# real-stanford/semantic-abstraction

Hardware: AMD Instinct MI355X
Metric: scenes/sec (relevancy+3D-UNet infer), 480x480x16-label x128^3 (higher is better)
Workload: dtype f16 (MFMA operands, fp32 accumulate; UNet hi/lo-split = fp32-equivalent); 1 GPU; end-to-end relevancy->fusion->OVSSC per scene: 480x480 RGB-D, 16 labels, ViT-B/16, 'ours' saliency config (2448 tile forwards), 128^3 voxels, 80000 input points; scene-sharded; arch=ViT-B/16, unet_precision=exact, tile_chunk_streams=1, scenes_per_gpu=26, parallelism=scene-shard x1, mode=throughput

## Files before the change

### include/semabs.h

```cpp
#ifndef SEMABS_H
#define SEMABS_H
#include <stdint.h>
#ifdef __cplusplus
extern "C" {
#endif

#define SEMABS_OK 0
#define SEMABS_EINVAL (-1)
#define SEMABS_EHIP (-2)

const char* semabs_last_error(void);
int semabs_abi_version(void);
int semabs_stream_create_cumask(const unsigned int* mask, int n_words, void** stream);
int semabs_stream_destroy(void* stream);
int semabs_stream_cu_count(void* stream, int* cus);

int semabs_fill_u32(void* p, long long nbytes, unsigned int value, void* stream);
int semabs_replicate(const void* src, void* dst, long long nbytes, int reps, void* stream);
int semabs_copy2d(const void* src, long long src_pitch_bytes, void* dst, long long dst_pitch_bytes, long long width_bytes, long long rows, void* stream);
int semabs_poison_empty(const long long* n_in, float* logits, long long n_logits, int* labels, long long n_labels, void* stream);
int semabs_device_info(char* name , int name_len, int* cu_count , long long* hbm_bytes );


int semabs_pointcloud(const float* depth, int H, int W, const double* params, int has_pose, float* xyz,
                      unsigned char* mask, void* stream);
int semabs_pointcloud_f64(const float* depth, int H, int W, const double* params_dev, int has_pose, double* xyz64, void* stream);

int semabs_voxel_index(const float* pts, long N, const float* off3, const float* scale3, const int* shape3,
                       long long* flat, int* idx3, void* stream);

int semabs_tsdf_integrate(const unsigned char* color, const float* depth, int H, int W, const double* params,
                          const float* origin3, const float* intr4, const int* dims3, float* tsdf, float* weight,
                          float* colvol, long long* pix_out, void* stream);

int semabs_frustum_mask(const double* pts, long M, const double* params, int H, int W, unsigned char* mask, void* stream);

int semabs_compact_subsample(const unsigned char* mask, long n, unsigned long long seed, long num, long long* pix, long long* n_in,
                             long long* sel, void* stream);

int semabs_gather_point_features(const float* rel, const long long* sel, const float* xyz, int L, long HW, long n,
                                 float mult, int subtract_mean, float* feat, float* xyz_out, void* stream);

int semabs_ovssc_labels(const float* logits, const unsigned char* in_frustum, const float* tsdf, int L, long M,
                        float cutoff, int* label, void* stream);


int semabs_resize_coeffs(int in_size, int out_size, int* xmin, int* kk, int kmax, int* ksize);

int semabs_tile_patches(const unsigned char* images, int n_img, int H, int W, const int* tiles, int n_tiles,
                        const int* coef_xmin, const int* coef_kk, const int* coef_ksize, const void* lut, void* patches,
                        int patch, int flip, int max_ksize, void* stream);

int semabs_patchify(const float* x, void* patches, int n, int patch, int flip, void* stream);

int semabs_aggregate(const float* rel, const float* rel_flip, int L, int N, int g, int H, int W, const int* scales,
                     int n_scales, int n_img, int tiles_per_img, float* out, void* stream);

int semabs_unflip_average(const float* rel, const float* rel_flip, float* out, long n_maps, int g, void* stream);
int semabs_unflip_average_rows(const float* rel, const float* rel_flip, float* out, int L, long maps_per_label, long in_label_stride, int g, void* stream);

int semabs_color_jitter(unsigned char* img, int H, int W, const int* order4, const float* factors4, void* scratch8, void* stream);
int semabs_color_jitter_op(unsigned char* img, int H, int W, int op, float factor, void* scratch8, void* stream);


int semabs_gemm_f16(const void* A, const void* B, void* C, const float* bias, const float* addend, long M, int N, int K,
                    long lda, int ldb, long ldc, int epi, const int* rowmap3, void* stream);

int semabs_gemm_f16_ex(const void* A, const void* B, void* C, const float* bias, const float* addend, long M, int N, int K,
                       long lda, int ldb, long ldc, int epi, const int* rowmap3, int kernel, void* start_event, void* stop_event,
                       void* stream);

int semabs_gemm_f16_ln(const void* A, const void* B, void* C, const float* bias, long M, int N, int K, long lda, int ldb, long ldc, int epi,
                       void* ln_xg, const float* ln_gamma, float* ln_part, const float* ln_center, const float* ln_rowac, const float* ln_colsum,
                       void* lo_out, int lo_cols, long ld_lo, int reverse,
                       void* start_event, void* stop_event, void* stream);
int semabs_ln_rowstats(const float* part, long M, int ntile, int D, float eps, float* rowac, const float* center_in, float* center_out, void* stream);


int semabs_layernorm(const float* x, const float* gamma, const float* beta, void* out, long M, int D, float eps,
                     int out_f32, long ld_in, float* mean_out, void* stream);
int semabs_layernorm2(const float* x, const float* g1, const float* b1, float* out1, const float* g2, const float* b2, void* out2, long M, int D, float eps,
                      int order, float* mean_out, void* stream);
int semabs_add_layernorm(float* x, const void* delta, const float* gamma, const float* beta, void* out, long M, int D, float eps,
                         void* stream);
int semabs_embed_finish(float* x, const float* cls, const float* pos, int n, int T, int D, void* stream);
int semabs_attention(const void* qkv, void* out, void* row_stats, int n_seq, int T, int H, int head_dim, int ld,
                     int causal, void* stream);
int semabs_attention_split(const void* qkv, const void* qk_lo, void* out, void* row_stats, int n_seq, int T, int H, int head_dim, int ld, int ld_lo,
                           int causal, void* stream);
int semabs_attention_cls(const float* q, const float* k, const void* v, float* probs, void* o, int n, int T, int H, int head_dim, int split, void* stream);
int semabs_cls_scores(const float* q, const void* wk, const float* bk, const void* x, long ldx, int split, float* probs, int n, int T, int D, void* stream);
int semabs_rows_gather(const float* src, float* dst, long rows, int cols, long src_stride, long offset, void* stream);
int semabs_eot_rows_gather(const long long* tokens, const float* x, float* dst, int B, int T, int D, void* stream);
int semabs_quickgelu(const float* fc, void* act, long n, int split_w, void* stream);
int semabs_quickgelu_grad(const float* fc, float* gd, long n, void* stream);
int semabs_logit_grad(const float* feat, const float* w_text, int n, int L, int E, float* logits, void* dfeat, float* scale, int split, void* stream);
int semabs_ln_bwd(const float* x, const float* gamma, const float* gy, const float* resid, float* out32, void* out16,
                  long M, int D, int n_x, long ld_x, float eps, int split, void* stream);
int semabs_gelu_bwd(const float* dact, const float* fc, void* dfc, long M, int W, int n_x, int split, void* stream);
int semabs_rollout(const float* probs, const void* v , const float* u, const float* scale, float* rel, int n, int T, int H,
                   int L, int positive_only, long n_total, long tile0, void* stream);
int semabs_attention_bwd(const void* qkv, const void* att, const float* fwd_stats, const void* dO, const float* rvec, const float* gscale,
                         float* c, float* stats, void* dqkv, int n, int L, int T, int H, int head_dim, int positive_only, void* stream);
int semabs_seq_rescale(float* g32, void* g16, float* gscale, long R, long len, void* stream);
int semabs_rollout_step(float* r, float* c, long n, void* stream);
int semabs_gather_text(const long long* tokens, const float* emb, const float* pos, float* x, int B, int T, int D, void* stream);
int semabs_text_finish(const float* e, float* w, int C, int P, int E, void* stream);


int semabs_point_mlp(const float* xyz, const float* feat, const float* w1, const float* b1, const float* w2, const float* b2,
                     const float* w3, const float* b3, float* out, int P, long N, int hidden, int cout, void* stream);
int semabs_point_mlp_fma(const float* xyz, const float* feat, const float* w1, const float* b1, const float* w2, const float* b2,
                         const float* w3, const float* b3, float* out, int P, long N, int hidden, int cout, void* stream);
int semabs_scatter_mean(const long long* flat, const float* feat, int* head, int* next, void* vol, int P, long N, int C,
                        long nvox, int vol_f32, void* stream);
int semabs_scatter_mean_stats(const long long* flat, const float* feat, int* head, int* next, void* vol, int P, long N, int C,
                              long nvox, int vol_f32, double* out_sums, void* stream);
int semabs_scatter_mean_sparse(const long long* flat, const float* feat, int* head, int* next, void* vol, unsigned int* occ, int P, long N, int C, long nvox,
                               int vol_f32, double* out_sums, void* stream);
int semabs_gn_stats(const void* x, double* sums, int B, long nvox, int C, int G, int x_f32, void* stream);
int semabs_gn_finalize(const double* sums, const float* gamma, const float* beta, float* scale, float* shift, int B, int C,
                       int G, long nvox, float eps, void* stream);
int semabs_conv3d(const void* x, const void* w_hi, const void* w_lo, void* y, const float* gn_scale, const float* gn_shift,
                  const float* bias, const void* resid, int B, int D0, int D1, int D2, int Cin, int Cout, int ksize, int relu,
                  int act_f32, void* stream);
int semabs_conv3d_stats(const void* x, const void* w_hi, const void* w_lo, void* y, const float* gn_scale, const float* gn_shift,
                        const float* bias, const void* resid, int B, int D0, int D1, int D2, int Cin, int Cout, int ksize, int relu,
                        int act_f32, double* out_sums, int out_groups, void* stream);
int semabs_conv3d_sparse_stats(const void* x, const unsigned int* occ, const void* w_hi, const void* w_lo, void* y, const float* gn_scale, const float* gn_shift,
                               const float* bias, const void* resid, int B, int D0, int D1, int D2, int Cin, int Cout, int ksize, int relu, int act_f32,
                               double* out_sums, int out_groups, void* stream);
int semabs_convtranspose3d(const void* x, const void* w_hi, const void* w_lo, const long* class_off , void* y,
                           const float* bias, const void* skip, int B, int D0, int D1, int D2, int Cin, int Cout, int act_f32,
                           void* stream);
int semabs_convtranspose3d_stats(const void* x, const void* w_hi, const void* w_lo, const long* class_off, void* y, const float* bias,
                                 const void* skip, int B, int D0, int D1, int D2, int Cin, int Cout, int act_f32, double* out_sums,
                                 int out_groups, void* stream);
int semabs_maxpool3d(const void* x, void* y, int B, int D0, int D1, int D2, int C, int act_f32, void* stream);
int semabs_decoder(const void* vol, const float* query, const float* off3, const float* sc3, const int* shape3, const float* w1,
                   const float* b1, const float* w2, const float* b2, int concat_xyz, int P, long M, long q_stride_p, int vol_f32,
                   float* out, const int* qgrid3, const float* final_w, const float* final_b, void* stream);

int semabs_vool_head(const void* vol_t, const void* vol_r, const float* query, const float* params, const float* rel,
                     const float* off3, const float* sc3, const int* shape3, float temperature, int P, long M, int vol_f32,
                     float* out, void* stream);


int semabs_lamb_step(const long long* chunks, int n_chunks, const long long* ptrs, int n_tensors, double lr, double beta1,
                     double beta2, double eps, double weight_decay, int adam, double* norms, float* stats, void* stream);


int semabs_conv3d_gather(const void* x, const void* w_hi, const void* w_lo, void* y, const float* in_scale, const float* in_shift, int B,
                         int I0, int I1, int I2, int M0, int M1, int M2, int in_stride, int Cin, int Cout, int ntaps, const signed char* taps,
                         int act_f32, void* stream);

int semabs_wgrad(const float* A, const float* X, const float* gn_scale, const float* gn_shift, float* dW, int B, int M0, int M1, int M2,
                 int I0, int I1, int I2, int in_stride, int Ca, int Cx, int ntaps, const signed char* taps, int tap_minor, void* stream);

int semabs_wgrad_mfma(const float* A, const float* X, const float* gn_scale, const float* gn_shift, const float* sA2, const float* sX2, float* dW,
                      int B, int M0, int M1, int M2, int I0, int I1, int I2, int in_stride, int Ca, int Cx, int ntaps, const signed char* taps,
                      int tap_minor, float* scratch, long scratch_floats, void* stream);

int semabs_wgrad_conv3(const float* dZ, const float* X, const float* gn_scale, const float* gn_shift, const float* s2, float* dW, int B, int D0,
                       int D1, int D2, int Ca, int Cx, int tap_minor, float* scratch, long scratch_floats, void* stream);
int semabs_wgrad_conv3_supported(int D0, int D1, int D2, int Ca, int Cx, long scratch_floats, int* kernel);
int semabs_wgrad_conv3_gn_supported(int B, int D0, int D1, int D2, int Ca, int Cx, long scratch_floats, int* ok);
int semabs_wgrad_conv3_gn(const float* dZ, const float* X, const float* mean, const float* rstd, int G, const float* gamma, const float* beta,
                          const float* W, const float* s2, float* dW, double* red, int B, int D0, int D1, int D2, int Ca, int Cx, float* scratch,
                          long scratch_floats, void* stream);

int semabs_conv3d_gnbwd_supported(int B, int D0, int D1, int D2, int Cin, int Cout, int G, int have_add1, int* ok);
int semabs_conv3d_gnbwd(const void* dZ, const void* w_hi, const void* w_lo, void* dX, const float* in_scale, const float* in_shift, const void* X,
                        const float* mean, const float* rstd, const float* coef, int G, const float* add1, int relu_mask, unsigned int* absmax_bits, int B,
                        int D0, int D1, int D2, int Cin, int Cout, int act_flags, void* stream);

int semabs_chan_reduce(const float* dY, const float* X, const float* mean, const float* rstd, double* out, int B, long nvox, int C, int G,
                       void* stream);
int semabs_gn_meanrstd(const double* sums, float* mean, float* rstd, int B, int G, long count, float eps, void* stream);
int semabs_gn_bwd_coef(const double* red, const float* gamma, const float* rstd, const float* inv_scale, float* coef, float* dgamma,
                       float* dbeta, int B, int C, int G, long nvox, void* stream);
int semabs_gn_bwd_apply(const float* dXn, const float* X, const float* mean, const float* rstd, const float* coef, const float* add1,
                        const float* add2, const float* mask_y, unsigned int* absmax_bits, float* dX, int B, long nvox, int C, int G, void* stream);

int semabs_ew(const float* a, const float* b, float* out, long n, int mode, float slope, unsigned int* absmax_bits, void* stream);
int semabs_ew_scaled(const float* a, const float* b, const float* in_scale, float* out, long n, int mode, float slope, unsigned int* absmax_bits,
                     void* stream);
int semabs_grad_scale(const float* x, long n, float* scale_arr, float* shift_arr, int n_arr, float* s2, unsigned int* bits, int have_bits,
                      void* stream);
int semabs_maxpool3d_bwd(const float* X, const float* dY, float* dX, int B, int D0, int D1, int D2, int C, void* stream);
int semabs_maxpool3d_bwd_add(const float* X, const float* dY, const float* add, float* dX, unsigned int* absmax_bits, int relu_mask, int B, int D0, int D1,
                             int D2, int C, void* stream);

int semabs_linear_f32(const float* X, const float* W, const float* bias, float* Y, long R, int Ci, int Co, int act, float slope, void* stream);
int semabs_linear_rows(const float* X, long ldx, const float* W, long w_sn, long w_sk, const float* bias, float* Y, long R, int Ci, int Co,
                       int act, float slope, const float* in_scale, const float* out_scale, const float* relu_mask, unsigned int* absmax_bits, float* colsum,
                       float* x_colsum, void* stream);

int semabs_scatter_mean_bwd(const long long* flat, int* count, const float* dvol, float* dpf, int P, long N, int C, long nvox, void* stream);

int semabs_vool_sample(const float* vol_t, const float* vol_r, const float* query, const float* off3, const float* sc3, const int* shape3,
                       int P, long M, float* f, void* stream);
int semabs_vool_sample_bwd(const float* df, const float* query, const float* off3, const float* sc3, const int* shape3, int P, long M,
                           int* head, int* next, float* dvol_t, float* dvol_r, unsigned int* absmax_bits, void* stream);

int semabs_cos_bce(const float* o, const float* rel, const float* label, const float* weight, int P, long M, float temperature, long n_total,
                   float* logits, float* dO, float* drel, double* loss, float* dbias, void* stream);

int semabs_gather_split16(const float* src, const int* idx, long n, void* hi, void* lo, void* stream);
int semabs_gather_split16_batched(const void* jobs, int njobs, long total_blocks, void* stream);

int semabs_cos_head(const float* o, const float* rel, const float* dlogits, int P, long M, float temperature, float* logits, float* dO,
                    float* drel, void* stream);

int semabs_clip_grad_norm(const long long* chunks, int n_chunks, const long long* ptrs, int n_tensors, float max_norm, float extra_scale,
                          double* sq, void* stream);


int semabs_relevancy_pack(const float* maps, float* out, int L, int H, int W, int h, int w, void* stream);
int semabs_text_pack(const float* feats, float* out, int L, int E, void* stream);
int semabs_relevancy_unpack(const float* stored, const long long* rows, const float* mean_map, float* out, int P, int h, int w, int H, int W,
                            float out_scale, void* stream);

int semabs_voxelize_eval(const long long* flat, const unsigned char* pred, const unsigned char* label, const unsigned char* ignore,
                         int* vol_scratch, unsigned char* out_pred, unsigned char* out_label, unsigned char* out_ignore, long BP, long N,
                         long nvox, void* stream);
int semabs_prediction_counts(const unsigned char* pred, const unsigned char* label, const unsigned char* ignore, unsigned long long* counts,
                             long BP, long M, void* stream);

int semabs_event_create(void** ev);
int semabs_event_destroy(void* ev);
int semabs_event_elapsed_ms(void* start, void* stop, float* ms);

#ifdef __cplusplus
}
#endif
#endif
```

### semantic-abstraction_amd/_lib.py

```python
from __future__ import annotations

import ctypes as C
import os

import torch

_HERE = os.path.dirname(os.path.abspath(__file__))
LIB_PATH = os.path.join(_HERE, "lib", "libsemabs_hip.so")
if os.environ.get("SEMABS_LIB_PATH"):
    LIB_PATH = os.environ["SEMABS_LIB_PATH"]
elif os.environ.get("SEMABS_TUNE_LIB") == "1":
    LIB_PATH = os.path.join(_HERE, "lib", "libsemabs_hip_tune.so")

_lib = None

P = C.c_void_p
I = C.c_int
L = C.c_long
F = C.c_float
D = C.c_double

SIGNATURES = {
    "semabs_abi_version": [],
    "semabs_stream_create_cumask": [P, I, P],
    "semabs_stream_destroy": [P],
    "semabs_stream_cu_count": [P, P],
    "semabs_fill_u32": [P, C.c_longlong, C.c_uint, P],
    "semabs_replicate": [P, P, C.c_longlong, I, P],
    "semabs_copy2d": [P, C.c_longlong, P, C.c_longlong, C.c_longlong, C.c_longlong, P],
    "semabs_poison_empty": [P, P, C.c_longlong, P, C.c_longlong, P],
    "semabs_device_info": [C.c_char_p, I, C.POINTER(I), C.POINTER(C.c_longlong)],
    "semabs_pointcloud": [P, I, I, P, I, P, P, P],
    "semabs_pointcloud_f64": [P, I, I, P, I, P, P],
    "semabs_voxel_index": [P, L, C.POINTER(F), C.POINTER(F), C.POINTER(I), P, P, P],
    "semabs_tsdf_integrate": [P, P, I, I, P, C.POINTER(F), C.POINTER(F), C.POINTER(I), P, P, P, P, P],
    "semabs_frustum_mask": [P, L, P, I, I, P, P],
    "semabs_compact_subsample": [P, L, C.c_ulonglong, L, P, P, P, P],
    "semabs_gather_point_features": [P, P, P, I, L, L, F, I, P, P, P],
    "semabs_ovssc_labels": [P, P, P, I, L, F, P, P],
    "semabs_resize_coeffs": [I, I, P, P, I, P],
    "semabs_tile_patches": [P, I, I, I, P, I, P, P, P, P, P, I, I, I, P],
    "semabs_patchify": [P, P, I, I, I, P],
    "semabs_aggregate": [P, P, I, I, I, I, I, P, I, I, I, P, P],
    "semabs_unflip_average": [P, P, P, L, I, P],
    "semabs_unflip_average_rows": [P, P, P, I, L, L, I, P],
    "semabs_color_jitter": [P, I, I, C.POINTER(I), C.POINTER(F), P, P],
    "semabs_color_jitter_op": [P, I, I, I, F, P, P],
    "semabs_gemm_f16": [P, P, P, P, P, L, I, I, L, I, L, I, C.POINTER(I), P],
    "semabs_gemm_f16_ex": [P, P, P, P, P, L, I, I, L, I, L, I, C.POINTER(I), I, P, P, P],
    "semabs_gemm_f16_ln": [P, P, P, P, L, I, I, L, I, L, I, P, P, P, P, P, P, P, I, L, I, P, P, P],
    "semabs_ln_rowstats": [P, L, I, I, F, P, P, P, P],
    "semabs_layernorm": [P, P, P, P, L, I, F, I, L, P, P],
    "semabs_layernorm2": [P, P, P, P, P, P, P, L, I, F, I, P, P],
    "semabs_add_layernorm": [P, P, P, P, P, L, I, F, P],
    "semabs_embed_finish": [P, P, P, I, I, I, P],
    "semabs_attention": [P, P, P, I, I, I, I, I, I, P],
    "semabs_attention_split": [P, P, P, P, I, I, I, I, I, I, I, P],
    "semabs_attention_cls": [P, P, P, P, P, I, I, I, I, I, P],
    "semabs_cls_scores": [P, P, P, P, L, I, P, I, I, I, P],
    "semabs_rows_gather": [P, P, L, I, L, L, P],
    "semabs_eot_rows_gather": [P, P, P, I, I, I, P],
    "semabs_quickgelu": [P, P, L, I, P],
    "semabs_quickgelu_grad": [P, P, L, P],
    "semabs_logit_grad": [P, P, I, I, I, P, P, P, I, P],
    "semabs_ln_bwd": [P, P, P, P, P, P, L, I, I, L, F, I, P],
    "semabs_gelu_bwd": [P, P, P, L, I, I, I, P],
    "semabs_rollout": [P, P, P, P, P, I, I, I, I, I, L, L, P],
    "semabs_gather_text": [P, P, P, P, I, I, I, P],
    "semabs_attention_bwd": [P, P, P, P, P, P, P, P, P, I, I, I, I, I, I, P],
    "semabs_seq_rescale": [P, P, P, L, L, P],
    "semabs_rollout_step": [P, P, L, P],
    "semabs_text_finish": [P, P, I, I, I, P],
    "semabs_point_mlp": [P, P, P, P, P, P, P, P, P, I, L, I, I, P],
    "semabs_point_mlp_fma": [P, P, P, P, P, P, P, P, P, I, L, I, I, P],
    "semabs_scatter_mean": [P, P, P, P, P, I, L, I, L, I, P],
    "semabs_scatter_mean_stats": [P, P, P, P, P, I, L, I, L, I, P, P],
    "semabs_scatter_mean_sparse": [P, P, P, P, P, P, I, L, I, L, I, P, P],
    "semabs_gn_stats": [P, P, I, L, I, I, I, P],
    "semabs_gn_finalize": [P, P, P, P, P, I, I, I, L, F, P],
    "semabs_conv3d": [P, P, P, P, P, P, P, P, I, I, I, I, I, I, I, I, I, P],
    "semabs_conv3d_stats": [P, P, P, P, P, P, P, P, I, I, I, I, I, I, I, I, I, P, I, P],
    "semabs_conv3d_sparse_stats": [P, P, P, P, P, P, P, P, P, I, I, I, I, I, I, I, I, I, P, I, P],
    "semabs_convtranspose3d": [P, P, P, C.POINTER(C.c_long), P, P, P, I, I, I, I, I, I, I, P],
    "semabs_convtranspose3d_stats": [P, P, P, C.POINTER(C.c_long), P, P, P, I, I, I, I, I, I, I, P, I, P],
    "semabs_maxpool3d": [P, P, I, I, I, I, I, I, P],
    "semabs_vool_head": [P, P, P, P, P, C.POINTER(F), C.POINTER(F), C.POINTER(I), F, I, L, I, P, P],
    "semabs_lamb_step": [P, I, P, I, D, D, D, D, D, I, P, P, P],
    "semabs_decoder": [P, P, C.POINTER(F), C.POINTER(F), C.POINTER(I), P, P, P, P, I, I, L, L, I, P, C.POINTER(I), P, P, P],
    "semabs_conv3d_gather": [P, P, P, P, P, P, I, I, I, I, I, I, I, I, I, I, I, C.c_char_p, I, P],
    "semabs_wgrad": [P, P, P, P, P, I, I, I, I, I, I, I, I, I, I, I, C.c_char_p, I, P],
    "semabs_wgrad_mfma": [P, P, P, P, P, P, P, I, I, I, I, I, I, I, I, I, I, I, C.c_char_p, I, P, L, P],
    "semabs_wgrad_conv3": [P, P, P, P, P, P, I, I, I, I, I, I, I, P, L, P],
    "semabs_wgrad_conv3_supported": [I, I, I, I, I, L, C.POINTER(I)],
    "semabs_conv3d_gnbwd_supported": [I, I, I, I, I, I, I, I, C.POINTER(I)],
    "semabs_conv3d_gnbwd": [P, P, P, P, P, P, P, P, P, P, I, P, I, P, I, I, I, I, I, I, I, P],
    "semabs_wgrad_conv3_gn_supported": [I, I, I, I, I, I, L, C.POINTER(I)],
    "semabs_wgrad_conv3_gn": [P, P, P, P, I, P, P, P, P, P, P, I, I, I, I, I, I, P, L, P],
    "semabs_chan_reduce": [P, P, P, P, P, I, L, I, I, P],
    "semabs_gn_meanrstd": [P, P, P, I, I, L, F, P],
    "semabs_gn_bwd_coef": [P, P, P, P, P, P, P, I, I, I, L, P],
    "semabs_gn_bwd_apply": [P, P, P, P, P, P, P, P, P, P, I, L, I, I, P],
    "semabs_ew": [P, P, P, L, I, F, P, P],
    "semabs_ew_scaled": [P, P, P, P, L, I, F, P, P],
    "semabs_grad_scale": [P, L, P, P, I, P, P, I, P],
    "semabs_maxpool3d_bwd": [P, P, P, I, I, I, I, I, P],
    "semabs_maxpool3d_bwd_add": [P, P, P, P, P, I, I, I, I, I, I, P],
    "semabs_linear_f32": [P, P, P, P, L, I, I, I, F, P],
    "semabs_linear_rows": [P, L, P, L, L, P, P, L, I, I, I, F, P, P, P, P, P, P, P],
    "semabs_scatter_mean_bwd": [P, P, P, P, I, L, I, L, P],
    "semabs_vool_sample": [P, P, P, C.POINTER(F), C.POINTER(F), C.POINTER(I), I, L, P, P],
    "semabs_vool_sample_bwd": [P, P, C.POINTER(F), C.POINTER(F), C.POINTER(I), I, L, P, P, P, P, P, P],
    "semabs_cos_bce": [P, P, P, P, I, L, F, L, P, P, P, P, P, P],
    "semabs_cos_head": [P, P, P, I, L, F, P, P, P, P],
    "semabs_gather_split16": [P, P, L, P, P, P],
    "semabs_gather_split16_batched": [P, I, L, P],
    "semabs_clip_grad_norm": [P, I, P, I, F, F, P, P],
    "semabs_relevancy_pack": [P, P, I, I, I, I, I, P],
    "semabs_text_pack": [P, P, I, I, P],
    "semabs_relevancy_unpack": [P, P, P, P, I, I, I, I, I, F, P],
    "semabs_voxelize_eval": [P, P, P, P, P, P, P, P, L, L, L, P],
    "semabs_prediction_counts": [P, P, P, P, L, L, P],
    "semabs_event_create": [C.POINTER(P)],
    "semabs_event_destroy": [P],
    "semabs_event_elapsed_ms": [P, P, C.POINTER(F)],
}


TUNING_SIGNATURES = {"semabs_gemm_tune": [I, C.c_longlong], "semabs_conv_tune": [I, C.c_longlong]}


def lib():
    global _lib
    if _lib is None:
        if not os.path.exists(LIB_PATH):
            raise RuntimeError(
                f"{LIB_PATH} is missing: the HIP extension was not built. Run "
                "`python semantic-abstraction_amd/build.py` (or __graft_entry__.build()). There is no CPU fallback."
            )
        h = C.CDLL(LIB_PATH)
        for name, argtypes in SIGNATURES.items():
            if not hasattr(h, name):
                continue
            fn = getattr(h, name)
            fn.argtypes = argtypes
            fn.restype = C.c_int
        for name, argtypes in TUNING_SIGNATURES.items():
            if hasattr(h, name):
                fn = getattr(h, name)
                fn.argtypes = argtypes
                fn.restype = C.c_int
        h.semabs_last_error.restype = C.c_char_p
        _lib = h
    return _lib


CALL_HOOK = None


def call(name: str, *args) -> None:
    h = lib()
    fn = getattr(h, name, None)
    if fn is None:
        raise RuntimeError(f"libsemabs_hip.so does not export {name}")
    hook = CALL_HOOK
    tok = hook.before(name, args) if hook is not None else None
    rc = fn(*args)
    if hook is not None:
        hook.after(tok)
    if rc != 0:
        raise RuntimeError(f"{name} failed (rc={rc}): {h.semabs_last_error().decode()}")


def ptr(t) -> int | None:
    if t is None:
        return None
    assert t.is_contiguous(), "semabs C ABI takes contiguous buffers"
    return t.data_ptr()


def stream() -> int:
    return torch.cuda.current_stream().cuda_stream


def require_gpu() -> torch.device:
    if not torch.cuda.is_available():
        raise RuntimeError("semabs_amd needs a HIP device (MI355X); there is no CPU fallback on the product path")
    return torch.device("cuda", torch.cuda.current_device())


def filled(shape, dtype: torch.dtype, value=0, device=None) -> torch.Tensor:
    t = torch.empty(shape, dtype=dtype, device=device if device is not None else require_gpu())
    fill_(t, value)
    return t


def fill_(t: torch.Tensor, value=0) -> torch.Tensor:
    import struct
    assert t.is_contiguous()
    nbytes = t.numel() * t.element_size()
    if nbytes == 0:
        return t
    if value == 0:
        pat = 0
    elif t.dtype == torch.float32:
        pat = struct.unpack("<I", struct.pack("<f", float(value)))[0]
    elif t.dtype == torch.int32:
        pat = int(value) & 0xFFFFFFFF
    else:
        raise TypeError(f"fill_: non-zero fill of {t.dtype}")
    assert nbytes % 4 == 0, "fill_: byte count must be a multiple of 4"
    call("semabs_fill_u32", t.data_ptr(), nbytes, pat, stream())
    return t


def farr(vals):
    return (F * len(vals))(*[float(v) for v in vals])


def iarr(vals):
    return (I * len(vals))(*[int(v) for v in vals])
```

### semantic-abstraction_amd/clip/__init__.py

```python
from __future__ import annotations

import ctypes as C
import os
from typing import Dict, List, Optional, Sequence

import numpy as np
import torch

from .. import _lib
from .templates import imagenet_templates
from .vit import TextEncoder, VisionRollout, make_vision_engine

KMAX = 24
CLIP_MEAN = (0.48145466, 0.4578275, 0.40821073)
CLIP_STD = (0.26862954, 0.26130258, 0.27577711)

saliency_configs = {
    "ours": lambda img_dim: {
        "distractor_labels": {},
        "horizontal_flipping": True,
        "augmentations": 5,
        "imagenet_prompt_ensemble": False,
        "positive_attn_only": True,
        "cropping_augmentations": [
# ... 48 lines not shown
        if ts not in self.sizes:
            xmin = np.zeros(224, np.int32)
            kk = np.zeros((224, KMAX), np.int32)
            ks = C.c_int(0)
            _lib.call("semabs_resize_coeffs", int(ts), 224, xmin.ctypes.data, kk.ctypes.data, KMAX, C.addressof(ks))
            self.sizes.append(ts); self.xmin.append(xmin); self.kk.append(kk); self.ksize.append(int(ks.value))
            self._dev = None
        return self.sizes.index(ts)

    def device(self):
        if self._dev is None:
            self._dev = (torch.from_numpy(np.stack(self.xmin)).to(self.dev), torch.from_numpy(np.stack(self.kk)).to(self.dev),
                         torch.tensor(self.ksize, dtype=torch.int32, device=self.dev))
        return self._dev


class ClipWrapper:

    engine: Optional[VisionRollout] = None
    text: Optional[TextEncoder] = None
    tokenizer = None
    device = None
    clip_model_type = None
    templates: List[str] = ["{}"]
    positive_attn_only = False
    class_to_language_feature: Dict[str, torch.Tensor] = {}
    _coeffs: Optional[_ResizeCoeffs] = None
    _lut = None
    _rng = np.random.default_rng(0)
    n_streams = 1
    _streams = None
    _patches = {}
    _plans = {}
    _jitter_scratch = None
    state_dict_provider = None

    def __init__(self, clip_model_type, device=None, state_dict=None, chunk_tiles=2448, max_labels=32, precision: str | None = None, **kwargs):
        dev = _lib.require_gpu()
        assert precision in (None, "default", "parity"), precision
        if state_dict is None:
            state_dict = ClipWrapper._load_checkpoint(clip_model_type)
        ClipWrapper.device = dev
        ClipWrapper.clip_model_type = clip_model_type
        ClipWrapper.engine = make_vision_engine(state_dict, chunk_tiles=chunk_tiles, max_labels=max_labels)
        if precision == "parity":
            if not hasattr(ClipWrapper.engine, "qk_split"):
                raise NotImplementedError('precision="parity" is implemented for the ViT-B towers (closed-form rollout)')
            ClipWrapper.engine.qk_split = True
        ClipWrapper.text = TextEncoder(state_dict) if "token_embedding.weight" in state_dict else None
        ClipWrapper._coeffs = _ResizeCoeffs(dev)
        u = np.arange(256, dtype=np.float32)[None, :] / np.float32(255)
        lut = (u - np.asarray(CLIP_MEAN, np.float32)[:, None]) / np.asarray(CLIP_STD, np.float32)[:, None]
        ClipWrapper._lut = torch.from_numpy(lut.astype(np.float32)).to(dev, torch.float16).contiguous()
        ClipWrapper.class_to_language_feature = {}
        ClipWrapper._patches = {}
        ClipWrapper._plans = {}
        ClipWrapper._jitter_scratch = None

    @staticmethod
    def _load_checkpoint(clip_model_type):
        if ClipWrapper.state_dict_provider is not None:
            return ClipWrapper.state_dict_provider(clip_model_type)
        fname = {"ViT-B/32": "ViT-B-32.pt", "ViT-B/16": "ViT-B-16.pt", "ViT-L/14": "ViT-L-14.pt"}.get(clip_model_type)
        if fname is None:
            raise RuntimeError(f"Model {clip_model_type} not found; available models = ['ViT-B/32', 'ViT-B/16', 'ViT-L/14']")
        path = clip_model_type if os.path.isfile(clip_model_type) else os.path.expanduser(f"~/.cache/clip/{fname}")
        if not os.path.isfile(path):
            raise RuntimeError(f"CLIP checkpoint {path} not found (no network here): put the OpenAI checkpoint there or "
                               "pass state_dict= / set ClipWrapper.state_dict_provider")
        try:
            return torch.jit.load(path, map_location="cpu").state_dict()
        except RuntimeError:
            return torch.load(path, map_location="cpu")

    @classmethod
    def check_initialized(cls, clip_model_type="ViT-B/32", **kwargs):
        if cls.engine is None:
            ClipWrapper(clip_model_type=clip_model_type, **kwargs)

    @classmethod
    def set_classes(cls, classes: Sequence[str]):
        cls.check_initialized()
        if cls.tokenizer is None:
            from .tokenizer import BPETokenizer
            cls.tokenizer = BPETokenizer()
        classes = [str(c) for c in classes]
        texts = [t.format(c) for c in classes for t in cls.templates]
        w = cls.set_classes_tokens(classes, cls.tokenizer.tokenize(texts), len(cls.templates))
        return w

    @classmethod
    def set_classes_tokens(cls, classes: Sequence[str], tokens: torch.Tensor, n_templates: int):
        cls.check_initialized()
        if cls.text is None:
            raise RuntimeError("the loaded state dict has no text tower")
        w = cls.text.zeroshot_weights(tokens, len(classes), n_templates)
        cls.class_to_language_feature = {c: w[i] for i, c in enumerate(classes)}
        return w

    @classmethod
    def get_clip_text_feature(cls, string):
        cls.check_initialized()
        if cls.tokenizer is None:
            from .tokenizer import BPETokenizer
            cls.tokenizer = BPETokenizer()
        strings = [string] if isinstance(string, str) else list(string)
        tok = cls.tokenizer.tokenize(strings)
        e = cls.text.encode(tok)
        return e.squeeze().cpu().numpy()

    @classmethod
    def get_clip_saliency(cls, img, text_labels, prompts, distractor_labels=set(), use_lavt=False, **kwargs):
        cls.check_initialized()
        if use_lavt:
            raise NotImplementedError("LAVT is not part of the reference either (ClipWrapper.lavt is never set)")
        cls.templates = prompts
        text_labels = [str(t) for t in text_labels]
        w = cls.set_classes(text_labels)
        text_label_features = w.cpu()
        text_maps = cls.get_clip_saliency_convolve(img=img, text_labels=text_labels, **kwargs)
        if len(distractor_labels) > 0:
            distractor_labels = set(distractor_labels) - set(text_labels)
            cls.set_classes(list(distractor_labels))
            distractor_maps = cls.get_clip_saliency_convolve(img=img, text_labels=list(distractor_labels), **kwargs)
            text_maps -= distractor_maps.mean(dim=0)
        return text_maps.cpu(), text_label_features

    @classmethod
    def get_clip_saliency_convolve(cls, text_labels, horizontal_flipping=False, positive_attn_only: bool = False,
                                   tile_batch_size=32, prompt_batch_size=32, tile_interpolate_batch_size=32, **kwargs):
        cls.positive_attn_only = positive_attn_only
        w = torch.stack([cls.class_to_language_feature[str(c)] for c in text_labels], dim=0).contiguous()
        images = cls.make_images(kwargs["img"], kwargs["augmentations"], kwargs.get("jittered_images"))
        return cls.relevancy_device(images, w, kwargs["cropping_augmentations"], horizontal_flipping, positive_attn_only).cpu()

    @classmethod
    def make_images(cls, img, augmentations: int, jittered_images=None, img_dev: torch.Tensor | None = None, seed: int | None = None) -> torch.Tensor:
        assert type(img) == np.ndarray and img.dtype == np.uint8 and img.ndim == 3 and img.shape[2] == 3
        cls.check_initialized()
        dev = cls.device
        base = img_dev if img_dev is not None else torch.from_numpy(np.ascontiguousarray(img)).to(dev)
        if augmentations == 0:
            return base[None].contiguous()
        if jittered_images is not None:
            assert len(jittered_images) == augmentations
            return torch.stack([base] + [torch.from_numpy(np.ascontiguousarray(j)).to(dev) for j in jittered_images])
        H, W = img.shape[:2]
        base = base.contiguous()
        out = torch.empty(augmentations + 1, H, W, 3, dtype=torch.uint8, device=dev)
        if (H * W * 3) % 4 == 0:
            _lib.call("semabs_replicate", _lib.ptr(base), _lib.ptr(out), H * W * 3, augmentations + 1, _lib.stream())
        else:
            out.copy_(base[None].expand_as(out))
        if cls._jitter_scratch is None:
            cls._jitter_scratch = torch.empty(1, dtype=torch.int64, device=dev)
        scratch = cls._jitter_scratch
        rng = cls._rng if seed is None else np.random.default_rng(seed)
        for k in range(1, augmentations + 1):
            order = rng.permutation(4)
            f = [rng.uniform(0.4, 1.6), rng.uniform(0.4, 1.6), rng.uniform(0.4, 1.6), rng.uniform(-0.1, 0.1)]
            _lib.call("semabs_color_jitter", out[k].data_ptr(), H, W, _lib.iarr(order), _lib.farr(f), _lib.ptr(scratch), _lib.stream())
        return out

    @classmethod
    def relevancy_device(cls, images: torch.Tensor, w_text: torch.Tensor, cropping_augmentations, horizontal_flipping: bool,
                         positive_attn_only: bool, tile_range=None, return_tiles: bool = False):
        cls.check_initialized()
        eng = cls.engine
        dev = cls.device
        n_img, H, W = int(images.shape[0]), int(images.shape[1]), int(images.shape[2])
        table, scales, tiles_dev, _ = cls._plan(H, W, n_img, cropping_augmentations)
        N = len(table)
        L = int(w_text.shape[0])
        g = eng.g
        xmin_d, kk_d, ks_d = cls._coeffs.device()
        max_ks = max(cls._coeffs.ksize) if cls._coeffs.ksize else 0
        passes = 2 if horizontal_flipping else 1
        G, Kp = g * g, 3 * eng.p * eng.p
        t_lo, t_hi = (0, N) if tile_range is None else tile_range
        rel_all = torch.empty(L, passes * (t_hi - t_lo), g, g, dtype=torch.float32, device=dev)
        main = torch.cuda.current_stream()
        n_per = t_hi - t_lo
        work = []
        for v0 in range(0, passes * n_per, eng.chunk):
            v1 = min(passes * n_per, v0 + eng.chunk)
            segs = []
            for flip in range(passes):
                a, b = max(v0, flip * n_per), min(v1, (flip + 1) * n_per)
                if a < b:
                    segs.append((flip, t_lo + a - flip * n_per, b - a))
            work.append(segs)
        ns = max(1, min(cls.n_streams, len(work)))
        if cls._streams is None or len(cls._streams) < ns:
            cls._streams = cls._make_streams(ns)
        key = (passes * n_per * G, Kp)
        if cls._patches.get("key") != key:
            cls._patches = {"key": key, "buf": torch.empty(key[0], Kp, dtype=torch.float16, device=dev)}
        patches_all = cls._patches["buf"]
        if n_per > 0:
            _lib.call("semabs_tile_patches", _lib.ptr(images), n_img, H, W, tiles_dev[t_lo:].data_ptr(), n_per, _lib.ptr(xmin_d),
                      _lib.ptr(kk_d), _lib.ptr(ks_d), _lib.ptr(cls._lut), _lib.ptr(patches_all), eng.p, 2 if passes == 2 else 0, max_ks, _lib.stream())
        for i in range(ns):
            cls._streams[i].wait_stream(main)
        w_chunks = [w_text[l0:l0 + eng.max_labels].contiguous() for l0 in range(0, L, eng.max_labels)]
        for i, segs in enumerate(work):
            slot = i % ns
            with torch.cuda.stream(cls._streams[slot]):
                eng.slot = slot
                m = sum(cnt for _, _, cnt in segs)
                v0 = i * eng.chunk
                patches = patches_all[v0 * G:(v0 + m) * G]
                if isinstance(eng, VisionRollout):
                    eng.embed(patches, m, defer_ln_pre=os.environ.get("SEMABS_LN2", "1") == "1")
                else:
                    eng.embed(patches, m)
                eng.trunk(m); eng.head(m)
                col0 = i * eng.chunk
                for li, wl in enumerate(w_chunks):
                    l0 = li * eng.max_labels
                    eng.rollout(m, wl, positive_attn_only, rel_all[l0:l0 + eng.max_labels], col0)
        for i in range(ns):
            main.wait_stream(cls._streams[i])
        eng.slot = 0
        for t in (images, tiles_dev, w_text, rel_all, patches_all, *w_chunks):
            for i in range(ns):
                t.record_stream(cls._streams[i])
        if tile_range is None and not return_tiles:
            return cls.aggregate_device([rel_all], scales, n_img, H, W, passes=passes, plan_key=(H, W, n_img, cls._aug_key(cropping_augmentations)))
        if tile_range is None:
            rel = [rel_all[:, p * N:(p + 1) * N].contiguous() if passes > 1 else rel_all for p in range(passes)]
        else:
            rel = [rel_all[:, p * n_per:(p + 1) * n_per].contiguous() for p in range(passes)]
        if return_tiles:
            return rel, table, scales
        return cls.aggregate_device(rel, scales, n_img, H, W)

    @classmethod
    def _make_streams(cls, ns: int):
        return [torch.cuda.Stream() for _ in range(ns)]

    @staticmethod
    def _aug_key(cropping_augmentations):
        return tuple((int(a["tile_size"]), int(a["stride"])) for a in cropping_augmentations)

    @classmethod
    def _plan(cls, H: int, W: int, n_img: int, cropping_augmentations):
        key = (H, W, n_img, cls._aug_key(cropping_augmentations))
        pl = cls._plans.get(key)
        if pl is None or pl[4] != len(cls._coeffs.sizes):
            table, scales = plan_tiles(H, W, n_img, cropping_augmentations)
            coef_ids = np.asarray([cls._coeffs.id_of(int(ts)) for ts in table[:, 3]], np.int32)
            tiles_dev = torch.from_numpy(np.concatenate([table, coef_ids[:, None]], axis=1).astype(np.int32)).to(cls.device).contiguous()
            scales_dev = torch.from_numpy(np.ascontiguousarray(scales, np.int32)).to(cls.device)
            if len(cls._plans) > 64:
                cls._plans.clear()
            pl = cls._plans[key] = (table, scales, tiles_dev, scales_dev, len(cls._coeffs.sizes))
        return pl[0], pl[1], pl[2], pl[3]

    @classmethod
    def aggregate_device(cls, rel, scales: np.ndarray, n_img: int, H: int, W: int, passes: int | None = None, plan_key=None) -> torch.Tensor:
        dev = cls.device
        fused = passes is not None
        L, g = int(rel[0].shape[0]), int(rel[0].shape[2])
        N = int(rel[0].shape[1]) // (passes if fused else 1)
        out = torch.empty(L, H, W, dtype=torch.float32, device=dev)
        pl = cls._plans.get(plan_key) if plan_key is not None else None
        sc = pl[3] if pl is not None else torch.from_numpy(np.ascontiguousarray(scales, np.int32)).to(dev)
        maps = rel[0]
        if fused and passes > 1:
            maps = torch.empty(L, N, g, g, dtype=torch.float32, device=dev)
            _lib.call("semabs_unflip_average_rows", _lib.ptr(rel[0]), rel[0].data_ptr() + N * g * g * 4, _lib.ptr(maps), L, N, passes * N, g, _lib.stream())
        elif len(rel) > 1:
            maps = torch.empty_like(rel[0])
            _lib.call("semabs_unflip_average", _lib.ptr(rel[0]), _lib.ptr(rel[1]), _lib.ptr(maps), L * N, g, _lib.stream())
        _lib.call("semabs_aggregate", _lib.ptr(maps), None, L, N, g, H, W, _lib.ptr(sc), len(scales), n_img, N // n_img, _lib.ptr(out), _lib.stream())
        return out


__all__ = ["ClipWrapper", "saliency_configs", "imagenet_templates", "plan_tiles"]
```

### semantic-abstraction_amd/csrc/tiles.hip

```cpp
#include "semabs_common.h"
#include <math.h>
#include <vector>

#define OUT_RES 224
#define PRECISION_BITS 22
#define KMAX 24

static double bicubic(double x) {
    const double a = -0.5;
    if (x < 0.0) x = -x;
    if (x < 1.0) return ((a + 2.0) * x - (a + 3.0)) * x * x + 1;
    if (x < 2.0) return (((x - 5) * x + 8) * x - 4) * a;
    return 0.0;
}

extern "C" int semabs_resize_coeffs(int in_size, int out_size, int* xmin_out, int* kk_out, int kmax, int* ksize_out) {
    SEMABS_REQUIRE(in_size > 0 && out_size > 0 && xmin_out && kk_out && ksize_out, "semabs_resize_coeffs: bad args");
    double scale = (double)((float)in_size - 0.0f) / out_size;
    double filterscale = scale < 1.0 ? 1.0 : scale;
    double support = 2.0 * filterscale;
    int ksize = (int)ceil(support) * 2 + 1;
    SEMABS_REQUIRE(ksize <= kmax, "semabs_resize_coeffs: down-scale factor too large for KMAX taps");
    std::vector<double> k(ksize);
    for (int xx = 0; xx < out_size; ++xx) {
// ... 155 lines not shown
    }
    __syncthreads();
    if (tid >= OUT_RES) return;
    const int g = OUT_RES / p, pp = p * p, Kp = 3 * pp;
    const int rg = tid / (OUT_RES / 2), x = (tid - rg * (OUT_RES / 2)) * 2;
    const unsigned short* shs = reinterpret_cast<const unsigned short*>(&sh[0][0][0]);
    const int xf = OUT_RES - 2 - x;
    const int px0 = x / p, ix0 = x - px0 * p, px1 = xf / p, ix1 = xf - px1 * p;
    for (int yy = rg * (BAND / 2); yy < (rg + 1) * (BAND / 2); ++yy) {
        const int y = y_first + yy;
        int v[2][3];
        if (identity) {
            const unsigned short* s = shs + (((y - r_lo) * OUT_RES + x) >> 1) * 3;
            const int s0 = s[0], s1 = s[1], s2 = s[2];
            v[0][0] = s0 & 255; v[0][1] = s0 >> 8; v[0][2] = s1 & 255; v[1][0] = s1 >> 8; v[1][1] = s2 & 255; v[1][2] = s2 >> 8;
        } else {
            const int yb = s_xmin[y] - r_lo;
            switch (ksize) {
                case 5: tile_vpass<5>(shs, s_ky[yy], ksize, yb, n_rows, x, v); break;
                case 7: tile_vpass<7>(shs, s_ky[yy], ksize, yb, n_rows, x, v); break;
                case 9: tile_vpass<9>(shs, s_ky[yy], ksize, yb, n_rows, x, v); break;
                case 11: tile_vpass<11>(shs, s_ky[yy], ksize, yb, n_rows, x, v); break;
                default: tile_vpass<0>(shs, s_ky[yy], ksize, yb, n_rows, x, v); break;
            }
        }
        f16x2 o[3], of[3];
#pragma unroll
        for (int c = 0; c < 3; ++c) {
            const f16 l = s_lut[c * 256 + v[0][c]], r = s_lut[c * 256 + v[1][c]];
            o[c][0] = l; o[c][1] = r; of[c][0] = r; of[c][1] = l;
        }
        const int py = y / p, iy = y - py * p;
        if (flip != 1) {
            f16* dst = patches + ((long)t * g * g + py * g + px0) * Kp + iy * p + ix0;
#pragma unroll
            for (int c = 0; c < 3; ++c) *reinterpret_cast<f16x2*>(dst + c * pp) = o[c];
        }
        if (flip != 0) {
            f16* dst = patches + ((long)(flip == 2 ? t + n_tiles : t) * g * g + py * g + px1) * Kp + iy * p + ix1;
#pragma unroll
            for (int c = 0; c < 3; ++c) *reinterpret_cast<f16x2*>(dst + c * pp) = of[c];
        }
    }
}

extern "C" int semabs_tile_patches(const unsigned char* images, int n_img, int H, int W, const int* tiles_dev, int n_tiles,
                                   const int* coef_xmin, const int* coef_kk, const int* coef_ksize, const void* lut,
                                   void* patches, int patch, int flip, int max_ksize, void* stream) {
    if (n_tiles == 0) return SEMABS_OK;
    SEMABS_REQUIRE(images && tiles_dev && coef_xmin && coef_kk && coef_ksize && lut && patches, "semabs_tile_patches: null pointer");
    SEMABS_REQUIRE(n_img > 0 && H > 0 && W > 0 && (patch == 16 || patch == 32 || patch == 14), "semabs_tile_patches: bad shape / patch size");
    SEMABS_REQUIRE(flip >= 0 && flip <= 2, "semabs_tile_patches: flip must be 0 (as is), 1 (mirrored) or 2 (both: patches holds 2 n_tiles tiles)");
    SEMABS_REQUIRE(OUT_RES % patch == 0, "semabs_tile_patches: patch must divide 224");
    SEMABS_REQUIRE(max_ksize <= KMAX && (max_ksize - 1) / 4.0 * BAND + max_ksize + 2 <= MAX_IN_ROWS,
                   "semabs_tile_patches: tile_size / 224 too large for the LDS band (tile_size must be <= ~490)");
    hipLaunchKernelGGL(k_tile_patches, dim3(n_tiles, OUT_RES / BAND), dim3(256), 0, (hipStream_t)stream, images, H, W, tiles_dev,
                       coef_xmin, coef_kk, coef_ksize, (const f16*)lut, (f16*)patches, patch, flip, n_tiles);
    SEMABS_CHECK_LAUNCH();
    return SEMABS_OK;
}

__global__ void k_patchify(const float* __restrict__ x, f16* __restrict__ patches, int n, int p, int flip) {
    long i = (long)blockIdx.x * blockDim.x + threadIdx.x;
    const long tot = (long)n * 3 * OUT_RES * OUT_RES;
    if (i >= tot) return;
    int xq = (int)(i % OUT_RES); long r = i / OUT_RES;
    int y = (int)(r % OUT_RES); r /= OUT_RES;
    int c = (int)(r % 3); long t = r / 3;
    const int g = OUT_RES / p, pp = p * p;
    const int xo = flip ? OUT_RES - 1 - xq : xq;
    const int py = y / p, iy = y % p, px = xo / p, ix = xo % p;
    patches[((long)t * g * g + py * g + px) * 3 * pp + c * pp + iy * p + ix] = (f16)x[i];
}
extern "C" int semabs_patchify(const float* x, void* patches, int n, int patch, int flip, void* stream) {
    if (n == 0) return SEMABS_OK;
    SEMABS_REQUIRE(x && patches && n > 0 && OUT_RES % patch == 0, "semabs_patchify: bad args");
    hipLaunchKernelGGL(k_patchify, dim3(semabs_cdiv((long)n * 3 * OUT_RES * OUT_RES, 256)), dim3(256), 0, (hipStream_t)stream, x,
                       (f16*)patches, n, patch, flip);
    SEMABS_CHECK_LAUNCH();
    return SEMABS_OK;
}

struct AggArgs {
    int L, N, g, H, W, n_img, tiles_per_img, n_scales;
};

__device__ __forceinline__ void bil_setup(int d, float scale, int g, int& i0, int& i1, float& l0, float& l1) {
    float s = scale * ((float)d + 0.5f) - 0.5f;
    if (s < 0.f) s = 0.f;
    i0 = (int)s;
    if (i0 > g - 1) i0 = g - 1;
    i1 = i0 + (i0 < g - 1 ? 1 : 0);
    l1 = s - (float)i0;
    l0 = 1.f - l1;
}

__global__ __launch_bounds__(256) void k_aggregate(const float* __restrict__ rel, const float* __restrict__ rel_flip,
                                                   const int* __restrict__ scales, AggArgs a, float* __restrict__ out) {
    const long i = (long)blockIdx.x * blockDim.x + threadIdx.x;
    const long tot = (long)a.L * a.H * a.W;
    if (i >= tot) return;
    const int c = (int)(i % a.W); const long t = i / a.W;
    const int r = (int)(t % a.H); const int l = (int)(t / a.H);
    const int g = a.g, gg = g * g;
    float total = 0.f;
    for (int s = 0; s < a.n_scales; ++s) {
        const int ts = scales[s * 5], stride = scales[s * 5 + 1], nx = scales[s * 5 + 2], ny = scales[s * 5 + 3], base = scales[s * 5 + 4];
        int ix_hi = r / stride; if (ix_hi > nx - 1) ix_hi = nx - 1;
        int ix_lo = r - ts + 1 <= 0 ? 0 : (r - ts + 1 + stride - 1) / stride;
        int iy_hi = c / stride; if (iy_hi > ny - 1) iy_hi = ny - 1;
        int iy_lo = c - ts + 1 <= 0 ? 0 : (c - ts + 1 + stride - 1) / stride;
        __half acc = __float2half(0.f);
        float cnt = 1e-5f;
        const float bscale = (float)g / (float)ts;
        for (int im = 0; im < a.n_img; ++im) {
            for (int iy = iy_lo; iy <= iy_hi; ++iy) {
                int w0, w1; float lw0, lw1;
                bil_setup(c - iy * stride, bscale, g, w0, w1, lw0, lw1);
                for (int ix = ix_lo; ix <= ix_hi; ++ix) {
                    int h0, h1; float lh0, lh1;
                    bil_setup(r - ix * stride, bscale, g, h0, h1, lh0, lh1);
                    const long tile = (long)im * a.tiles_per_img + base + iy * nx + ix;
                    const float* p = rel + ((long)l * a.N + tile) * gg;
                    float v00 = p[h0 * g + w0], v01 = p[h0 * g + w1], v10 = p[h1 * g + w0], v11 = p[h1 * g + w1];
                    if (rel_flip) {
                        const float* q = rel_flip + ((long)l * a.N + tile) * gg;
                        v00 = (v00 + q[h0 * g + (g - 1 - w0)]) / 2; v01 = (v01 + q[h0 * g + (g - 1 - w1)]) / 2;
                        v10 = (v10 + q[h1 * g + (g - 1 - w0)]) / 2; v11 = (v11 + q[h1 * g + (g - 1 - w1)]) / 2;
                    }
                    const float val = lh0 * (lw0 * v00 + lw1 * v01) + lh1 * (lw0 * v10 + lw1 * v11);
                    acc = __float2half(__half2float(acc) + val);
                    cnt += 1.0f;
                }
            }
        }
        total = total + __half2float(acc) / cnt;
    }
    out[i] = total / (float)a.n_scales;
}

extern "C" int semabs_aggregate(const float* rel, const float* rel_flip, int L, int N, int g, int H, int W,
                                const int* scales_dev, int n_scales, int n_img, int tiles_per_img, float* out, void* stream) {
    if (L == 0) return SEMABS_OK;
    SEMABS_REQUIRE(rel && scales_dev && out && L > 0 && N > 0 && g > 0 && H > 0 && W > 0 && n_scales > 0 && n_img > 0,
                   "semabs_aggregate: bad args");
    SEMABS_REQUIRE((long)n_img * tiles_per_img == N, "semabs_aggregate: tile count does not match n_img * tiles_per_img");
    AggArgs a{L, N, g, H, W, n_img, tiles_per_img, n_scales};
    hipLaunchKernelGGL(k_aggregate, dim3(semabs_cdiv((long)L * H * W, 256)), dim3(256), 0, (hipStream_t)stream, rel, rel_flip,
                       scales_dev, a, out);
    SEMABS_CHECK_LAUNCH();
    return SEMABS_OK;
}

__global__ void k_unflip_average(const float* __restrict__ rel, const float* __restrict__ rel_flip, float* __restrict__ out, long n, int g,
                                 long per, long in_stride) {
    const long i = (long)blockIdx.x * blockDim.x + threadIdx.x;
    if (i >= n) return;
    const int w = (int)(i % g);
    const long l = i / per, src = l * in_stride + (i - l * per);
    out[i] = (rel[src] + rel_flip[src - w + (g - 1 - w)]) / 2;
}
extern "C" int semabs_unflip_average(const float* rel, const float* rel_flip, float* out, long n_maps, int g, void* stream) {
    if (n_maps == 0) return SEMABS_OK;
    SEMABS_REQUIRE(rel && rel_flip && out && n_maps > 0 && g > 0, "semabs_unflip_average: bad args");
    const long n = n_maps * g * g;
    hipLaunchKernelGGL(k_unflip_average, dim3(semabs_cdiv(n, 256)), dim3(256), 0, (hipStream_t)stream, rel, rel_flip, out, n, g, n, n);
    SEMABS_CHECK_LAUNCH();
    return SEMABS_OK;
}
extern "C" int semabs_unflip_average_rows(const float* rel, const float* rel_flip, float* out, int L, long maps_per_label, long in_label_stride,
                                          int g, void* stream) {
    if (L == 0 || maps_per_label == 0) return SEMABS_OK;
    SEMABS_REQUIRE(rel && rel_flip && out && L > 0 && maps_per_label > 0 && in_label_stride >= maps_per_label && g > 0, "semabs_unflip_average_rows: bad args");
    const long per = maps_per_label * g * g, n = (long)L * per;
    hipLaunchKernelGGL(k_unflip_average, dim3(semabs_cdiv(n, 256)), dim3(256), 0, (hipStream_t)stream, rel, rel_flip, out, n, g, per, in_label_stride * g * g);
    SEMABS_CHECK_LAUNCH();
    return SEMABS_OK;
}

__device__ __forceinline__ int grey_u8(int r, int g, int b) { return (r * 19595 + g * 38470 + b * 7471 + 0x8000) >> 16; }
__device__ __forceinline__ unsigned char blend_u8(float a, float b, float f) {
    float t = a + f * (b - a);
    return (unsigned char)(t <= 0.f ? 0.f : (t >= 255.f ? 255.f : t));
}
__device__ __forceinline__ int clip8(int v) { return v < 0 ? 0 : (v > 255 ? 255 : v); }
__device__ __forceinline__ void rgb2hsv_u8(int r, int g, int b, int& uh, int& us, int& uv) {
    const int maxc = max(r, max(g, b)), minc = min(r, min(g, b));
    uv = maxc;
    if (minc == maxc) { uh = 0; us = 0; return; }
    const float cr = (float)(maxc - minc);
    const float s = __fdiv_rn(cr, (float)maxc);
    const float rc = __fdiv_rn((float)(maxc - r), cr), gc = __fdiv_rn((float)(maxc - g), cr), bc = __fdiv_rn((float)(maxc - b), cr);
    float h;
    if (r == maxc) h = __fsub_rn(bc, gc);
    else if (g == maxc) h = (float)(2.0 + (double)rc - (double)bc);
    else h = (float)(4.0 + (double)gc - (double)rc);
    h = (float)fmod((double)h / 6.0 + 1.0, 1.0);
    uh = clip8((int)((double)h * 255.0));
    us = clip8((int)((double)s * 255.0));
}
__device__ __forceinline__ void hsv2rgb_u8(int h, int s, int v, int& r, int& g, int& b) {
    if (s == 0) { r = g = b = v; return; }
    const double hd = (double)(float)h * 6.0 / 255.0;
    const int i = (int)floor(hd);
    const double f = (double)(float)(hd - (double)(float)i);
    const double fs = (double)(float)((double)(float)s / 255.0);
    const double vf = (double)(float)v;
    const int p = clip8((int)round(vf * (1.0 - fs)));
    const int q = clip8((int)round(vf * (1.0 - fs * f)));
    const int t = clip8((int)round(vf * (1.0 - fs * (1.0 - f))));
    switch (i % 6) {
        case 0: r = v; g = t; b = p; break;
        case 1: r = q; g = v; b = p; break;
        case 2: r = p; g = v; b = t; break;
        case 3: r = p; g = q; b = v; break;
        case 4: r = t; g = p; b = v; break;
        default: r = v; g = p; b = q; break;
    }
}

__global__ void k_grey_sum(const unsigned char* __restrict__ img, long n, unsigned long long* __restrict__ sum) {
    long i = (long)blockIdx.x * blockDim.x + threadIdx.x;
    float v = 0.f;
    if (i < n) v = (float)grey_u8(img[i * 3], img[i * 3 + 1], img[i * 3 + 2]);
    v = wave_sum(v);
    if ((threadIdx.x & 63) == 0) atomicAdd(sum, (unsigned long long)(v + 0.5f));
}

__global__ void k_jitter_op(const unsigned char* __restrict__ src, unsigned char* __restrict__ dst, long n, int op, float f,
                            const unsigned long long* __restrict__ grey_sum) {
    long i = (long)blockIdx.x * blockDim.x + threadIdx.x;
    if (i >= n) return;
    int r = src[i * 3], g = src[i * 3 + 1], b = src[i * 3 + 2];
    if (op == 0) {
        r = blend_u8(0.f, r, f); g = blend_u8(0.f, g, f); b = blend_u8(0.f, b, f);
    } else if (op == 1) {
        float m = (float)(int)((double)(*grey_sum) / (double)n + 0.5);
        r = blend_u8(m, r, f); g = blend_u8(m, g, f); b = blend_u8(m, b, f);
    } else if (op == 2) {
        float m = (float)grey_u8(r, g, b);
        r = blend_u8(m, r, f); g = blend_u8(m, g, f); b = blend_u8(m, b, f);
    } else {
        int uh, us, uv;
        rgb2hsv_u8(r, g, b, uh, us, uv);
        uh = (uh + (int)f) & 255;
        hsv2rgb_u8(uh, us, uv, r, g, b);
    }
    dst[i * 3] = (unsigned char)r; dst[i * 3 + 1] = (unsigned char)g; dst[i * 3 + 2] = (unsigned char)b;
}

extern "C" int semabs_color_jitter_op(unsigned char* img, int H, int W, int op, float factor, void* scratch8, void* stream) {
    SEMABS_REQUIRE(img && scratch8 && H > 0 && W > 0, "semabs_color_jitter_op: bad args");
    SEMABS_REQUIRE(op >= 0 && op < 4, "semabs_color_jitter_op: op must be 0..3");
    hipStream_t s = (hipStream_t)stream;
    const long n = (long)H * W;
    float f = factor;
    if (op == 1) {
        semabs_fill32(scratch8, 8, 0u, s);
        hipLaunchKernelGGL(k_grey_sum, dim3(semabs_cdiv(n, 256)), dim3(256), 0, s, img, n, (unsigned long long*)scratch8);
    } else if (op == 3) {
        SEMABS_REQUIRE(f >= -0.5f && f <= 0.5f, "semabs_color_jitter_op: hue factor must lie in [-0.5, 0.5] (torchvision adjust_hue)");
        f = (float)(((int)((double)f * 255.0) % 256 + 256) % 256);
    }
    hipLaunchKernelGGL(k_jitter_op, dim3(semabs_cdiv(n, 256)), dim3(256), 0, s, img, img, n, op, f, (const unsigned long long*)scratch8);
    SEMABS_CHECK_LAUNCH();
    return SEMABS_OK;
}

extern "C" int semabs_color_jitter(unsigned char* img, int H, int W, const int* order4, const float* factors4,
                                   void* scratch8, void* stream) {
    SEMABS_REQUIRE(img && order4 && factors4 && scratch8 && H > 0 && W > 0, "semabs_color_jitter: bad args");
    for (int k = 0; k < 4; ++k) {
        SEMABS_REQUIRE(order4[k] >= 0 && order4[k] < 4, "semabs_color_jitter: op must be 0..3");
        const int rc = semabs_color_jitter_op(img, H, W, order4[k], factors4[order4[k]], scratch8, stream);
        if (rc != SEMABS_OK) return rc;
    }
    return SEMABS_OK;
}
```

### semantic-abstraction_amd/csrc/unet.hip

```cpp
#include "semabs_common.h"

__device__ __forceinline__ int xcd_remap(int vb, int nb) {
    const int q = nb >> 3, r = nb & 7, x = vb & 7, k = vb >> 3;
    return (x < r ? x * (q + 1) : r * (q + 1) + (x - r) * q) + k;
}
__device__ __forceinline__ int xcd_persistent_tile(int vb, int G, int it, int total) {
    if (G & 7) { const long t = (long)it * G + vb; return t < total ? (int)t : -1; }
    const int x = vb & 7, j = vb >> 3, g8 = G >> 3;
    const int q = total >> 3, r = total & 7;
    const int lo = x < r ? x * (q + 1) : r * (q + 1) + (x - r) * q, cnt = q + (x < r ? 1 : 0);
    const long o = (long)it * g8 + j;
    return o < cnt ? lo + (int)o : -1;
}


template <int HID, int COUT>
__global__ __launch_bounds__(256, 2) void k_point_mlp(const float* __restrict__ xyz, const float* __restrict__ feat,
                                                   const float* __restrict__ w1, const float* __restrict__ b1,
                                                   const float* __restrict__ w2, const float* __restrict__ b2,
                                                   const float* __restrict__ w3, const float* __restrict__ b3,
                                                   float* __restrict__ out, int P, long N) {
    extern __shared__ __attribute__((aligned(16))) char smem[];
    float* sw2 = reinterpret_cast<float*>(smem);
    float* sw3 = sw2 + HID * HID;
// ... 254 lines not shown
    }
    }
    if (stats) {
        if (__ballot(worker) != 0) {
            const int bw = __builtin_amdgcn_readfirstlane(b);
            const bool uniform_b = __ballot(b != bw) == 0;
            if (uniform_b) {
#pragma unroll
                for (int g = 0; g < 8; ++g) {
                    float a = gs[g], q = gq[g];
#pragma unroll
                    for (int m = 1; m < 64; m <<= 1) { a += __shfl_xor(a, m, 64); q += __shfl_xor(q, m, 64); }
                    if ((threadIdx.x & 63) == 0) { atomicAdd(stats + ((long)bw * 8 + g) * 2, (double)a); atomicAdd(stats + ((long)bw * 8 + g) * 2 + 1, (double)q); }
                }
            } else if (worker) {
#pragma unroll
                for (int g = 0; g < 8; ++g) { atomicAdd(stats + ((long)b * 8 + g) * 2, (double)gs[g]); atomicAdd(stats + ((long)b * 8 + g) * 2 + 1, (double)gq[g]); }
            }
        }
    }
}

static int scatter_mean_impl(const long long* flat, const float* feat, int* head, int* next, void* vol, int P, long N, int C,
                             long nvox, int vol_f32, double* stats, void* stream, unsigned int* occ = nullptr) {
    if (P == 0 || N == 0) return SEMABS_OK;
    SEMABS_REQUIRE(flat && feat && head && next && vol && C > 0 && nvox > 0, "semabs_scatter_mean: bad args");
    hipStream_t s = (hipStream_t)stream;
    hipLaunchKernelGGL(k_scatter_link, dim3(semabs_cdiv(N, 256)), dim3(256), 0, s, flat, N, head, next);
    if (vol_f32) hipLaunchKernelGGL(k_scatter_mean<float>, dim3(semabs_cdiv((long)P * N, 256)), dim3(256), 0, s, flat, feat, head, next, (float*)vol, P, N, C, nvox, stats, occ);
    else hipLaunchKernelGGL(k_scatter_mean<f16>, dim3(semabs_cdiv((long)P * N, 256)), dim3(256), 0, s, flat, feat, head, next, (f16*)vol, P, N, C, nvox, stats, occ);
    SEMABS_CHECK_LAUNCH();
    return SEMABS_OK;
}
extern "C" int semabs_scatter_mean(const long long* flat, const float* feat, int* head, int* next, void* vol, int P, long N, int C,
                                   long nvox, int vol_f32, void* stream) {
    return scatter_mean_impl(flat, feat, head, next, vol, P, N, C, nvox, vol_f32, nullptr, stream);
}
extern "C" int semabs_scatter_mean_stats(const long long* flat, const float* feat, int* head, int* next, void* vol, int P, long N, int C,
                                         long nvox, int vol_f32, double* out_sums, void* stream) {
    SEMABS_REQUIRE(out_sums && C == 16, "semabs_scatter_mean_stats: needs out_sums and C == 16");
    return scatter_mean_impl(flat, feat, head, next, vol, P, N, C, nvox, vol_f32, out_sums, stream);
}
extern "C" int semabs_scatter_mean_sparse(const long long* flat, const float* feat, int* head, int* next, void* vol, unsigned int* occ, int P, long N, int C,
                                          long nvox, int vol_f32, double* out_sums, void* stream) {
    SEMABS_REQUIRE(out_sums && occ && C == 16, "semabs_scatter_mean_sparse: needs out_sums, occ and C == 16");
    return scatter_mean_impl(flat, feat, head, next, vol, P, N, C, nvox, vol_f32, out_sums, stream, occ);
}

template <typename T>
__global__ __launch_bounds__(256) void k_gn_stats(const T* __restrict__ x, double* __restrict__ sums, long nvox, int C, int G) {
    const int b = blockIdx.y;
    const int cpv = C / 8;
    const long chunks = nvox * cpv;
    const int cg = C / G;
    const T* xb = x + (long)b * nvox * C;
    long stride = (long)gridDim.x * 256;
    stride -= stride % cpv;
    const long start = (long)blockIdx.x * 256 + threadIdx.x;
    float s[8], q[8];
#pragma unroll
    for (int j = 0; j < 8; ++j) { s[j] = 0.f; q[j] = 0.f; }
    if (start < stride)
        for (long i = start; i < chunks; i += stride) {
            float v[8];
            if (sizeof(T) == 2) {
                f16x8 h = *reinterpret_cast<const f16x8*>(reinterpret_cast<const f16*>(xb) + i * 8);
#pragma unroll
                for (int j = 0; j < 8; ++j) v[j] = (float)h[j];
            } else {
                const float4* p4 = reinterpret_cast<const float4*>(reinterpret_cast<const float*>(xb) + i * 8);
                float4 a = p4[0], c = p4[1];
                v[0] = a.x; v[1] = a.y; v[2] = a.z; v[3] = a.w; v[4] = c.x; v[5] = c.y; v[6] = c.z; v[7] = c.w;
            }
#pragma unroll
            for (int j = 0; j < 8; ++j) { s[j] += v[j]; q[j] += v[j] * v[j]; }
        }
    __shared__ float sh[2][512];
    for (int c = threadIdx.x; c < C; c += 256) { sh[0][c] = 0.f; sh[1][c] = 0.f; }
    __syncthreads();
    if (start < stride) {
        const int c0 = (int)(start % cpv) * 8;
#pragma unroll
        for (int j = 0; j < 8; ++j) { atomicAdd(&sh[0][c0 + j], s[j]); atomicAdd(&sh[1][c0 + j], q[j]); }
    }
    __syncthreads();
    for (int g = threadIdx.x; g < G; g += 256) {
        float ss = 0.f, qq = 0.f;
        for (int k = 0; k < cg; ++k) { ss += sh[0][g * cg + k]; qq += sh[1][g * cg + k]; }
        atomicAdd(&sums[((long)b * G + g) * 2], (double)ss);
        atomicAdd(&sums[((long)b * G + g) * 2 + 1], (double)qq);
    }
}

extern "C" int semabs_gn_stats(const void* x, double* sums, int B, long nvox, int C, int G, int x_f32, void* stream) {
    if (B == 0) return SEMABS_OK;
    SEMABS_REQUIRE(x && sums && nvox > 0 && C % 8 == 0 && C <= 512 && G > 0 && C % G == 0, "semabs_gn_stats: bad args (C % 8 == 0, C <= 512)");
    long chunks = nvox * (C / 8);
    int bx = semabs_cdiv(chunks, 256 * 16); if (bx < 1) bx = 1; if (bx > 256) bx = 256;
    if (x_f32) hipLaunchKernelGGL(k_gn_stats<float>, dim3(bx, B), dim3(256), 0, (hipStream_t)stream, (const float*)x, sums, nvox, C, G);
    else hipLaunchKernelGGL(k_gn_stats<f16>, dim3(bx, B), dim3(256), 0, (hipStream_t)stream, (const f16*)x, sums, nvox, C, G);
    SEMABS_CHECK_LAUNCH();
    return SEMABS_OK;
}

__global__ void k_gn_finalize(const double* __restrict__ sums, const float* __restrict__ gamma, const float* __restrict__ beta,
                              float* __restrict__ scale, float* __restrict__ shift, int B, int C, int G, double count, float eps) {
    int i = blockIdx.x * blockDim.x + threadIdx.x;
    if (i >= B * C) return;
    const int b = i / C, c = i % C, g = c / (C / G);
    const double mean = sums[((long)b * G + g) * 2] / count;
    double var = sums[((long)b * G + g) * 2 + 1] / count - mean * mean;
    if (var < 0) var = 0;
    const float rstd = (float)(1.0 / sqrt(var + (double)eps));
    const float sc = rstd * gamma[c];
    scale[i] = sc;
    shift[i] = beta[c] - (float)mean * sc;
}
extern "C" int semabs_gn_finalize(const double* sums, const float* gamma, const float* beta, float* scale, float* shift, int B, int C,
                                  int G, long nvox, float eps, void* stream) {
    if (B == 0) return SEMABS_OK;
    SEMABS_REQUIRE(sums && gamma && beta && scale && shift && C % G == 0 && nvox > 0, "semabs_gn_finalize: bad args");
    hipLaunchKernelGGL(k_gn_finalize, dim3(semabs_cdiv((long)B * C, 256)), dim3(256), 0, (hipStream_t)stream, sums, gamma, beta, scale,
                       shift, B, C, G, (double)nvox * (C / G), eps);
    SEMABS_CHECK_LAUNCH();
    return SEMABS_OK;
}

#ifdef SEMABS_TUNING
#define CONV16_ABL(c) (c)
#else
#define CONV16_ABL(c) false
#endif
struct ConvArgs {
    const void* x; void* y; const f16* w_hi; const f16* w_lo;
    const float* gn_scale; const float* gn_shift; const float* bias; const void* resid;
    int B, I0, I1, I2;
    int O0, O1, O2;
    int M0, M1, M2;
    int os, op0, op1, op2;
    int Cin, Cout, Kp;
    int ntaps; int relu;
    int is;
    int ksplit;
    signed char td0[28], td1[28], td2[28];
    double* stats;
    int ablate;
    long long* trace;
    const f16* wp_hi; const f16* wp_lo;
    int ncls; long cls_off[8];
    const float* gnb_coef = nullptr; const float* gnb_mean = nullptr; const float* gnb_rstd = nullptr; int gnb_G = 0, gnb_relu = 0;
    unsigned int* gnb_bits = nullptr;
    const unsigned int* occ = nullptr;
    const float* gnb_add = nullptr;
};

template <bool F32>
__device__ __forceinline__ void load8(const void* base, long idx, float (&v)[8]) {
    if (F32) {
        const float4* p = reinterpret_cast<const float4*>(reinterpret_cast<const float*>(base) + idx);
        float4 a = p[0], b = p[1];
        v[0] = a.x; v[1] = a.y; v[2] = a.z; v[3] = a.w; v[4] = b.x; v[5] = b.y; v[6] = b.z; v[7] = b.w;
    } else {
        f16x8 h = *reinterpret_cast<const f16x8*>(reinterpret_cast<const f16*>(base) + idx);
#pragma unroll
        for (int j = 0; j < 8; ++j) v[j] = (float)h[j];
    }
}

template <int NW, bool F32, bool CIN16, bool LDSW = false, bool CLS = false>
__global__ __launch_bounds__(256) void k_conv(ConvArgs a) {
    const int ccls = CLS ? (int)blockIdx.z : 0;
    const int cp0 = CLS ? ccls >> 2 : 0, cp1 = CLS ? (ccls >> 1) & 1 : 0, cp2 = CLS ? ccls & 1 : 0;
    const int k_ntaps = CLS ? (cp0 + 1) * (cp1 + 1) * (cp2 + 1) : a.ntaps;
    const int k_Kp = CLS ? k_ntaps * a.Cin : a.Kp;
    const int k_op0 = CLS ? cp0 : a.op0, k_op1 = CLS ? cp1 : a.op1, k_op2 = CLS ? cp2 : a.op2;
    const long k_woff = CLS ? a.cls_off[ccls] : 0;
    const f16* const k_w_hi = a.w_hi + k_woff; const f16* const k_w_lo = a.w_lo ? a.w_lo + k_woff : nullptr;
    const f16* const k_wp_hi = a.wp_hi ? a.wp_hi + k_woff : nullptr; const f16* const k_wp_lo = a.wp_lo ? a.wp_lo + k_woff : nullptr;
    constexpr int MW = 2;
    static_assert(!LDSW || (NW == 4 && !CIN16), "LDSW: four waves x four output-channel tiles");
    __shared__ __attribute__((aligned(16))) f16x8 s_w[LDSW ? 2 : 1][LDSW ? 4 : 1][2][LDSW ? 64 : 1];
    const int lane = threadIdx.x & 63, wid = threadIdx.x >> 6;
    const int vl = lane & 15, kg = lane >> 4;
    const long Mtot = (long)a.B * a.M0 * a.M1 * a.M2;
    const long mbase = ((long)blockIdx.x * 4 + wid) * (MW * 16);
    if (!LDSW && mbase >= Mtot) return;
    const int n0 = blockIdx.y * (NW * 16);
    const bool has_gn = a.gn_scale != nullptr;

    int vb[MW], v0[MW], v1[MW], v2[MW]; bool vok[MW];
#pragma unroll
    for (int mi = 0; mi < MW; ++mi) {
        long m = mbase + mi * 16 + vl;
        vok[mi] = m < Mtot;
        if (!vok[mi]) m = Mtot - 1;
        v2[mi] = (int)(m % a.M2); m /= a.M2;
        v1[mi] = (int)(m % a.M1); m /= a.M1;
        v0[mi] = (int)(m % a.M0); vb[mi] = (int)(m / a.M0);
    }
    f32x4 acc[MW][NW];
#pragma unroll
    for (int mi = 0; mi < MW; ++mi)
#pragma unroll
        for (int ni = 0; ni < NW; ++ni) acc[mi][ni] = f32x4{0.f, 0.f, 0.f, 0.f};

    float gsc[MW][8], gsh[MW][8];
    if (CIN16 && has_gn) {
#pragma unroll
        for (int mi = 0; mi < MW; ++mi)
#pragma unroll
            for (int j = 0; j < 8; ++j) {
                gsc[mi][j] = a.gn_scale[vb[mi] * 16 + 8 * (kg & 1) + j];
                gsh[mi][j] = a.gn_shift[vb[mi] * 16 + 8 * (kg & 1) + j];
            }
    }
    const int cin_steps = CIN16 ? 1 : a.Cin / 32;
    const int nsteps = CIN16 ? (k_ntaps + 1) / 2 : k_ntaps * cin_steps;
    struct Raw { float v[MW][8]; bool ok[MW]; f16x8 wh[NW], wl[NW]; };
    auto fetch = [&](int ks, Raw& R) {
        int tap, c0;
        if (CIN16) { tap = 2 * ks + (kg >> 1); c0 = 8 * (kg & 1); }
        else { tap = ks / cin_steps; c0 = (ks - tap * cin_steps) * 32 + 8 * kg; }
        const bool tap_ok = tap < k_ntaps;
        int d0 = 0, d1 = 0, d2 = 0;
        if (tap_ok) {
            if (CLS) {
                const int t2 = tap % (cp2 + 1), r = tap / (cp2 + 1), t1 = r % (cp1 + 1), t0 = r / (cp1 + 1);
                d0 = (cp0 && t0 == 0) ? 1 : 0; d1 = (cp1 && t1 == 0) ? 1 : 0; d2 = (cp2 && t2 == 0) ? 1 : 0;
            } else { d0 = a.td0[tap]; d1 = a.td1[tap]; d2 = a.td2[tap]; }
        }
#pragma unroll
        for (int mi = 0; mi < MW; ++mi) {
            const int i0 = v0[mi] * a.is + d0, i1 = v1[mi] * a.is + d1, i2 = v2[mi] * a.is + d2;
            const bool ok = tap_ok && vok[mi] && i0 >= 0 && i0 < a.I0 && i1 >= 0 && i1 < a.I1 && i2 >= 0 && i2 < a.I2;
            R.ok[mi] = ok;
            if (ok) load8<F32>(a.x, ((((long)vb[mi] * a.I0 + i0) * a.I1 + i1) * a.I2 + i2) * a.Cin + c0, R.v[mi]);
            else {
#pragma unroll
                for (int j = 0; j < 8; ++j) R.v[mi][j] = 0.f;
            }
        }
#pragma unroll
        for (int ni = 0; ni < NW; ++ni) {
            if (LDSW && ni != 0) continue;
            const int cb = (n0 >> 4) + (LDSW ? wid : ni);
            const long widx = k_wp_hi ? ((long)(ks * (a.Cout >> 4) + cb) * 64 + lane) * 8 : (long)(cb * 16 + vl) * k_Kp + ks * 32 + kg * 8;
            R.wh[ni] = *reinterpret_cast<const f16x8*>((k_wp_hi ? k_wp_hi : k_w_hi) + widx);
            if (F32) R.wl[ni] = *reinterpret_cast<const f16x8*>((k_wp_hi ? k_wp_lo : k_w_lo) + widx);
        }
    };
    auto park = [&](int ks, Raw& R) {
        s_w[ks & 1][wid][0][lane] = R.wh[0];
        if (F32) s_w[ks & 1][wid][1][lane] = R.wl[0];
        __syncthreads();
    };
    auto consume = [&](int ks, Raw& R) {
        int c0 = 0;
        if (!CIN16) { const int tap = ks / cin_steps; c0 = (ks - tap * cin_steps) * 32 + 8 * kg; }
        f16x8 xh[MW], xl[MW];
#pragma unroll
        for (int mi = 0; mi < MW; ++mi) {
            float v[8];
#pragma unroll
            for (int j = 0; j < 8; ++j) v[j] = R.v[mi][j];
            const bool ok = R.ok[mi];
            if (ok && has_gn) {
                if (CIN16) {
#pragma unroll
                    for (int j = 0; j < 8; ++j) v[j] = v[j] * gsc[mi][j] + gsh[mi][j];
                } else {
                    const float4* ps = reinterpret_cast<const float4*>(a.gn_scale + (long)vb[mi] * a.Cin + c0);
                    const float4* pt = reinterpret_cast<const float4*>(a.gn_shift + (long)vb[mi] * a.Cin + c0);
                    float4 s0 = ps[0], s1 = ps[1], t0 = pt[0], t1 = pt[1];
                    v[0] = v[0] * s0.x + t0.x; v[1] = v[1] * s0.y + t0.y; v[2] = v[2] * s0.z + t0.z; v[3] = v[3] * s0.w + t0.w;
                    v[4] = v[4] * s1.x + t1.x; v[5] = v[5] * s1.y + t1.y; v[6] = v[6] * s1.z + t1.z; v[7] = v[7] * s1.w + t1.w;
                }
            }
            if (!ok) {
#pragma unroll
                for (int j = 0; j < 8; ++j) v[j] = 0.f;
            }
#pragma unroll
            for (int j = 0; j < 8; ++j) {
                xh[mi][j] = (f16)v[j];
                if (F32) xl[mi][j] = (f16)(v[j] - (float)xh[mi][j]);
            }
        }
#pragma unroll
        for (int ni = 0; ni < NW; ++ni) {
            const f16x8 wh = LDSW ? s_w[ks & 1][ni][0][lane] : R.wh[ni];
            f16x8 wl;
            if (F32) wl = LDSW ? s_w[ks & 1][ni][1][lane] : R.wl[ni];
#pragma unroll
            for (int mi = 0; mi < MW; ++mi) acc[mi][ni] = __builtin_amdgcn_mfma_f32_16x16x32_f16(wh, xh[mi], acc[mi][ni], 0, 0, 0);
            if (F32) {
#pragma unroll
                for (int mi = 0; mi < MW; ++mi) {
                    acc[mi][ni] = __builtin_amdgcn_mfma_f32_16x16x32_f16(wl, xh[mi], acc[mi][ni], 0, 0, 0);
                    acc[mi][ni] = __builtin_amdgcn_mfma_f32_16x16x32_f16(wh, xl[mi], acc[mi][ni], 0, 0, 0);
                }
            }
        }
    };
    int ks_lo = 0, ks_hi = nsteps;
    if (a.ksplit > 1) {
        const int per = (nsteps + a.ksplit - 1) / a.ksplit;
        ks_lo = blockIdx.z * per; ks_hi = ks_lo + per < nsteps ? ks_lo + per : nsteps;
    }
    Raw R0, R1;
    if (ks_lo < ks_hi) fetch(ks_lo, R0);
    if (LDSW) {
        if (ks_lo < ks_hi) park(ks_lo, R0);
        for (int ks = ks_lo; ks < ks_hi; ks += 2) {
            if (ks + 1 < ks_hi) fetch(ks + 1, R1);
            consume(ks, R0);
            if (ks + 1 < ks_hi) {
                park(ks + 1, R1);
                if (ks + 2 < ks_hi) fetch(ks + 2, R0);
                consume(ks + 1, R1);
                if (ks + 2 < ks_hi) park(ks + 2, R0);
            }
        }
    } else
    for (int ks = ks_lo; ks < ks_hi; ks += 2) {
        if (ks + 1 < ks_hi) fetch(ks + 1, R1);
        consume(ks, R0);
        if (ks + 1 < ks_hi) {
            if (ks + 2 < ks_hi) fetch(ks + 2, R0);
            consume(ks + 1, R1);
        }
    }
#pragma unroll
    for (int mi = 0; mi < MW; ++mi) {
        if (!vok[mi]) continue;
        const long ovox = (((long)vb[mi] * a.O0 + (v0[mi] * a.os + k_op0)) * a.O1 + (v1[mi] * a.os + k_op1)) * a.O2 + (v2[mi] * a.os + k_op2);
#pragma unroll
        for (int ni = 0; ni < NW; ++ni) {
            const int co = n0 + ni * 16 + 4 * kg;
            float o[4] = {acc[mi][ni][0], acc[mi][ni][1], acc[mi][ni][2], acc[mi][ni][3]};
            if (F32 && a.ksplit > 1) {
                float* yp = reinterpret_cast<float*>(a.y) + ovox * a.Cout + co;
#pragma unroll
                for (int e = 0; e < 4; ++e) atomicAdd(yp + e, o[e]);
                continue;
            }
            if (a.bias) {
                const float4 bv = *reinterpret_cast<const float4*>(a.bias + co);
                o[0] += bv.x; o[1] += bv.y; o[2] += bv.z; o[3] += bv.w;
            }
            const long oidx = ovox * a.Cout + co;
            if (a.resid) {
                if (F32) {
                    const float4 r = *reinterpret_cast<const float4*>(reinterpret_cast<const float*>(a.resid) + oidx);
                    o[0] += r.x; o[1] += r.y; o[2] += r.z; o[3] += r.w;
                } else {
                    const f16x4 r = *reinterpret_cast<const f16x4*>(reinterpret_cast<const f16*>(a.resid) + oidx);
                    o[0] += (float)r[0]; o[1] += (float)r[1]; o[2] += (float)r[2]; o[3] += (float)r[3];
                }
            }
            if (a.relu == 1) { o[0] = fmaxf(o[0], 0.f); o[1] = fmaxf(o[1], 0.f); o[2] = fmaxf(o[2], 0.f); o[3] = fmaxf(o[3], 0.f); }
            else if (a.relu == 2) {
#pragma unroll
                for (int j = 0; j < 4; ++j) o[j] = o[j] > 0.f ? o[j] : 0.01f * o[j];
            }
            if (F32) {
                *reinterpret_cast<float4*>(reinterpret_cast<float*>(a.y) + oidx) = make_float4(o[0], o[1], o[2], o[3]);
            } else {
                f16x4 h; h[0] = (f16)o[0]; h[1] = (f16)o[1]; h[2] = (f16)o[2]; h[3] = (f16)o[3];
                *reinterpret_cast<f16x4*>(reinterpret_cast<f16*>(a.y) + oidx) = h;
            }
        }
    }
}

#define C16_T1 8
#define C16_T2 16
#define C16_H1 (C16_T1 + 2)
#define C16_H2 (C16_T2 + 2)

__device__ __forceinline__ void conv_absmax_commit(unsigned int* bits, float m) {
#pragma unroll
    for (int o = 1; o < 64; o <<= 1) m = fmaxf(m, __shfl_xor(m, o, 64));
    if ((threadIdx.x & 63) == 0) atomicMax(bits, __float_as_uint(m));
}
template <bool F32, int C16_T0, bool GNB = false, bool SPARSE = false>
__global__ __launch_bounds__(512) void k_conv16_lds(ConvArgs a) {
    constexpr int C16_H0 = C16_T0 + 2, C16_HALO = C16_H0 * C16_H1 * C16_H2;
    constexpr int PLANE = (C16_HALO * 8 + 127) / 128 * 128;
    constexpr int BUF_EL = PLANE * 2 * (F32 ? 2 : 1);
    extern __shared__ __attribute__((aligned(16))) char smem[];
    const int tid = threadIdx.x, lane = tid & 63;
    const int wid = __builtin_amdgcn_readfirstlane(tid >> 6);
    const int vl = lane & 15, kg = lane >> 4;
    const int n2 = a.I2 / C16_T2, n1 = a.I1 / C16_T1, n0 = a.I0 / C16_T0;
    const int per_vol = n0 * n1 * n2, total = a.B * per_vol;
    const bool has_gn = a.gn_scale != nullptr;
    const bool producer = wid >= 4;
    const int ptid = tid - 256;
    float* const s_gnb = reinterpret_cast<float*>(smem + (size_t)BUF_EL * 2 * 2);
    if (GNB) {
        for (int e = tid; e < a.B * 16; e += 512) {
            const int b = e >> 4, c = e & 15, g = c / (16 / a.gnb_G);
            const float mu = a.gnb_mean[b * a.gnb_G + g], rs = a.gnb_rstd[b * a.gnb_G + g];
            const float* k = a.gnb_coef + (long)e * 3;
            s_gnb[b * 48 + c] = k[0]; s_gnb[b * 48 + 16 + c] = -rs * k[2]; s_gnb[b * 48 + 32 + c] = mu * rs * k[2] - k[1];
        }
    }
    float amax = 0.f;

    auto produce = [&](int brick, int buf) {
        const int b = brick / per_vol; int t = brick - b * per_vol;
        const int t2 = t % n2; t /= n2;
        const int t1 = t % n1; const int t0 = t / n1;
        const int z0 = t0 * C16_T0, y0 = t1 * C16_T1, x0 = t2 * C16_T2;
        f16* s_hi = reinterpret_cast<f16*>(smem) + buf * BUF_EL;
        f16* s_lo = s_hi + PLANE * 2;
        const int hsel = (ptid >> 3) & 1;
        const int vsub = (ptid & 7) + ((ptid >> 4) << 3);
        float gs[8], gh[8];
        if (has_gn) {
            const float4* ps = reinterpret_cast<const float4*>(a.gn_scale + b * 16 + hsel * 8);
            const float4* pt = reinterpret_cast<const float4*>(a.gn_shift + b * 16 + hsel * 8);
            const float4 s0 = ps[0], s1 = ps[1], h0 = pt[0], h1 = pt[1];
            gs[0] = s0.x; gs[1] = s0.y; gs[2] = s0.z; gs[3] = s0.w; gs[4] = s1.x; gs[5] = s1.y; gs[6] = s1.z; gs[7] = s1.w;
            gh[0] = h0.x; gh[1] = h0.y; gh[2] = h0.z; gh[3] = h0.w; gh[4] = h1.x; gh[5] = h1.y; gh[6] = h1.z; gh[7] = h1.w;
        } else {
#pragma unroll
            for (int j = 0; j < 8; ++j) { gs[j] = 1.f; gh[j] = 0.f; }
        }
        constexpr int NT = (C16_HALO + 127) / 128;
        const float* xb = reinterpret_cast<const float*>(a.x) + (size_t)b * a.I0 * a.I1 * a.I2 * 16;
        const f16* xbh = reinterpret_cast<const f16*>(a.x) + (size_t)b * a.I0 * a.I1 * a.I2 * 16;
        float raw[NT][8];
        bool inb[NT];
        [[maybe_unused]] unsigned oword[NT];
        [[maybe_unused]] int vflat[NT];
        if constexpr (SPARSE) {
#pragma unroll
            for (int k = 0; k < NT; ++k) {
                const int v = min(vsub + k * 128, C16_HALO - 1);
                const int hx = v % C16_H2, hy = (v / C16_H2) % C16_H1, hz = v / (C16_H2 * C16_H1);
                const int cz = min(max(z0 + hz - 1, 0), a.I0 - 1), cy = min(max(y0 + hy - 1, 0), a.I1 - 1), cx = min(max(x0 + hx - 1, 0), a.I2 - 1);
                vflat[k] = (cz * a.I1 + cy) * a.I2 + cx;
                oword[k] = a.occ[vflat[k] >> 5];
            }
        }
#pragma unroll
        for (int k = 0; k < NT; ++k) {
            const int v = min(vsub + k * 128, C16_HALO - 1);
            const int hx = v % C16_H2, hy = (v / C16_H2) % C16_H1, hz = v / (C16_H2 * C16_H1);
            const int gz = z0 + hz - 1, gy = y0 + hy - 1, gx = x0 + hx - 1;
            inb[k] = gz >= 0 && gz < a.I0 && gy >= 0 && gy < a.I1 && gx >= 0 && gx < a.I2;
            const int cz = min(max(gz, 0), a.I0 - 1), cy = min(max(gy, 0), a.I1 - 1), cx = min(max(gx, 0), a.I2 - 1);
            unsigned eo = (unsigned)(((cz * a.I1 + cy) * a.I2 + cx) * 16 + hsel * 8);
            if constexpr (SPARSE) {
                const bool full = (oword[k] >> (vflat[k] & 31)) & 1u;
                oword[k] = full ? 1u : 0u;
                if (!full) eo = (unsigned)(hsel * 8);
            }
            {
                if (F32) {
                    const float4 q0 = *reinterpret_cast<const float4*>(xb + eo), q1 = *reinterpret_cast<const float4*>(xb + eo + 4);
                    raw[k][0] = q0.x; raw[k][1] = q0.y; raw[k][2] = q0.z; raw[k][3] = q0.w; raw[k][4] = q1.x; raw[k][5] = q1.y; raw[k][6] = q1.z; raw[k][7] = q1.w;
                } else {
                    const f16x8 q = *reinterpret_cast<const f16x8*>(xbh + eo);
#pragma unroll
                    for (int c = 0; c < 8; ++c) raw[k][c] = (float)q[c];
                }
            }
        }
#pragma unroll
        for (int k = 0; k < NT; ++k) {
            const int v = vsub + k * 128;
            f16x8 h, l;
#pragma unroll
            for (int c = 0; c < 8; ++c) {
                const float rv = (SPARSE && !oword[k]) ? 0.f : raw[k][c];
                const float val = inb[k] ? rv * gs[c] + gh[c] : 0.f;
                h[c] = (f16)val;
                if (F32) l[c] = (f16)(val - (float)h[c]);
            }
            if (v < C16_HALO) {
                *reinterpret_cast<f16x8*>(s_hi + hsel * PLANE + v * 8) = h;
                if (F32) *reinterpret_cast<f16x8*>(s_lo + hsel * PLANE + v * 8) = l;
            }
        }
    };

    f16x8 wh[3][5], wl[3][5];
    auto load_weights = [&]() {
#pragma unroll
        for (int dy = 0; dy < 3; ++dy)
#pragma unroll
            for (int st = 0; st < 5; ++st) {
                const int qa = 2 * st, qb = 2 * st + 1;
                const int tapa = (qa / 3) * 9 + dy * 3 + (qa % 3);
                const int tapb = qb < 9 ? (qb / 3) * 9 + dy * 3 + (qb % 3) : 27;
                const long widx = (long)vl * a.Kp + ((kg >> 1) ? tapb : tapa) * 16 + (kg & 1) * 8;
                wh[dy][st] = *reinterpret_cast<const f16x8*>(a.w_hi + widx);
                if (F32) wl[dy][st] = *reinterpret_cast<const f16x8*>(a.w_lo + widx);
            }
    };
    const int half = kg & 1, tsel = kg >> 1;
    f32x4 bias4 = f32x4{0.f, 0.f, 0.f, 0.f};
    if (a.bias) bias4 = *reinterpret_cast<const f32x4*>(a.bias + 4 * kg);
    const float relu_floor = a.relu ? 0.f : -__builtin_inff();
    double st[4] = {0.0, 0.0, 0.0, 0.0};
    int st_b = -1;
    auto flush_stats = [&]() {
        if (st_b >= 0) {
#pragma unroll
            for (int j = 0; j < 4; ++j) {
                double v = st[j];
#pragma unroll
                for (int m = 1; m < 16; m <<= 1) v += __shfl_xor(v, m, 64);
                if (vl == 0) atomicAdd(a.stats + ((long)st_b * 8 + 2 * kg + (j >> 1)) * 2 + (j & 1), v);
                st[j] = 0.0;
            }
        }
    };
    constexpr int ROWS_PER_WAVE = C16_T0 * 2;

    auto consume = [&](int brick, int buf) {
        const int b = brick / per_vol; int t = brick - b * per_vol;
        const int t2 = t % n2; t /= n2;
        const int t1 = t % n1; const int t0 = t / n1;
        const int z0 = t0 * C16_T0, y0 = t1 * C16_T1, x0 = t2 * C16_T2;
        const f16* s_hi = reinterpret_cast<const f16*>(smem) + buf * BUF_EL;
        const f16* s_lo = s_hi + PLANE * 2;
        const size_t vol_off = (size_t)b * a.I0 * a.I1 * a.I2 * 16;
        if (a.stats && b != st_b) { flush_stats(); st_b = b; }
        constexpr int MR = 8;
        int tapoff[5];
#pragma unroll
        for (int st = 0; st < 5; ++st) {
            const int qa = 2 * st, qb = 2 * st + 1 < 9 ? 2 * st + 1 : 2 * st;
            const int q = tsel ? qb : qa;
            tapoff[st] = ((q / 3) * C16_H1 * C16_H2 + (q % 3)) * 8;
        }
#pragma unroll 1
        for (int pr = 0; pr < ROWS_PER_WAVE / MR; ++pr) {
            const int zl = (wid * ROWS_PER_WAVE + pr * MR) >> 3;
            const int fbase = half * PLANE + (zl * C16_H1 * C16_H2 + vl) * 8;
            f32x4 acc[MR];
#pragma unroll
            for (int mi = 0; mi < MR; ++mi) acc[mi] = f32x4{0.f, 0.f, 0.f, 0.f};
            unsigned ooff[MR];
            f32x4 res[MR];
#pragma unroll
            for (int mi = 0; mi < MR; ++mi) {
                ooff[mi] = (unsigned)((((z0 + zl) * a.I1 + (y0 + mi)) * a.I2 + (x0 + vl)) * 16 + 4 * kg);
                res[mi] = f32x4{0.f, 0.f, 0.f, 0.f};
            }
            if (a.resid) {
#pragma unroll
                for (int mi = 0; mi < MR; ++mi) {
                    if (F32) res[mi] = *reinterpret_cast<const f32x4*>(reinterpret_cast<const float*>(a.resid) + vol_off + ooff[mi]);
                    else {
                        const f16x4 r = *reinterpret_cast<const f16x4*>(reinterpret_cast<const f16*>(a.resid) + vol_off + ooff[mi]);
                        res[mi] = f32x4{(float)r[0], (float)r[1], (float)r[2], (float)r[3]};
                    }
                }
            }
            f16x8 xh[3], xl[3];
            constexpr int RHO[10] = {2, 0, 3, 1, 4, 9, 5, 8, 6, 7};
            auto request = [&](int i, int slot) {
                const int st = i / 10, rho = RHO[i % 10];
                const int off = fbase + tapoff[st] + rho * (C16_H2 * 8);
                xh[slot] = *reinterpret_cast<const f16x8*>(s_hi + off);
                if (F32) xl[slot] = *reinterpret_cast<const f16x8*>(s_lo + off);
            };
            request(0, 0);
            request(1, 1);
            __builtin_amdgcn_sched_barrier(0);
#pragma unroll
            for (int st = 0; st < 5; ++st) {
#pragma unroll
                for (int ri = 0; ri < 10; ++ri) {
                    const int i = st * 10 + ri, slot = i % 3, rho = RHO[ri];
                    bool first = true;
#pragma unroll
                    for (int kind = 0; kind < (F32 ? 3 : 1); ++kind) {
#pragma unroll
                        for (int dy = 0; dy < 3; ++dy) {
                            const int r = rho - dy;
                            if (r < 0 || r >= MR) continue;
                            acc[r] = __builtin_amdgcn_mfma_f32_16x16x32_f16(kind == 1 ? wl[dy][st] : wh[dy][st], kind == 2 ? xl[slot] : xh[slot], acc[r], 0, 0, 0);
                            if (first) {
                                first = false;
                                if (i + 2 < 50) request(i + 2, (i + 2) % 3);
                                __builtin_amdgcn_sched_barrier(0);
                            }
                        }
                    }
                    __builtin_amdgcn_sched_barrier(0);
                }
            }
#ifdef SEMABS_TUNING
            if (a.ablate == 4) { if (acc[0][0] != 1234.5f) continue; }
#endif
            float ps[4] = {0.f, 0.f, 0.f, 0.f};
            f32x4 cA, cB, cC;
            f32x4 ad[MR];
            if (GNB && a.gnb_add) {
                ad[0] = *reinterpret_cast<const f32x4*>(a.gnb_add + vol_off + ooff[0]);
                ad[1] = *reinterpret_cast<const f32x4*>(a.gnb_add + vol_off + ooff[1]);
            }
            if (GNB) {
                cA = *reinterpret_cast<const f32x4*>(s_gnb + b * 48 + 4 * kg); cB = *reinterpret_cast<const f32x4*>(s_gnb + b * 48 + 16 + 4 * kg);
                cC = *reinterpret_cast<const f32x4*>(s_gnb + b * 48 + 32 + 4 * kg);
            }
#pragma unroll
            for (int mi = 0; mi < MR; ++mi) {
                float o[4];
                if (GNB) {
                    if (a.gnb_add && mi + 2 < MR) { ad[mi + 2] = *reinterpret_cast<const f32x4*>(a.gnb_add + vol_off + ooff[mi + 2]); __builtin_amdgcn_sched_barrier(0); }
#pragma unroll
                    for (int e = 0; e < 4; ++e) {
                        o[e] = acc[mi][e] * cA[e] + (res[mi][e] * cB[e] + cC[e]);
                        if (a.gnb_add) o[e] += ad[mi][e];
                        if (a.gnb_relu) o[e] = res[mi][e] > 0.f ? o[e] : 0.f;
                        amax = fmaxf(amax, fabsf(o[e]));
                    }
                } else {
#pragma unroll
                for (int e = 0; e < 4; ++e) o[e] = fmaxf(acc[mi][e] + bias4[e] + res[mi][e], relu_floor);
                }
                if (!F32) {
#pragma unroll
                    for (int e = 0; e < 4; ++e) o[e] = (float)(f16)o[e];
                }
                ps[0] += o[0] + o[1]; ps[1] += o[0] * o[0] + o[1] * o[1];
                ps[2] += o[2] + o[3]; ps[3] += o[2] * o[2] + o[3] * o[3];
                if (F32) {
                    *reinterpret_cast<float4*>(reinterpret_cast<float*>(a.y) + vol_off + ooff[mi]) = make_float4(o[0], o[1], o[2], o[3]);
                } else {
                    f16x4 h; h[0] = (f16)o[0]; h[1] = (f16)o[1]; h[2] = (f16)o[2]; h[3] = (f16)o[3];
                    *reinterpret_cast<f16x4*>(reinterpret_cast<f16*>(a.y) + vol_off + ooff[mi]) = h;
                }
            }
            if (a.stats) {
#pragma unroll
                for (int j = 0; j < 4; ++j) st[j] += (double)ps[j];
            }
        }
    };

    auto lds_barrier = [&]() { asm volatile("s_waitcnt lgkmcnt(0)\n\ts_barrier" ::: "memory"); };
    auto brick_of = [&](int it) { return xcd_persistent_tile((int)blockIdx.x, (int)gridDim.x, it, total); };
    if (producer) {
        int it = 0, brick = brick_of(0);
        if (brick >= 0) produce(brick, 0);
        lds_barrier();
        int buf = 0;
        for (; brick >= 0; buf ^= 1) {
            const int next = brick_of(++it);
            if (next >= 0 && !CONV16_ABL(a.ablate == 2 || a.ablate >= 4)) produce(next, buf ^ 1);
            lds_barrier();
            brick = next;
        }
    } else {
        load_weights();
        lds_barrier();
        int buf = 0, it = 0;
        for (int brick = brick_of(0); brick >= 0; brick = brick_of(++it), buf ^= 1) {
            if (!CONV16_ABL(a.ablate == 1)) consume(brick, buf);
            lds_barrier();
        }
        if (a.stats) flush_stats();
        if (GNB && a.gnb_bits) conv_absmax_commit(a.gnb_bits, amax);
    }
}

#define SEMABS_CONV_GENERIC 256
#define SEMABS_CONV_PACKED 512
#ifdef SEMABS_TUNING
static int g_conv16_ablate = 0;
static long long* g_conv_trace = nullptr;
static int g_brick_persist = 0;
static int g_convt_no_line = 0;
extern "C" int semabs_conv_tune(int key, long long value) {
    if (key == 0) g_conv16_ablate = (int)value & 7;
    else if (key == 1) g_conv_trace = reinterpret_cast<long long*>(value);
    else if (key == 2) g_brick_persist = (int)value;
    else if (key == 3) g_convt_no_line = (int)value;
    return SEMABS_OK;
}
#endif

static int conv16_lds_launch(const ConvArgs& a_in, int f32, hipStream_t s) {
    ConvArgs a = a_in;
#ifdef SEMABS_TUNING
    a.ablate = g_conv16_ablate;
#endif
    if (f32) {
        constexpr int T0 = 4;
        const size_t lds = (size_t)(((T0 + 2) * C16_H1 * C16_H2 * 8 + 127) / 128 * 128) * 2 * 2 * 2 * 2;
        const long total = (long)a.B * (a.I0 / T0) * (a.I1 / C16_T1) * (a.I2 / C16_T2);
        long nb = semabs_stream_cus(s); if (nb > total) nb = total;
        if (a.gnb_coef) {
            static SemabsLdsAttr attrg;
            semabs_ensure_lds(&k_conv16_lds<true, T0, true>, (int)(lds + 32 * 192), attrg);
            hipLaunchKernelGGL((k_conv16_lds<true, T0, true>), dim3((unsigned)nb), dim3(512), lds + (size_t)a.B * 192, s, a);
            SEMABS_CHECK_LAUNCH();
            return SEMABS_OK;
        }
        if (a.occ) {
            static SemabsLdsAttr attrs;
            semabs_ensure_lds(&k_conv16_lds<true, T0, false, true>, (int)lds, attrs);
            hipLaunchKernelGGL((k_conv16_lds<true, T0, false, true>), dim3((unsigned)nb), dim3(512), lds, s, a);
            SEMABS_CHECK_LAUNCH();
            return SEMABS_OK;
        }
        static SemabsLdsAttr attr;
        semabs_ensure_lds(&k_conv16_lds<true, T0>, (int)lds, attr);
        hipLaunchKernelGGL((k_conv16_lds<true, T0>), dim3((unsigned)nb), dim3(512), lds, s, a);
    } else {
        constexpr int T0 = 8;
        const size_t lds = (size_t)(((T0 + 2) * C16_H1 * C16_H2 * 8 + 127) / 128 * 128) * 2 * 2 * 2;
        const long total = (long)a.B * (a.I0 / T0) * (a.I1 / C16_T1) * (a.I2 / C16_T2);
        long nb = semabs_stream_cus(s); if (nb > total) nb = total;
        if (a.occ) {
            static SemabsLdsAttr attrs;
            semabs_ensure_lds(&k_conv16_lds<false, T0, false, true>, (int)lds, attrs);
            hipLaunchKernelGGL((k_conv16_lds<false, T0, false, true>), dim3((unsigned)nb), dim3(512), lds, s, a);
            SEMABS_CHECK_LAUNCH();
            return SEMABS_OK;
        }
        static SemabsLdsAttr attr;
        semabs_ensure_lds(&k_conv16_lds<false, T0>, (int)lds, attr);
        hipLaunchKernelGGL((k_conv16_lds<false, T0>), dim3((unsigned)nb), dim3(512), lds, s, a);
    }
    SEMABS_CHECK_LAUNCH();
    return SEMABS_OK;
}

template <bool F32, int CW, int NB, bool ONE, bool PERSIST, int TX = 16, bool GNB = false>
__global__ __launch_bounds__(512) void k_conv_brick(ConvArgs a, int total) {
    constexpr int T0 = 4, H0 = T0 + 2, HX = TX + 2, HALO = H0 * C16_H1 * HX, NTHR = 512;
    constexpr int R = TX / 4;
    constexpr int CPV = CW / 8;
    constexpr int NSTEPS = CW == 32 ? 27 : 14;
    constexpr bool EARLY = false;
    extern __shared__ __attribute__((aligned(16))) char smem[];
    constexpr int PLANE = (HALO * 8 + 127) / 128 * 128;
    f16* s_hi = reinterpret_cast<f16*>(smem);
    f16* s_lo = s_hi + PLANE * CPV;
    const int tid = threadIdx.x, lane = tid & 63;
    const int wid = __builtin_amdgcn_readfirstlane(tid >> 6);
    const int vl = lane & 15, kg = lane >> 4;
    const int n2 = a.I2 / TX, n1 = a.I1 / C16_T1, n0 = a.I0 / T0;
    const int per_vol = n0 * n1 * n2;
    const bool has_gn = a.gn_scale != nullptr;
    const int Cin = ONE ? CW : a.Cin;
    const int nchunks = ONE ? 1 : Cin / CW;
#ifdef SEMABS_TUNING
    long long* trc = a.trace ? a.trace + (long)blockIdx.x * 8 : nullptr;
#define BRICK_STAMP(i) do { if (trc && tid == 0) trc[i] = (long long)__builtin_readcyclecounter(); } while (0)
#else
#define BRICK_STAMP(i) do { } while (0)
#endif
    auto decode = [&](int t, int& b, int& cout0, int& z0, int& y0, int& x0) {
        int br = t % per_vol; t /= per_vol;
        b = t % a.B; cout0 = (t / a.B) * (NB * 16);
        const int t2 = br % n2; br /= n2;
        const int t1 = br % n1; const int t0 = br / n1;
        z0 = t0 * T0; y0 = t1 * C16_T1; x0 = t2 * TX;
    };
    auto frag_z = [&](int f) { return TX == 16 ? f >> 3 : f >> 2; };
    auto frag_y = [&](int f, int v) { return TX == 16 ? (f & 7) : 2 * (f & 3) + (v >> 3); };
    auto frag_x = [&](int v) { return TX == 16 ? v : (v & 7); };
    int rbase[R];
#pragma unroll
    for (int r = 0; r < R; ++r) {
        const int f = wid * R + r;
        rbase[r] = ((frag_z(f) + 1) * C16_H1 + (frag_y(f, vl) + 1)) * HX + (frag_x(vl) + 1);
    }
    constexpr int VPI = NTHR / CPV;
    constexpr int NIT = (HALO + VPI - 1) / VPI;
    const int c = tid % CPV;
    const int vsub = tid / CPV;
    float raw[NIT][8];
    float gs[8], gh[8];
    unsigned inb = 0;
    auto issue = [&](int tile, int cc) {
        int b, cout0, z0, y0, x0;
        decode(tile, b, cout0, z0, y0, x0);
        const int ch = cc * CW + c * 8;
        if (has_gn) {
            const float4* ps = reinterpret_cast<const float4*>(a.gn_scale + (long)b * Cin + ch);
            const float4* pt = reinterpret_cast<const float4*>(a.gn_shift + (long)b * Cin + ch);
            const float4 s0 = ps[0], s1 = ps[1], h0 = pt[0], h1 = pt[1];
            gs[0] = s0.x; gs[1] = s0.y; gs[2] = s0.z; gs[3] = s0.w; gs[4] = s1.x; gs[5] = s1.y; gs[6] = s1.z; gs[7] = s1.w;
            gh[0] = h0.x; gh[1] = h0.y; gh[2] = h0.z; gh[3] = h0.w; gh[4] = h1.x; gh[5] = h1.y; gh[6] = h1.z; gh[7] = h1.w;
        } else {
#pragma unroll
            for (int j = 0; j < 8; ++j) { gs[j] = 1.f; gh[j] = 0.f; }
        }
        inb = 0;
#pragma unroll
        for (int it = 0; it < NIT; ++it) {
            const int v = min(vsub + it * VPI, HALO - 1);
            const int hx = v % HX, hy = (v / HX) % C16_H1, hz = v / (HX * C16_H1);
            const int gz = z0 + hz - 1, gy = y0 + hy - 1, gx = x0 + hx - 1;
            if (gz >= 0 && gz < a.I0 && gy >= 0 && gy < a.I1 && gx >= 0 && gx < a.I2) inb |= 1u << it;
            const int cz = min(max(gz, 0), a.I0 - 1), cy = min(max(gy, 0), a.I1 - 1), cx = min(max(gx, 0), a.I2 - 1);
            load8<F32>(a.x, ((((long)b * a.I0 + cz) * a.I1 + cy) * a.I2 + cx) * Cin + ch, raw[it]);
        }
    };
    auto commit = [&]() {
#pragma unroll
        for (int it = 0; it < NIT; ++it) {
            const int v = vsub + it * VPI;
            const bool in = (inb >> it) & 1u;
            f16x8 h, l;
#pragma unroll
            for (int j = 0; j < 8; ++j) {
                const float val = in ? raw[it][j] * gs[j] + gh[j] : 0.f;
                h[j] = (f16)val; if (F32) l[j] = (f16)(val - (float)h[j]);
            }
            if (v < HALO) {
                const int off = c * PLANE + v * 8;
                *reinterpret_cast<f16x8*>(s_hi + off) = h;
                if (F32) *reinterpret_cast<f16x8*>(s_lo + off) = l;
            }
        }
    };

    int tile = PERSIST ? (int)blockIdx.x : xcd_remap((int)blockIdx.x, (int)gridDim.x);
    if (tile >= total) return;
    BRICK_STAMP(6);
    issue(tile, 0);
    for (;;) {
    int b, cout0, z0, y0, x0;
    decode(tile, b, cout0, z0, y0, x0);
    BRICK_STAMP(0);
    f32x4 acc[R][NB];
#pragma unroll
    for (int r = 0; r < R; ++r)
#pragma unroll
        for (int nb = 0; nb < NB; ++nb) acc[r][nb] = f32x4{0.f, 0.f, 0.f, 0.f};
    for (int cc = 0; cc < nchunks; ++cc) {
        __syncthreads();
        commit();
        BRICK_STAMP(2);
        __syncthreads();
        BRICK_STAMP(3);
        int ntile = tile, ncc = cc + 1;
        if (ncc == nchunks) { ntile = PERSIST ? tile + (int)gridDim.x : total; ncc = 0; }
        if (EARLY && ntile < total) issue(ntile, ncc);
        auto step_geom = [&](int ks, int& voff, int& chunk, long& kofs) {
            if (CW == 32) {
                chunk = kg; voff = ((ks / 9) - 1) * C16_H1 * HX + (((ks / 3) % 3) - 1) * HX + ((ks % 3) - 1);
                kofs = (long)ks * Cin + cc * 32 + kg * 8;
            } else {
                const int ta = 2 * ks, tb = (2 * ks + 1 < 27) ? 2 * ks + 1 : 26;
                const int offa = ((ta / 9) - 1) * C16_H1 * HX + (((ta / 3) % 3) - 1) * HX + ((ta % 3) - 1);
                const int offb = ((tb / 9) - 1) * C16_H1 * HX + (((tb / 3) % 3) - 1) * HX + ((tb % 3) - 1);
                voff = (kg >> 1) ? offb : offa; chunk = kg & 1;
                const int tap = ONE ? 2 * ks + (kg >> 1) : min(2 * ks + (kg >> 1), 26);
                kofs = (long)tap * Cin + cc * 16 + (kg & 1) * 8;
            }
        };
        const bool packed = a.wp_hi != nullptr;
        const int ncb = a.Cout >> 4;
        auto w_index = [&](int ks, int nb, long kofs) -> long {
            return packed ? ((long)((CW == 32 ? ks * (Cin >> 5) + cc : ks) * ncb + (cout0 >> 4) + nb) * 64 + lane) * 8
                          : (long)(cout0 + nb * 16 + vl) * a.Kp + kofs;
        };
        const f16* const wbase_h = packed ? a.wp_hi : a.w_hi;
        const f16* const wbase_l = packed ? a.wp_lo : a.w_lo;
        auto load_w = [&](int ks, f16x8* wh, f16x8* wl) {
            int voff, chunk; long kofs;
            step_geom(ks, voff, chunk, kofs);
#pragma unroll
            for (int nb = 0; nb < NB; ++nb) {
                const long widx = w_index(ks, nb, kofs);
                wh[nb] = *reinterpret_cast<const f16x8*>(wbase_h + widx);
                if (F32) wl[nb] = *reinterpret_cast<const f16x8*>(wbase_l + widx);
                if (CW == 16 && !ONE) {
                    const bool dead = ks == NSTEPS - 1 && (kg >> 1);
// ... 160 lines not shown
        if (a.stats) {
            const int cg = a.Cout >> 3;
            float* s_stat = reinterpret_cast<float*>(smem);
            __syncthreads();
            if (tid < 16) s_stat[tid] = 0.f;
            __syncthreads();
#pragma unroll
            for (int nb = 0; nb < NB; ++nb) {
                float vs = st_s[nb], vq = st_q[nb];
#pragma unroll
                for (int m = 4; m < 64; m <<= 1) { vs += __shfl_xor(vs, m, 64); vq += __shfl_xor(vq, m, 64); }
                if (v2 == 0) {
                    const int gl = (nb * 16 + 4 * k2) / cg;
                    atomicAdd(&s_stat[gl * 2], vs); atomicAdd(&s_stat[gl * 2 + 1], vq);
                }
            }
            __syncthreads();
            const int ngl = (NB * 16 >= cg) ? NB * 16 / cg : 1;
            if (tid < ngl * 2) atomicAdd(a.stats + ((long)b * 8 + cout0 / cg + (tid >> 1)) * 2 + (tid & 1), (double)s_stat[tid]);
            if (PERSIST) __syncthreads();
        }
    }
    BRICK_STAMP(5);
    if (!PERSIST) break;
    tile += gridDim.x;
    if (tile >= total) break;
    }
    BRICK_STAMP(7);
}

template <bool F32, int CW, int NB, bool ONE, bool PERSIST, int TX = 16, bool GNB = false>
static int conv_brick_launch_p(const ConvArgs& a, hipStream_t s) {
    const size_t lds = (size_t)((6 * C16_H1 * (TX + 2) * 8 + 127) / 128 * 128) * (CW / 8) * 2 * (F32 ? 2 : 1);
    static int per_cu = 0;
    if (!per_cu) {
        (void)hipFuncSetAttribute(reinterpret_cast<const void*>(&k_conv_brick<F32, CW, NB, ONE, PERSIST, TX, GNB>), hipFuncAttributeMaxDynamicSharedMemorySize, (int)lds);
        int n = 0;
        if (hipOccupancyMaxActiveBlocksPerMultiprocessor(&n, k_conv_brick<F32, CW, NB, ONE, PERSIST, TX, GNB>, 512, lds) != hipSuccess || n < 1) n = 1;
        per_cu = n;
    }
    const long total = (long)(a.I0 / 4) * (a.I1 / C16_T1) * (a.I2 / TX) * a.B * (a.Cout / (NB * 16));
    SEMABS_REQUIRE(total < (1L << 30), "conv brick: too many tiles");
    long nwg = total;
    if (PERSIST) { nwg = (long)semabs_stream_cus(s) * per_cu; if (nwg > total) nwg = total; }
    ConvArgs at = a;
#ifdef SEMABS_TUNING
    at.trace = g_conv_trace;
#endif
    hipLaunchKernelGGL((k_conv_brick<F32, CW, NB, ONE, PERSIST, TX, GNB>), dim3((unsigned)nwg), dim3(512), lds, s, at, (int)total);
    SEMABS_CHECK_LAUNCH();
    return SEMABS_OK;
}
template <bool F32, int CW, int NB, bool ONE>
static int conv_brick_launch_t(const ConvArgs& a, hipStream_t s) {
#ifdef SEMABS_TUNING
    if (g_brick_persist) return conv_brick_launch_p<F32, CW, NB, ONE, true>(a, s);
#endif
    return conv_brick_launch_p<F32, CW, NB, ONE, false>(a, s);
}
static int conv_brick_launch(const ConvArgs& a, int f32, hipStream_t s) {
    if (a.gnb_coef) {
        if (a.Cin == 32) return conv_brick_launch_p<true, 32, 2, true, false, 16, true>(a, s);
        return conv_brick_launch_p<true, 32, 2, false, false, 16, true>(a, s);
    }
    if (a.I2 % C16_T2 != 0) {
        return f32 ? conv_brick_launch_p<true, 32, 2, false, false, 8>(a, s) : conv_brick_launch_p<false, 32, 2, false, false, 8>(a, s);
    }
    const long bricks = (long)a.B * (a.I0 / 4) * (a.I1 / C16_T1) * (a.I2 / C16_T2);
    if (a.Cout == 16) {
        if (a.Cin == 32) return f32 ? conv_brick_launch_t<true, 32, 1, true>(a, s) : conv_brick_launch_t<false, 32, 1, true>(a, s);
        return f32 ? conv_brick_launch_t<true, 32, 1, false>(a, s) : conv_brick_launch_t<false, 32, 1, false>(a, s);
    }
    const bool nb4 = a.Cout % 64 == 0 && bricks * (a.Cout / 64) >= 512;
    if (a.Cin == 16) {
        if (nb4) return f32 ? conv_brick_launch_t<true, 16, 4, true>(a, s) : conv_brick_launch_t<false, 16, 4, true>(a, s);
        return f32 ? conv_brick_launch_t<true, 16, 2, true>(a, s) : conv_brick_launch_t<false, 16, 2, true>(a, s);
    }
    if (a.Cin == 32) {
        if (nb4) return f32 ? conv_brick_launch_t<true, 32, 4, true>(a, s) : conv_brick_launch_t<false, 32, 4, true>(a, s);
        return f32 ? conv_brick_launch_t<true, 32, 2, true>(a, s) : conv_brick_launch_t<false, 32, 2, true>(a, s);
    }
    if (nb4) return f32 ? conv_brick_launch_t<true, 32, 4, false>(a, s) : conv_brick_launch_t<false, 32, 4, false>(a, s);
    return f32 ? conv_brick_launch_t<true, 32, 2, false>(a, s) : conv_brick_launch_t<false, 32, 2, false>(a, s);
}

__global__ void k_conv_finish(float* __restrict__ y, const float* __restrict__ bias, const float* __restrict__ resid, long n4, int C, int relu) {
    const long i = (long)blockIdx.x * blockDim.x + threadIdx.x;
    if (i >= n4) return;
    float4 v = *reinterpret_cast<float4*>(y + i * 4);
    if (bias) { const float4 b = *reinterpret_cast<const float4*>(bias + (i * 4) % C); v.x += b.x; v.y += b.y; v.z += b.z; v.w += b.w; }
    if (resid) { const float4 r = *reinterpret_cast<const float4*>(resid + i * 4); v.x += r.x; v.y += r.y; v.z += r.z; v.w += r.w; }
    if (relu == 1) { v.x = fmaxf(v.x, 0.f); v.y = fmaxf(v.y, 0.f); v.z = fmaxf(v.z, 0.f); v.w = fmaxf(v.w, 0.f); }
    else if (relu == 2) { v.x = v.x > 0.f ? v.x : 0.01f * v.x; v.y = v.y > 0.f ? v.y : 0.01f * v.y; v.z = v.z > 0.f ? v.z : 0.01f * v.z; v.w = v.w > 0.f ? v.w : 0.01f * v.w; }
    *reinterpret_cast<float4*>(y + i * 4) = v;
}

static int conv_launch(const ConvArgs& a_in, int f32, hipStream_t s) {
    ConvArgs a = a_in;
    const long Mtot = (long)a.B * a.M0 * a.M1 * a.M2;
    a.ksplit = 1;
    if (f32 && a.os == 1 && a.Cout % 64 == 0 && a.Cin % 32 == 0 && a.ntaps == 27 && Mtot <= 16384) {
        const long slices = semabs_cdiv(Mtot, 4 * 32) * (a.Cout / 64);
        int ks = (int)(2048 / (slices > 0 ? slices : 1));
        if (ks > 27) ks = 27;
        if (ks >= 3) {
            a.ksplit = ks;
            semabs_fill32(a.y, (size_t)Mtot * a.Cout * sizeof(float), 0u, s);
            dim3 grid(semabs_cdiv(Mtot, 4 * 32), a.Cout / 64, ks), block(256);
            hipLaunchKernelGGL((k_conv<4, true, false, true>), grid, block, 0, s, a);
            const long n4 = Mtot * a.Cout / 4;
            hipLaunchKernelGGL(k_conv_finish, dim3(semabs_cdiv(n4, 256)), dim3(256), 0, s, reinterpret_cast<float*>(a.y), a.bias,
                               reinterpret_cast<const float*>(a.resid), n4, a.Cout, a.relu);
            SEMABS_CHECK_LAUNCH();
            return SEMABS_OK;
        }
    }
    const int ncls = a.ncls > 0 ? a.ncls : 1;
    int nw = a.Cout >= 64 ? 4 : (a.Cout >= 32 ? 2 : 1);
    while (nw > 1 && (long)semabs_cdiv(Mtot, 4 * 32) * (a.Cout / (nw * 16)) * ncls < 1024) nw >>= 1;
    dim3 grid(semabs_cdiv(Mtot, 4 * 32), a.Cout / (nw * 16), ncls), block(256);
    const bool c16 = a.Cin == 16;
    if (a.ncls > 0) {
#define CONVC_GO(NW_, F_) hipLaunchKernelGGL((k_conv<NW_, F_, false, false, true>), grid, block, 0, s, a)
        if (f32) { if (nw == 4) CONVC_GO(4, true); else if (nw == 2) CONVC_GO(2, true); else CONVC_GO(1, true); }
        else { if (nw == 4) CONVC_GO(4, false); else if (nw == 2) CONVC_GO(2, false); else CONVC_GO(1, false); }
#undef CONVC_GO
        SEMABS_CHECK_LAUNCH();
        return SEMABS_OK;
    }
#define CONV_GO(NW_, F_, C_) hipLaunchKernelGGL((k_conv<NW_, F_, C_>), grid, block, 0, s, a)
#define CONV_NW(F_, C_) { if (nw == 4) CONV_GO(4, F_, C_); else if (nw == 2) CONV_GO(2, F_, C_); else CONV_GO(1, F_, C_); }
    if (nw == 4 && !c16) {
        if (f32) hipLaunchKernelGGL((k_conv<4, true, false, true>), grid, block, 0, s, a);
        else hipLaunchKernelGGL((k_conv<4, false, false, true>), grid, block, 0, s, a);
    }
    else if (f32) { if (c16) CONV_NW(true, true) else CONV_NW(true, false) }
    else { if (c16) CONV_NW(false, true) else CONV_NW(false, false) }
#undef CONV_NW
#undef CONV_GO
    SEMABS_CHECK_LAUNCH();
    return SEMABS_OK;
}

static int conv_common_checks(const void* x, const void* w_hi, const void* w_lo, void* y, int Cin, int Cout, int f32) {
    SEMABS_REQUIRE(x && w_hi && y, "semabs conv: null pointer");
    SEMABS_REQUIRE(!f32 || w_lo, "semabs conv: exact (fp32) mode needs the lo half of the split weights");
    SEMABS_REQUIRE(Cin == 16 || Cin % 32 == 0, "semabs conv: Cin must be 16 or a multiple of 32");
    SEMABS_REQUIRE(Cout % 16 == 0 && (Cout < 64 || Cout % 64 == 0), "semabs conv: Cout must be 16, 32 or a multiple of 64");
    return SEMABS_OK;
}

static int conv3d_impl(const void* x, const void* w_hi, const void* w_lo, void* y, const float* gn_scale, const float* gn_shift,
                       const float* bias, const void* resid, int B, int D0, int D1, int D2, int Cin, int Cout, int ksize,
                       int relu, int act_flags, double* out_sums, int out_groups, void* stream, const unsigned int* occ = nullptr) {
    if (B == 0) return SEMABS_OK;
    const int act_f32 = act_flags & 1;
    const bool bricks = !(act_flags & SEMABS_CONV_GENERIC);
    int rc = conv_common_checks(x, w_hi, w_lo, y, Cin, Cout, act_f32);
    if (rc) return rc;
    SEMABS_REQUIRE(ksize == 1 || ksize == 3, "semabs_conv3d: kernel size must be 1 or 3");
    SEMABS_REQUIRE((gn_scale == nullptr) == (gn_shift == nullptr), "semabs_conv3d: gn_scale and gn_shift go together");
    ConvArgs a;
    a.x = x; a.y = y; a.w_hi = (const f16*)w_hi; a.w_lo = (const f16*)w_lo; a.gn_scale = gn_scale; a.gn_shift = gn_shift;
    a.bias = bias; a.resid = resid; a.B = B; a.I0 = D0; a.I1 = D1; a.I2 = D2; a.O0 = D0; a.O1 = D1; a.O2 = D2;
    a.M0 = D0; a.M1 = D1; a.M2 = D2; a.os = 1; a.is = 1; a.op0 = a.op1 = a.op2 = 0; a.Cin = Cin; a.Cout = Cout; a.relu = relu;
    a.ntaps = ksize * ksize * ksize;
    a.Kp = ((a.ntaps * Cin + 31) / 32) * 32;
    a.stats = nullptr; a.ablate = 0; a.trace = nullptr; a.wp_hi = nullptr; a.wp_lo = nullptr; a.ncls = 0;
    if (act_flags & SEMABS_CONV_PACKED) {
        a.wp_hi = a.w_hi + (long)Cout * a.Kp;
        if (w_lo) a.wp_lo = a.w_lo + (long)Cout * a.Kp;
    }
    int t = 0;
    for (int kd = 0; kd < ksize; ++kd)
        for (int kh = 0; kh < ksize; ++kh)
            for (int kw = 0; kw < ksize; ++kw, ++t) { a.td0[t] = kd - ksize / 2; a.td1[t] = kh - ksize / 2; a.td2[t] = kw - ksize / 2; }
    SEMABS_REQUIRE(relu == 0 || relu == 1 || (relu == 2 && ksize == 1), "semabs_conv3d: relu must be 0, 1, or 2 (LeakyReLU, ksize 1 only)");
    SEMABS_REQUIRE(!out_sums || (out_groups > 0 && Cout % out_groups == 0), "semabs_conv3d_stats: Cout must be a multiple of out_groups");
    bool fused = false;
    if (bricks && ksize == 3 && Cin == 16 && Cout == 16 && D0 % 8 == 0 && D1 % C16_T1 == 0 && D2 % C16_T2 == 0 && (long)D0 * D1 * D2 * 16 < (1L << 31)) {
        if (out_sums && out_groups == 8) { a.stats = out_sums; fused = true; }
        a.occ = occ;
        rc = conv16_lds_launch(a, act_f32, (hipStream_t)stream);
    } else if (occ) {
        semabs_set_error("semabs_conv3d_sparse_stats: the occupancy bitmap is read by the 16 -> 16 level-0 kernel only (D0 % 8, D1 % 8, D2 % 16 == 0)");
        return SEMABS_EINVAL;
    } else if (bricks && ksize == 3 && (Cout % 32 == 0 || (Cout == 16 && Cin % 32 == 0 && D2 % C16_T2 == 0)) && (Cin == 16 || Cin % 32 == 0) && relu != 2 &&
               D0 % 4 == 0 && D1 % C16_T1 == 0 && (D2 % C16_T2 == 0 || (D2 % 8 == 0 && Cin % 32 == 0))) {
        if (out_sums && out_groups == 8 && Cout >= 32) { a.stats = out_sums; fused = true; }
        rc = conv_brick_launch(a, act_f32, (hipStream_t)stream);
    } else {
        rc = conv_launch(a, act_f32, (hipStream_t)stream);
    }
    if (rc == SEMABS_OK && out_sums && !fused) rc = semabs_gn_stats(y, out_sums, B, (long)D0 * D1 * D2, Cout, out_groups, act_f32, stream);
    return rc;
}
extern "C" int semabs_conv3d(const void* x, const void* w_hi, const void* w_lo, void* y, const float* gn_scale, const float* gn_shift,
                             const float* bias, const void* resid, int B, int D0, int D1, int D2, int Cin, int Cout, int ksize,
                             int relu, int act_f32, void* stream) {
    return conv3d_impl(x, w_hi, w_lo, y, gn_scale, gn_shift, bias, resid, B, D0, D1, D2, Cin, Cout, ksize, relu, act_f32, nullptr, 0, stream);
}
extern "C" int semabs_conv3d_stats(const void* x, const void* w_hi, const void* w_lo, void* y, const float* gn_scale, const float* gn_shift,
                                   const float* bias, const void* resid, int B, int D0, int D1, int D2, int Cin, int Cout, int ksize,
                                   int relu, int act_f32, double* out_sums, int out_groups, void* stream) {
    SEMABS_REQUIRE(out_sums, "semabs_conv3d_stats: out_sums is null");
    return conv3d_impl(x, w_hi, w_lo, y, gn_scale, gn_shift, bias, resid, B, D0, D1, D2, Cin, Cout, ksize, relu, act_f32, out_sums, out_groups, stream);
}

extern "C" int semabs_conv3d_sparse_stats(const void* x, const unsigned int* occ, const void* w_hi, const void* w_lo, void* y, const float* gn_scale, const float* gn_shift,
                                          const float* bias, const void* resid, int B, int D0, int D1, int D2, int Cin, int Cout, int ksize,
                                          int relu, int act_f32, double* out_sums, int out_groups, void* stream) {
    SEMABS_REQUIRE(out_sums && occ, "semabs_conv3d_sparse_stats: out_sums / occ is null");
    SEMABS_REQUIRE(!(act_f32 & SEMABS_CONV_GENERIC), "semabs_conv3d_sparse_stats: the generic kernel reads the whole volume");
    return conv3d_impl(x, w_hi, w_lo, y, gn_scale, gn_shift, bias, resid, B, D0, D1, D2, Cin, Cout, ksize, relu, act_f32, out_sums, out_groups, stream, occ);
}

static int conv3d_gnbwd_route(int B, int D0, int D1, int D2, int Cin, int Cout, int G, bool have_add) {
    if (B <= 0 || G <= 0) return 0;
    if (B <= 32 && Cin == 16 && Cout == 16 && D0 % 8 == 0 && D1 % C16_T1 == 0 && D2 % C16_T2 == 0 && (long)D0 * D1 * D2 * 16 < (1L << 31) && 16 % G == 0) return 1;
    if (!have_add && Cin % 32 == 0 && Cout % 32 == 0 && Cout % G == 0 && (Cout / G) % 4 == 0 && D0 % 4 == 0 && D1 % C16_T1 == 0 && D2 % C16_T2 == 0) return 2;
    return 0;
}
extern "C" int semabs_conv3d_gnbwd_supported(int B, int D0, int D1, int D2, int Cin, int Cout, int G, int have_add1, int* ok) {
    SEMABS_REQUIRE(ok, "semabs_conv3d_gnbwd_supported: null pointer");
    *ok = conv3d_gnbwd_route(B, D0, D1, D2, Cin, Cout, G, have_add1 != 0) ? 1 : 0;
    return SEMABS_OK;
}
extern "C" int semabs_conv3d_gnbwd(const void* dZ, const void* w_hi, const void* w_lo, void* dX, const float* in_scale, const float* in_shift, const void* X,
                                   const float* mean, const float* rstd, const float* coef, int G, const float* add1, int relu_mask, unsigned int* absmax_bits,
                                   int B, int D0, int D1, int D2, int Cin, int Cout, int act_flags, void* stream) {
    if (B == 0) return SEMABS_OK;
    SEMABS_REQUIRE(dZ && w_hi && w_lo && dX && X && mean && rstd && coef, "semabs_conv3d_gnbwd: null pointer");
    const int route = conv3d_gnbwd_route(B, D0, D1, D2, Cin, Cout, G, add1 != nullptr);
    SEMABS_REQUIRE((act_flags & 1) && route, "semabs_conv3d_gnbwd: exact mode and a supported shape (see semabs_conv3d_gnbwd_supported)");
    SEMABS_REQUIRE((in_scale == nullptr) == (in_shift == nullptr), "semabs_conv3d_gnbwd: in_scale and in_shift go together");
    ConvArgs a;
    a.x = dZ; a.y = dX; a.w_hi = (const f16*)w_hi; a.w_lo = (const f16*)w_lo; a.gn_scale = in_scale; a.gn_shift = in_shift;
    a.bias = nullptr; a.resid = X; a.B = B; a.I0 = D0; a.I1 = D1; a.I2 = D2; a.O0 = D0; a.O1 = D1; a.O2 = D2;
    a.M0 = D0; a.M1 = D1; a.M2 = D2; a.os = 1; a.is = 1; a.op0 = a.op1 = a.op2 = 0; a.Cin = Cin; a.Cout = Cout; a.relu = 0;
    a.ntaps = 27; a.Kp = ((27 * Cin + 31) / 32) * 32;
    a.stats = nullptr; a.ablate = 0; a.trace = nullptr; a.wp_hi = nullptr; a.wp_lo = nullptr; a.ncls = 0; a.ksplit = 1;
    int t = 0;
    for (int kd = 0; kd < 3; ++kd)
        for (int kh = 0; kh < 3; ++kh)
            for (int kw = 0; kw < 3; ++kw, ++t) { a.td0[t] = kd - 1; a.td1[t] = kh - 1; a.td2[t] = kw - 1; }
    a.gnb_coef = coef; a.gnb_mean = mean; a.gnb_rstd = rstd; a.gnb_G = G; a.gnb_relu = relu_mask; a.gnb_bits = absmax_bits; a.gnb_add = add1;
    if (act_flags & SEMABS_CONV_PACKED) { a.wp_hi = a.w_hi + (long)Cout * a.Kp; a.wp_lo = a.w_lo + (long)Cout * a.Kp; }
    return route == 1 ? conv16_lds_launch(a, 1, (hipStream_t)stream) : conv_brick_launch(a, 1, (hipStream_t)stream);
}

extern "C" int semabs_conv3d_gather(const void* x, const void* w_hi, const void* w_lo, void* y, const float* in_scale, const float* in_shift,
                                    int B, int I0, int I1, int I2, int M0, int M1, int M2, int in_stride, int Cin, int Cout, int ntaps,
                                    const signed char* taps, int act_f32, void* stream) {
    if (B == 0) return SEMABS_OK;
    const int act_flags = act_f32;
    act_f32 = act_flags & 1;
    int rc = conv_common_checks(x, w_hi, w_lo, y, Cin, Cout, act_f32);
    if (rc) return rc;
    SEMABS_REQUIRE(taps && ntaps >= 1 && ntaps <= 28 && in_stride >= 1, "semabs_conv3d_gather: bad taps / stride");
    ConvArgs a;
    SEMABS_REQUIRE((in_scale == nullptr) == (in_shift == nullptr), "semabs_conv3d_gather: in_scale and in_shift go together");
    a.x = x; a.y = y; a.w_hi = (const f16*)w_hi; a.w_lo = (const f16*)w_lo; a.gn_scale = in_scale; a.gn_shift = in_shift;
    a.bias = nullptr; a.resid = nullptr; a.stats = nullptr; a.ablate = 0; a.trace = nullptr; a.wp_hi = nullptr; a.wp_lo = nullptr; a.ncls = 0; a.B = B; a.I0 = I0; a.I1 = I1; a.I2 = I2; a.O0 = M0; a.O1 = M1; a.O2 = M2;
    a.M0 = M0; a.M1 = M1; a.M2 = M2; a.os = 1; a.is = in_stride; a.op0 = a.op1 = a.op2 = 0; a.Cin = Cin; a.Cout = Cout; a.relu = 0;
    a.ntaps = ntaps; a.Kp = ((ntaps * Cin + 31) / 32) * 32;
    if (act_flags & SEMABS_CONV_PACKED) { a.wp_hi = a.w_hi + (long)Cout * a.Kp; if (a.w_lo) a.wp_lo = a.w_lo + (long)Cout * a.Kp; }
    for (int t = 0; t < ntaps; ++t) { a.td0[t] = taps[t * 3]; a.td1[t] = taps[t * 3 + 1]; a.td2[t] = taps[t * 3 + 2]; }
    return conv_launch(a, act_f32, (hipStream_t)stream);
}

struct ConvTArgs {
    const void* x; void* y; const f16* w_hi; const f16* w_lo; const float* bias; const void* skip;
    long class_off[8];
    int B, D0, D1, D2, Cin, Cout;
    double* stats;
    long packed_off;
};
template <bool F32, int P0, bool LINE = false>
__global__ __launch_bounds__(512) void k_convT_brick(ConvTArgs a) {
    constexpr int T0 = 4, T1 = 8, T2 = 16, H0 = T0 + 1, H1 = T1 + 1, H2 = T2 + 1, HALO = H0 * H1 * H2, NTHR = 512, CW = 32, CPV = 4;
    extern __shared__ __attribute__((aligned(16))) char smem[];
    f16* s_hi = reinterpret_cast<f16*>(smem);
    f16* s_lo = s_hi + HALO * CW;
    const int tid = threadIdx.x, lane = tid & 63;
    const int wid = __builtin_amdgcn_readfirstlane(tid >> 6);
    const int vl = lane & 15, kg = lane >> 4;
    const int b = blockIdx.y, cout0 = blockIdx.z * 16;
    const int n2 = a.D2 / T2, n1 = a.D1 / T1;
    int t = (gridDim.y * gridDim.z == 1 || gridDim.x % 8 == 0) ? xcd_remap((int)blockIdx.x, (int)gridDim.x) : (int)blockIdx.x;
    const int t2 = t % n2; t /= n2;
    const int t1 = t % n1; const int t0 = t / n1;
    const int z0 = t0 * T0, y0 = t1 * T1, x0 = t2 * T2;
    auto swz = [](int v, int chunk) { return chunk ^ ((v >> 2) & 3); };

    f32x4 acc[4][4];
#pragma unroll
    for (int r = 0; r < 4; ++r)
#pragma unroll
        for (int c = 0; c < 4; ++c) acc[r][c] = f32x4{0.f, 0.f, 0.f, 0.f};
    int rbase[4];
#pragma unroll
    for (int r = 0; r < 4; ++r) {
        const int row = wid * 4 + r;
        rbase[r] = ((row >> 3) * H1 + (row & 7)) * H2 + vl;
    }
    const int nchunks = a.Cin / CW;
    for (int cc = 0; cc < nchunks; ++cc) {
        if (cc) __syncthreads();
        constexpr int NIT = (HALO * CPV + NTHR - 1) / NTHR;
        const int c = tid % CPV;
        const int ch = cc * CW + c * 8;
        float raw[NIT][8];
        bool inb[NIT];
#pragma unroll
        for (int it = 0; it < NIT; ++it) {
            const int v = (tid + it * NTHR) / CPV;
            const int hx = v % H2, hy = (v / H2) % H1, hz = v / (H2 * H1);
            const int gz = z0 + hz, gy = y0 + hy, gx = x0 + hx;
            inb[it] = v < HALO && gz < a.D0 && gy < a.D1 && gx < a.D2;
            if (inb[it]) load8<F32>(a.x, ((((long)b * a.D0 + gz) * a.D1 + gy) * a.D2 + gx) * a.Cin + ch, raw[it]);
        }
#pragma unroll
        for (int it = 0; it < NIT; ++it) {
            const int v = (tid + it * NTHR) / CPV;
            f16x8 h, l;
#pragma unroll
            for (int j = 0; j < 8; ++j) {
                const float val = inb[it] ? raw[it][j] : 0.f;
                h[j] = (f16)val; if (F32) l[j] = (f16)(val - (float)h[j]);
            }
            if (v < HALO) {
                const int off = v * CW + swz(v, c) * 8;
                *reinterpret_cast<f16x8*>(s_hi + off) = h;
                if (F32) *reinterpret_cast<f16x8*>(s_lo + off) = l;
            }
        }
        __syncthreads();
#pragma unroll
        for (int c4 = 0; c4 < 4; ++c4) {
            constexpr int p0 = P0;
            const int cls = P0 * 4 + c4, p1 = (c4 >> 1) & 1, p2 = c4 & 1;
            const int ntaps = (p0 + 1) * (p1 + 1) * (p2 + 1);
            const long kp = (long)ntaps * a.Cin;
            const f16* wh_c = a.w_hi + a.packed_off + a.class_off[cls];
            const f16* wl_c = F32 ? a.w_lo + a.packed_off + a.class_off[cls] : nullptr;
            int tt = 0;
#pragma unroll
            for (int q0 = 0; q0 <= p0; ++q0)
#pragma unroll
                for (int q1 = 0; q1 <= p1; ++q1)
#pragma unroll
                    for (int q2 = 0; q2 <= p2; ++q2, ++tt) {
                        const int d0 = p0 ? (q0 == 0 ? 1 : 0) : 0, d1 = p1 ? (q1 == 0 ? 1 : 0) : 0, d2 = p2 ? (q2 == 0 ? 1 : 0) : 0;
                        const int voff = (d0 * H1 + d1) * H2 + d2;
                        const long widx = a.packed_off ? ((long)((tt * (a.Cin >> 5) + cc) * (a.Cout >> 4) + (cout0 >> 4)) * 64 + lane) * 8
                                                       : (long)(cout0 + vl) * kp + (long)tt * a.Cin + cc * 32 + kg * 8;
                        const f16x8 wh = *reinterpret_cast<const f16x8*>(wh_c + widx);
                        f16x8 wl;
                        if (F32) wl = *reinterpret_cast<const f16x8*>(wl_c + widx);
#pragma unroll
                        for (int r = 0; r < 4; ++r) {
                            const int v = rbase[r] + voff;
                            const int off = v * CW + swz(v, kg) * 8;
                            const f16x8 xh = *reinterpret_cast<const f16x8*>(s_hi + off);
                            acc[r][c4] = __builtin_amdgcn_mfma_f32_16x16x32_f16(wh, xh, acc[r][c4], 0, 0, 0);
                            if (F32) {
                                const f16x8 xl = *reinterpret_cast<const f16x8*>(s_lo + off);
// ... 479 lines not shown
```

### semantic-abstraction_amd/unet3d.py

```python
from __future__ import annotations

import ctypes as C
from typing import Dict, List

import numpy as np
import torch

from . import _lib


def number_of_features_per_level(init_channel_number, num_levels):
    return [init_channel_number * 2 ** k for k in range(num_levels)]



def _pack_fragments(w: torch.Tensor) -> torch.Tensor:
    cout, kp = int(w.shape[0]), int(w.shape[1])
    assert cout % 16 == 0 and kp % 32 == 0
    return w.reshape(cout // 16, 16, kp // 32, 4, 8).permute(2, 0, 3, 1, 4).contiguous().reshape(-1)


def matrix_layout(m: torch.Tensor):
    rows, k = int(m.shape[0]), int(m.shape[1])
    kp = (k + 31) // 32 * 32
    if kp != k:
        m = torch.cat([m, m.new_zeros(rows, kp - k)], dim=1)
    m = m.contiguous()
    if rows % 16 == 0:
        return torch.cat([m.reshape(-1), _pack_fragments(m)]), 512
    return m.reshape(-1), 0


def conv_fwd_layout(w: torch.Tensor):
    return matrix_layout(w.permute(0, 2, 3, 4, 1).reshape(w.shape[0], -1))


def conv_bwd_layout(w: torch.Tensor):
    return matrix_layout(w.flip(2, 3, 4).permute(1, 2, 3, 4, 0).reshape(w.shape[1], -1))


def linear_layout(w: torch.Tensor, transposed: bool = False):
    return matrix_layout(w.t() if transposed else w)


def convT_class_layout(w: torch.Tensor):
    cin, cout = int(w.shape[0]), int(w.shape[1])
    mats, offs, off = [], [], 0
    for cls in range(8):
        p = (cls >> 2, (cls >> 1) & 1, cls & 1)
        cols = []
        for t0 in range(p[0] + 1):
            for t1 in range(p[1] + 1):
                for t2 in range(p[2] + 1):
                    k = [1 if pp == 0 else (0 if t == 0 else 2) for pp, t in zip(p, (t0, t1, t2))]
                    cols.append(w[:, :, k[0], k[1], k[2]].t())
        mats.append(torch.cat(cols, dim=1).contiguous())
        offs.append(off)
        off += mats[-1].numel()
    packed = cout % 16 == 0 and cin % 32 == 0
    return torch.cat([m.reshape(-1) for m in mats] + ([_pack_fragments(m) for m in mats] if packed else [])), 512 if packed else 0, offs


def _split16(w: torch.Tensor, dev):
    hi = w.to(torch.float16)
    lo = (w - hi.float()).to(torch.float16)
    return hi.to(dev).contiguous(), lo.to(dev).contiguous()


class _Conv:
    name = None
    bwd = None

    def __init__(self, weight: torch.Tensor, gn_w, gn_b, bias, groups: int, dev):
        flat, packed = conv_fwd_layout(weight.float())
        f = lambda t: None if t is None else t.float().to(dev).contiguous()
        self._set((*_split16(flat, dev), packed), weight.shape, f(gn_w), f(gn_b), f(bias), groups)

    def _set(self, fwd, wshape, gn_w, gn_b, bias, groups):
        self.w_hi, self.w_lo, self.packed = fwd
        self.cout, self.cin, self.k = int(wshape[0]), int(wshape[1]), int(wshape[2])
        self.gn_w, self.gn_b, self.bias = gn_w, gn_b, bias
        self.groups = groups if self.cin >= groups else 1

    @classmethod
    def of(cls, name, fwd, bwd, wshape, gn_w, gn_b, bias, groups):
        r = cls.__new__(cls)
        r.name, r.bwd = name, bwd
        r._set(fwd, wshape, gn_w, gn_b, bias, groups)
        return r


class _ConvT:
    name = None
    bwd = None

    def __init__(self, weight: torch.Tensor, bias, dev):
        flat, packed, offs = convT_class_layout(weight.float())
        self._set((*_split16(flat, dev), packed, offs), weight.shape, bias.float().to(dev).contiguous())

    def _set(self, fwd, wshape, bias):
        self.w_hi, self.w_lo, self.packed, offs = fwd
        self.class_off = (C.c_long * 8)(*offs)
        self.cin, self.cout = int(wshape[0]), int(wshape[1])
        self.bias = bias

    @classmethod
    def of(cls, name, fwd, bwd, wshape, bias):
        r = cls.__new__(cls)
        r.name, r.bwd = name, bwd
        r._set(fwd, wshape, bias)
        return r


class _Rec:
    __slots__ = ("name", "x", "y", "mean", "rstd", "scale", "shift")



def gn_conv(x, conv: _Conv, relu, zeros, f32, resid=None, gn=True, in_sums=None, out_groups=0, generic=False, occ=None, rec: _Rec | None = None):
    B, D0, D1, D2, Cc = x.shape
    nvox, dev, st = D0 * D1 * D2, x.device, _lib.stream()
    scale = shift = None
    if gn:
        G, sums = conv.groups, in_sums
        if sums is None:
            sums = zeros((B, G, 2), torch.float64)
            _lib.call("semabs_gn_stats", _lib.ptr(x), _lib.ptr(sums), B, nvox, Cc, G, f32, st)
        scale = torch.empty(B, Cc, dtype=torch.float32, device=dev)
        shift = torch.empty_like(scale)
        _lib.call("semabs_gn_finalize", _lib.ptr(sums), _lib.ptr(conv.gn_w), _lib.ptr(conv.gn_b), _lib.ptr(scale), _lib.ptr(shift),
                  B, Cc, G, nvox, 1e-5, st)
        if rec is not None:
            rec.mean = torch.empty(B, G, dtype=torch.float32, device=dev)
            rec.rstd = torch.empty_like(rec.mean)
            _lib.call("semabs_gn_meanrstd", _lib.ptr(sums), _lib.ptr(rec.mean), _lib.ptr(rec.rstd), B, G, nvox * (Cc // G), 1e-5, st)
    y = torch.empty(B, D0, D1, D2, conv.cout, dtype=torch.float32 if f32 else torch.float16, device=dev)
    if rec is not None:
        rec.name, rec.x, rec.y, rec.scale, rec.shift = conv.name, x, y, scale, shift
    args = (_lib.ptr(x), _lib.ptr(conv.w_hi), _lib.ptr(conv.w_lo), _lib.ptr(y), _lib.ptr(scale), _lib.ptr(shift),
            _lib.ptr(conv.bias), _lib.ptr(resid), B, D0, D1, D2, conv.cin, conv.cout, conv.k, int(relu), f32 | (256 if generic else 0) | conv.packed)
    if not out_groups:
        assert occ is None
        _lib.call("semabs_conv3d", *args, st)
        return y, None
    out_sums = zeros((B, out_groups, 2), torch.float64)
    if occ is not None:
        _lib.call("semabs_conv3d_sparse_stats", args[0], _lib.ptr(occ), *args[1:], _lib.ptr(out_sums), out_groups, st)
    else:
        _lib.call("semabs_conv3d_stats", *args, _lib.ptr(out_sums), out_groups, st)
    return y, out_sums


def res_block(x, convs, zeros, f32, in_sums=None, occ=None, tape=None):
    r1, r2, r3 = (None,) * 3 if tape is None else (_Rec(), _Rec(), _Rec())
    out1, s1 = gn_conv(x, convs[0], True, zeros, f32, in_sums=in_sums, out_groups=convs[1].groups, occ=occ, rec=r1)
    out2, s2 = gn_conv(out1, convs[1], True, zeros, f32, in_sums=s1, out_groups=convs[2].groups, rec=r2)
    y, _ = gn_conv(out2, convs[2], True, zeros, f32, resid=out1, in_sums=s2, rec=r3)
    if tape is not None:
        tape.append(("block", r1, r2, r3))
    return y


def maxpool(x, f32):
    B, D0, D1, D2, Cc = x.shape
    y = torch.empty(B, D0 // 2, D1 // 2, D2 // 2, Cc, dtype=x.dtype, device=x.device)
    _lib.call("semabs_maxpool3d", _lib.ptr(x), _lib.ptr(y), B, D0, D1, D2, Cc, f32, _lib.stream())
    return y


def up_conv(x, skip, ct: _ConvT, zeros, f32, out_groups=0, generic=False):
    B, D0, D1, D2, _ = x.shape
    assert tuple(skip.shape) == (B, 2 * D0, 2 * D1, 2 * D2, ct.cout)
    y = torch.empty_like(skip)
    args = (_lib.ptr(x), _lib.ptr(ct.w_hi), _lib.ptr(ct.w_lo), ct.class_off, _lib.ptr(y),
            _lib.ptr(ct.bias), _lib.ptr(skip), B, D0, D1, D2, ct.cin, ct.cout, f32 | (256 if generic else 0) | ct.packed)
    if not out_groups:
        _lib.call("semabs_convtranspose3d", *args, _lib.stream())
        return y, None
    sums = zeros((B, out_groups, 2), torch.float64)
    _lib.call("semabs_convtranspose3d_stats", *args, _lib.ptr(sums), out_groups, _lib.stream())
    return y, sums


def unet_forward(x, enc, dec, final: _Conv, zeros, f32, in_sums=None, occ=None, taps=None, skip_final=False, tape=None, rows_w=None):
    feats = []
    for i, convs in enumerate(enc):
        if i > 0:
            if tape is not None:
                tape.append(("pool", x, i - 1))
            x = maxpool(x, f32)
        x = res_block(x, convs, zeros, f32, in_sums=in_sums if i == 0 else None, occ=occ if i == 0 else None, tape=tape)
        if taps is not None:
            taps[f"enc{i}"] = x
        feats.insert(0, x)
    for i, (skip, (ct, convs)) in enumerate(zip(feats[1:], dec)):
        y, sums = up_conv(x, skip, ct, zeros, f32, out_groups=convs[0].groups)
        if tape is not None:
            tape.append(("up", ct.name, x, len(enc) - 2 - i))
        x = res_block(y, convs, zeros, f32, in_sums=sums, tape=tape)
        if taps is not None:
            taps[f"dec{i}"] = x
    if skip_final:
        return x
    if tape is not None:
        tape.append(("final", x))
    if rows_w is None:
        return gn_conv(x, final, False, zeros, f32, gn=False)[0]
    B, D0, D1, D2, _ = x.shape
    y = torch.empty(B, D0, D1, D2, final.cout, dtype=torch.float32, device=x.device)
    _lib.call("semabs_linear_rows", _lib.ptr(x), final.cin, _lib.ptr(rows_w), final.cin, 1, _lib.ptr(final.bias), _lib.ptr(y),
              B * D0 * D1 * D2, final.cin, final.cout, 0, 0.0, None, None, None, None, None, None, _lib.stream())
    return y


class ResidualUNet3D(torch.nn.Module):

    def __init__(self, in_channels, out_channels, f_maps=64, num_groups=8, num_levels=5, final_sigmoid=False,
                 layer_order="gcr", is_segmentation=False, precision: str = "exact", **kwargs):
        super().__init__()
        assert layer_order == "gcr" and not is_segmentation, "the path uses order 'gcr' without a final activation"
        assert precision in ("fp16", "exact")
        if isinstance(f_maps, int):
            f_maps = number_of_features_per_level(f_maps, num_levels=num_levels)
        self.f_maps = list(f_maps)
        self.in_channels, self.out_channels, self.num_groups = in_channels, out_channels, num_groups
        self.precision = precision
        self.f32 = int(precision == "exact")
        self.act_dtype = torch.float32 if self.f32 else torch.float16
        from .module import register_tree
        from .weights import make_unet_state_dict
        seed = int(torch.randint(0, 2 ** 31 - 1, (1,)).item())
        register_tree(self, make_unet_state_dict(seed, in_channels, out_channels, self.f_maps[0], len(self.f_maps)))
        self._sums_arena = None
        self.enc: List[List[_Conv]] = []
        self.dec: List = []
        self.final = None
        self._sig = None

    @property
    def dev(self):
        return _lib.require_gpu()

    def expected_keys(self):
        from .weights import unet_layer_plan
        keys = []
        for pre, kind, cin, cout in unet_layer_plan(self.in_channels, self.out_channels, self.f_maps[0], len(self.f_maps)):
            if kind in ("gcr", "gc"):
                keys += [pre + "groupnorm.weight", pre + "groupnorm.bias", pre + "conv.weight"]
            else:
                keys += [pre + "weight", pre + "bias"]
        return keys

    def load_state_dict(self, state_dict, strict: bool = True, prefix: str = "", **kw):
        from .module import strip_module_prefix
        sd = strip_module_prefix(state_dict)
        if prefix:
            sd = {k[len(prefix):]: v for k, v in sd.items() if k.startswith(prefix)}
        return super().load_state_dict(sd, strict=strict, **kw)

    def _sync(self):
        from .module import signature
        dev = _lib.require_gpu()
        if any(p.device.type != "cuda" for p in self.parameters()):
            self.to(dev)
        sig = signature(self)
        if sig == self._sig:
            return
        sd = {k: v.detach() for k, v in self.state_dict().items()}
        G = self.num_groups

        def block(pre):
            return [_Conv(sd[pre + f"conv{j}.conv.weight"], sd[pre + f"conv{j}.groupnorm.weight"],
                          sd[pre + f"conv{j}.groupnorm.bias"], None, G, dev) for j in (1, 2, 3)]

        L = len(self.f_maps)
        self.enc = [block(f"encoders.{i}.basic_module.") for i in range(L)]
        self.dec = [(_ConvT(sd[f"decoders.{i}.upsampling.upsample.weight"], sd[f"decoders.{i}.upsampling.upsample.bias"], dev),
                     block(f"decoders.{i}.basic_module.")) for i in range(L - 1)]
        self.final = _Conv(sd["final_conv.weight"], None, None, sd["final_conv.bias"], G, dev)
        self._sig = sig

    def _zero_sums(self, shape, dtype=torch.float64) -> torch.Tensor:
        assert dtype == torch.float64 and len(shape) == 3
        n = shape[0] * shape[1] * shape[2]
        a = self._sums_arena
        if a is None or a[1] + n > a[0].numel():
            return _lib.filled(tuple(shape), torch.float64, 0, self.dev)
        t = a[0][a[1]:a[1] + n].view(*shape)
        a[1] += n
        return t

    def _conv(self, x, conv: _Conv, relu, resid=None, gn=True, in_sums=None, out_groups=0, generic=False, occ=None):
        y, sums = gn_conv(x, conv, relu, self._zero_sums, self.f32, resid, gn, in_sums, out_groups, generic, occ)
        return (y, sums) if out_groups else y

    @staticmethod
    def sparse_input_supported(shape, conv: "_Conv") -> bool:
        _, D0, D1, D2, Cc = shape
        return conv.k == 3 and conv.cin == 16 and conv.cout == 16 and Cc == 16 and D0 % 8 == 0 and D1 % 8 == 0 and D2 % 16 == 0 and D0 * D1 * D2 * 16 < 2 ** 31

    def _pool(self, x):
        return maxpool(x, self.f32)

    def _up(self, x, skip, ct: _ConvT, out_groups=0, generic=False):
        y, sums = up_conv(x, skip, ct, self._zero_sums, self.f32, out_groups, generic)
        return (y, sums) if out_groups else y

    @torch.no_grad()
    def forward_cl(self, x: torch.Tensor, taps: dict | None = None, skip_final: bool = False, in_sums=None, occ=None) -> torch.Tensor:
        self._sync()
        assert x.dtype == self.act_dtype and x.is_contiguous()
        n_layers = 3 * (len(self.enc) + len(self.dec)) + len(self.dec) + 2
        self._sums_arena = [_lib.filled((n_layers * int(x.shape[0]) * max(1, self.num_groups) * 2,), torch.float64, 0, self.dev), 0]
        try:
            return unet_forward(x, self.enc, self.dec, self.final, self._zero_sums, self.f32, in_sums, occ, taps, skip_final)
        finally:
            self._sums_arena = None

    def forward(self, x: torch.Tensor) -> torch.Tensor:
        dev = _lib.require_gpu()
        xc = x.to(dev).permute(0, 2, 3, 4, 1).contiguous().to(self.act_dtype)
        y = self.forward_cl(xc)
        return y.permute(0, 4, 1, 2, 3).contiguous().float()
```

Baseline: 8.799 scenes/s.

## Fuse maxpool into conv epilogue, batch color jitter, group labels in aggregation

Three unrelated changes. The encoder's last convolution per level now emits the 2x max-pooled volume and its GroupNorm sums from a fused epilogue in the 16->16 exact kernel, with a fallback that runs maxpool plus stats separately. This drops a separate pool pass and a separate stats pass. Color jitter for all augmentations is launched as batched kernels, one per permutation step, instead of a per-image loop, which cuts launch count. Relevancy aggregation now handles four labels per thread so tile geometry setup is shared across labels, at the cost of more register pressure and a larger LDS footprint for the pooled conv.

```diff
diff --git a/include/semabs.h b/include/semabs.h
--- a/include/semabs.h
+++ b/include/semabs.h
@@ -55,12 +55,16 @@
 
 int semabs_aggregate(const float* rel, const float* rel_flip, int L, int N, int g, int H, int W, const int* scales,
                      int n_scales, int n_img, int tiles_per_img, float* out, void* stream);
+int semabs_aggregate_grouped(const float* rel, const float* rel_flip, int L, int N, int g, int H, int W, const int* scales,
+                             int n_scales, int n_img, int tiles_per_img, float* out, void* stream);
 
 int semabs_unflip_average(const float* rel, const float* rel_flip, float* out, long n_maps, int g, void* stream);
 int semabs_unflip_average_rows(const float* rel, const float* rel_flip, float* out, int L, long maps_per_label, long in_label_stride, int g, void* stream);
 
 int semabs_color_jitter(unsigned char* img, int H, int W, const int* order4, const float* factors4, void* scratch8, void* stream);
 int semabs_color_jitter_op(unsigned char* img, int H, int W, int op, float factor, void* scratch8, void* stream);
+int semabs_color_jitter_batched(unsigned char* imgs, int n_img, int H, int W, const int* orders, const float* factors, void* scratch,
+                                long long scratch_bytes, void* stream);
 
 
 int semabs_gemm_f16(const void* A, const void* B, void* C, const float* bias, const float* addend, long M, int N, int K,
@@ -137,6 +141,9 @@
                                  const void* skip, int B, int D0, int D1, int D2, int Cin, int Cout, int act_f32, double* out_sums,
                                  int out_groups, void* stream);
 int semabs_maxpool3d(const void* x, void* y, int B, int D0, int D1, int D2, int C, int act_f32, void* stream);
+int semabs_conv3d_pool(const void* x, const void* w_hi, const void* w_lo, void* y, const float* gn_scale, const float* gn_shift, const float* bias,
+                       const void* resid, int B, int D0, int D1, int D2, int Cin, int Cout, int ksize, int relu, int act_f32, void* pooled,
+                       double* pool_sums, int pool_groups, void* stream);
 int semabs_decoder(const void* vol, const float* query, const float* off3, const float* sc3, const int* shape3, const float* w1,
                    const float* b1, const float* w2, const float* b2, int concat_xyz, int P, long M, long q_stride_p, int vol_f32,
                    float* out, const int* qgrid3, const float* final_w, const float* final_b, void* stream);
diff --git a/semantic-abstraction_amd/_lib.py b/semantic-abstraction_amd/_lib.py
--- a/semantic-abstraction_amd/_lib.py
+++ b/semantic-abstraction_amd/_lib.py
@@ -42,10 +42,12 @@
     "semabs_tile_patches": [P, I, I, I, P, I, P, P, P, P, P, I, I, I, P],
     "semabs_patchify": [P, P, I, I, I, P],
     "semabs_aggregate": [P, P, I, I, I, I, I, P, I, I, I, P, P],
+    "semabs_aggregate_grouped": [P, P, I, I, I, I, I, P, I, I, I, P, P],
     "semabs_unflip_average": [P, P, P, L, I, P],
     "semabs_unflip_average_rows": [P, P, P, I, L, L, I, P],
     "semabs_color_jitter": [P, I, I, C.POINTER(I), C.POINTER(F), P, P],
     "semabs_color_jitter_op": [P, I, I, I, F, P, P],
+    "semabs_color_jitter_batched": [P, I, I, I, C.POINTER(I), C.POINTER(F), P, C.c_longlong, P],
     "semabs_gemm_f16": [P, P, P, P, P, L, I, I, L, I, L, I, C.POINTER(I), P],
     "semabs_gemm_f16_ex": [P, P, P, P, P, L, I, I, L, I, L, I, C.POINTER(I), I, P, P, P],
     "semabs_gemm_f16_ln": [P, P, P, P, L, I, I, L, I, L, I, P, P, P, P, P, P, P, I, L, I, P, P, P],
@@ -84,6 +86,7 @@
     "semabs_convtranspose3d": [P, P, P, C.POINTER(C.c_long), P, P, P, I, I, I, I, I, I, I, P],
     "semabs_convtranspose3d_stats": [P, P, P, C.POINTER(C.c_long), P, P, P, I, I, I, I, I, I, I, P, I, P],
     "semabs_maxpool3d": [P, P, I, I, I, I, I, I, P],
+    "semabs_conv3d_pool": [P, P, P, P, P, P, P, P, I, I, I, I, I, I, I, I, I, P, P, I, P],
     "semabs_vool_head": [P, P, P, P, P, C.POINTER(F), C.POINTER(F), C.POINTER(I), F, I, L, I, P, P],
     "semabs_lamb_step": [P, I, P, I, D, D, D, D, D, I, P, P, P],
     "semabs_decoder": [P, P, C.POINTER(F), C.POINTER(F), C.POINTER(I), P, P, P, P, I, I, L, L, I, P, C.POINTER(I), P, P, P],
diff --git a/semantic-abstraction_amd/clip/__init__.py b/semantic-abstraction_amd/clip/__init__.py
--- a/semantic-abstraction_amd/clip/__init__.py
+++ b/semantic-abstraction_amd/clip/__init__.py
@@ -224,14 +224,16 @@
             _lib.call("semabs_replicate", _lib.ptr(base), _lib.ptr(out), H * W * 3, augmentations + 1, _lib.stream())
         else:
             out.copy_(base[None].expand_as(out))
-        if cls._jitter_scratch is None:
-            cls._jitter_scratch = torch.empty(1, dtype=torch.int64, device=dev)
+        if cls._jitter_scratch is None or cls._jitter_scratch.numel() < augmentations * 64:
+            cls._jitter_scratch = torch.empty(augmentations * 64, dtype=torch.int64, device=dev)
         scratch = cls._jitter_scratch
         rng = cls._rng if seed is None else np.random.default_rng(seed)
+        orders, factors = [], []
         for k in range(1, augmentations + 1):
-            order = rng.permutation(4)
-            f = [rng.uniform(0.4, 1.6), rng.uniform(0.4, 1.6), rng.uniform(0.4, 1.6), rng.uniform(-0.1, 0.1)]
-            _lib.call("semabs_color_jitter", out[k].data_ptr(), H, W, _lib.iarr(order), _lib.farr(f), _lib.ptr(scratch), _lib.stream())
+            orders.extend(rng.permutation(4))
+            factors.extend([rng.uniform(0.4, 1.6), rng.uniform(0.4, 1.6), rng.uniform(0.4, 1.6), rng.uniform(-0.1, 0.1)])
+        _lib.call("semabs_color_jitter_batched", out[1].data_ptr(), augmentations, H, W, _lib.iarr(orders), _lib.farr(factors),
+                  _lib.ptr(scratch), scratch.numel() * 8, _lib.stream())
         return out
 
     @classmethod
@@ -345,7 +347,7 @@
         elif len(rel) > 1:
             maps = torch.empty_like(rel[0])
             _lib.call("semabs_unflip_average", _lib.ptr(rel[0]), _lib.ptr(rel[1]), _lib.ptr(maps), L * N, g, _lib.stream())
-        _lib.call("semabs_aggregate", _lib.ptr(maps), None, L, N, g, H, W, _lib.ptr(sc), len(scales), n_img, N // n_img, _lib.ptr(out), _lib.stream())
+        _lib.call("semabs_aggregate_grouped", _lib.ptr(maps), None, L, N, g, H, W, _lib.ptr(sc), len(scales), n_img, N // n_img, _lib.ptr(out), _lib.stream())
         return out
 
 
diff --git a/semantic-abstraction_amd/csrc/tiles.hip b/semantic-abstraction_amd/csrc/tiles.hip
--- a/semantic-abstraction_amd/csrc/tiles.hip
+++ b/semantic-abstraction_amd/csrc/tiles.hip
@@ -331,6 +331,81 @@
     return SEMABS_OK;
 }
 
+template <int LG>
+__global__ __launch_bounds__(256) void k_aggregate_lg(const float* __restrict__ rel, const float* __restrict__ rel_flip,
+                                                      const int* __restrict__ scales, AggArgs a, float* __restrict__ out) {
+    const long i = (long)blockIdx.x * blockDim.x + threadIdx.x;
+    const long hw = (long)a.H * a.W;
+    if (i >= hw) return;
+    const int c = (int)(i % a.W), r = (int)(i / a.W);
+    const int l0 = blockIdx.y * LG;
+    const int g = a.g, gg = g * g;
+    long lbase[LG];
+#pragma unroll
+    for (int k = 0; k < LG; ++k) lbase[k] = (long)(l0 + k < a.L ? l0 + k : a.L - 1) * a.N * gg;
+    float total[LG];
+#pragma unroll
+    for (int k = 0; k < LG; ++k) total[k] = 0.f;
+    for (int s = 0; s < a.n_scales; ++s) {
+        const int ts = scales[s * 5], stride = scales[s * 5 + 1], nx = scales[s * 5 + 2], ny = scales[s * 5 + 3], base = scales[s * 5 + 4];
+        int ix_hi = r / stride; if (ix_hi > nx - 1) ix_hi = nx - 1;
+        int ix_lo = r - ts + 1 <= 0 ? 0 : (r - ts + 1 + stride - 1) / stride;
+        int iy_hi = c / stride; if (iy_hi > ny - 1) iy_hi = ny - 1;
+        int iy_lo = c - ts + 1 <= 0 ? 0 : (c - ts + 1 + stride - 1) / stride;
+        __half acc[LG];
+#pragma unroll
+        for (int k = 0; k < LG; ++k) acc[k] = __float2half(0.f);
+        float cnt = 1e-5f;
+        const float bscale = (float)g / (float)ts;
+        for (int im = 0; im < a.n_img; ++im) {
+            for (int iy = iy_lo; iy <= iy_hi; ++iy) {
+                int w0, w1; float lw0, lw1;
+                bil_setup(c - iy * stride, bscale, g, w0, w1, lw0, lw1);
+                for (int ix = ix_lo; ix <= ix_hi; ++ix) {
+                    int h0, h1; float lh0, lh1;
+                    bil_setup(r - ix * stride, bscale, g, h0, h1, lh0, lh1);
+                    const long tile = ((long)im * a.tiles_per_img + base + iy * nx + ix) * gg;
+                    const int o00 = h0 * g + w0, o01 = h0 * g + w1, o10 = h1 * g + w0, o11 = h1 * g + w1;
+                    const int f00 = h0 * g + (g - 1 - w0), f01 = h0 * g + (g - 1 - w1), f10 = h1 * g + (g - 1 - w0), f11 = h1 * g + (g - 1 - w1);
+#pragma unroll
+                    for (int k = 0; k < LG; ++k) {
+                        const float* p = rel + lbase[k] + tile;
+                        float v00 = p[o00], v01 = p[o01], v10 = p[o10], v11 = p[o11];
+                        if (rel_flip) {
+                            const float* q = rel_flip + lbase[k] + tile;
+                            v00 = (v00 + q[f00]) / 2; v01 = (v01 + q[f01]) / 2;
+                            v10 = (v10 + q[f10]) / 2; v11 = (v11 + q[f11]) / 2;
+                        }
+                        const float val = lh0 * (lw0 * v00 + lw1 * v01) + lh1 * (lw0 * v10 + lw1 * v11);
+                        acc[k] = __float2half(__half2float(acc[k]) + val);
+                    }
+                    cnt += 1.0f;
+                }
+            }
+        }
+#pragma unroll
+        for (int k = 0; k < LG; ++k) total[k] = total[k] + __half2float(acc[k]) / cnt;
+    }
+#pragma unroll
+    for (int k = 0; k < LG; ++k)
+        if (l0 + k < a.L) out[(long)(l0 + k) * hw + i] = total[k] / (float)a.n_scales;
+}
+
+#define AGG_LG 4
+extern "C" int semabs_aggregate_grouped(const float* rel, const float* rel_flip, int L, int N, int g, int H, int W,
+                                        const int* scales_dev, int n_scales, int n_img, int tiles_per_img, float* out, void* stream) {
+    if (L == 0) return SEMABS_OK;
+    SEMABS_REQUIRE(rel && scales_dev && out && L > 0 && N > 0 && g > 0 && H > 0 && W > 0 && n_scales > 0 && n_img > 0,
+                   "semabs_aggregate_grouped: bad args");
+    SEMABS_REQUIRE((long)n_img * tiles_per_img == N, "semabs_aggregate_grouped: tile count does not match n_img * tiles_per_img");
+    SEMABS_REQUIRE(semabs_cdiv(L, AGG_LG) <= 65535, "semabs_aggregate_grouped: too many labels");
+    AggArgs a{L, N, g, H, W, n_img, tiles_per_img, n_scales};
+    hipLaunchKernelGGL(k_aggregate_lg<AGG_LG>, dim3(semabs_cdiv((long)H * W, 256), semabs_cdiv(L, AGG_LG)), dim3(256), 0, (hipStream_t)stream,
+                       rel, rel_flip, scales_dev, a, out);
+    SEMABS_CHECK_LAUNCH();
+    return SEMABS_OK;
+}
+
 __global__ void k_unflip_average(const float* __restrict__ rel, const float* __restrict__ rel_flip, float* __restrict__ out, long n, int g,
                                  long per, long in_stride) {
     const long i = (long)blockIdx.x * blockDim.x + threadIdx.x;
@@ -428,6 +503,101 @@
     dst[i * 3] = (unsigned char)r; dst[i * 3 + 1] = (unsigned char)g; dst[i * 3 + 2] = (unsigned char)b;
 }
 
+#define JIT_MAX_IMG 16
+#define JIT_PARTS 64
+struct JitterStep { int op[JIT_MAX_IMG]; float f[JIT_MAX_IMG]; };
+
+__global__ __launch_bounds__(256) void k_grey_sum_batched(const unsigned char* __restrict__ imgs, long n, JitterStep st,
+                                                          unsigned long long* __restrict__ partial) {
+    if (st.op[blockIdx.y] != 1) return;
+    const unsigned char* img = imgs + (long)blockIdx.y * n * 3;
+    unsigned long long v = 0;
+    for (long i = (long)blockIdx.x * 256 + threadIdx.x; i < n; i += (long)JIT_PARTS * 256)
+        v += (unsigned long long)grey_u8(img[i * 3], img[i * 3 + 1], img[i * 3 + 2]);
+    __shared__ unsigned long long sh[256];
+    sh[threadIdx.x] = v;
+    __syncthreads();
+    for (int o = 128; o > 0; o >>= 1) {
+        if ((int)threadIdx.x < o) sh[threadIdx.x] += sh[threadIdx.x + o];
+        __syncthreads();
+    }
+    if (threadIdx.x == 0) partial[(long)blockIdx.y * JIT_PARTS + blockIdx.x] = sh[0];
+}
+
+__global__ __launch_bounds__(256) void k_jitter_op_batched(unsigned char* __restrict__ imgs, long n, JitterStep st,
+                                                           const unsigned long long* __restrict__ partial) {
+    const int op = st.op[blockIdx.y];
+    const float f = st.f[blockIdx.y];
+    __shared__ unsigned long long sh[JIT_PARTS];
+    if (op == 1) {
+        if (threadIdx.x < JIT_PARTS) sh[threadIdx.x] = partial[(long)blockIdx.y * JIT_PARTS + threadIdx.x];
+        __syncthreads();
+        for (int o = JIT_PARTS / 2; o > 0; o >>= 1) {
+            if ((int)threadIdx.x < o) sh[threadIdx.x] += sh[threadIdx.x + o];
+            __syncthreads();
+        }
+    }
+    const long i = (long)blockIdx.x * blockDim.x + threadIdx.x;
+    if (i >= n) return;
+    unsigned char* px = imgs + ((long)blockIdx.y * n + i) * 3;
+    int r = px[0], g = px[1], b = px[2];
+    if (op == 0) {
+        r = blend_u8(0.f, r, f); g = blend_u8(0.f, g, f); b = blend_u8(0.f, b, f);
+    } else if (op == 1) {
+        float m = (float)(int)((double)sh[0] / (double)n + 0.5);
+        r = blend_u8(m, r, f); g = blend_u8(m, g, f); b = blend_u8(m, b, f);
+    } else if (op == 2) {
+        float m = (float)grey_u8(r, g, b);
+        r = blend_u8(m, r, f); g = blend_u8(m, g, f); b = blend_u8(m, b, f);
+    } else {
+        int uh, us, uv;
+        rgb2hsv_u8(r, g, b, uh, us, uv);
+        uh = (uh + (int)f) & 255;
+        hsv2rgb_u8(uh, us, uv, r, g, b);
+    }
+    px[0] = (unsigned char)r; px[1] = (unsigned char)g; px[2] = (unsigned char)b;
+}
+
+extern "C" int semabs_color_jitter_batched(unsigned char* imgs, int n_img, int H, int W, const int* orders, const float* factors,
+                                           void* scratch, long long scratch_bytes, void* stream) {
+    if (n_img == 0) return SEMABS_OK;
+    SEMABS_REQUIRE(imgs && orders && factors && scratch && n_img > 0 && H > 0 && W > 0, "semabs_color_jitter_batched: bad args");
+    SEMABS_REQUIRE(scratch_bytes >= (long long)n_img * JIT_PARTS * 8, "semabs_color_jitter_batched: scratch must hold n_img * 64 * 8 bytes");
+    for (int k = 0; k < n_img; ++k) {
+        int seen = 0;
+        for (int p = 0; p < 4; ++p) {
+            const int op = orders[k * 4 + p];
+            SEMABS_REQUIRE(op >= 0 && op < 4, "semabs_color_jitter_batched: op must be 0..3");
+            seen |= 1 << op;
+        }
+        SEMABS_REQUIRE(seen == 15, "semabs_color_jitter_batched: every image's order must be a permutation of 0..3");
+        const float h = factors[k * 4 + 3];
+        SEMABS_REQUIRE(h >= -0.5f && h <= 0.5f, "semabs_color_jitter_batched: hue factor must lie in [-0.5, 0.5] (torchvision adjust_hue)");
+    }
+    hipStream_t s = (hipStream_t)stream;
+    const long n = (long)H * W;
+    for (int k0 = 0; k0 < n_img; k0 += JIT_MAX_IMG) {
+        const int nb = n_img - k0 < JIT_MAX_IMG ? n_img - k0 : JIT_MAX_IMG;
+        unsigned char* base = imgs + (long)k0 * n * 3;
+        unsigned long long* partial = (unsigned long long*)scratch + (long)k0 * JIT_PARTS;
+        for (int p = 0; p < 4; ++p) {
+            JitterStep st;
+            bool contrast = false;
+            for (int k = 0; k < JIT_MAX_IMG; ++k) {
+                const int op = k < nb ? orders[(k0 + k) * 4 + p] : 0;
+                float f = k < nb ? factors[(k0 + k) * 4 + op] : 1.f;
+                if (op == 3) f = (float)(((int)((double)f * 255.0) % 256 + 256) % 256);
+                st.op[k] = op; st.f[k] = f;
+                contrast |= k < nb && op == 1;
+            }
+            if (contrast) hipLaunchKernelGGL(k_grey_sum_batched, dim3(JIT_PARTS, nb), dim3(256), 0, s, base, n, st, partial);
+            hipLaunchKernelGGL(k_jitter_op_batched, dim3(semabs_cdiv(n, 256), nb), dim3(256), 0, s, base, n, st, partial);
+        }
+    }
+    SEMABS_CHECK_LAUNCH();
+    return SEMABS_OK;
+}
+
 extern "C" int semabs_color_jitter_op(unsigned char* img, int H, int W, int op, float factor, void* scratch8, void* stream) {
     SEMABS_REQUIRE(img && scratch8 && H > 0 && W > 0, "semabs_color_jitter_op: bad args");
     SEMABS_REQUIRE(op >= 0 && op < 4, "semabs_color_jitter_op: op must be 0..3");
diff --git a/semantic-abstraction_amd/csrc/unet.hip b/semantic-abstraction_amd/csrc/unet.hip
--- a/semantic-abstraction_amd/csrc/unet.hip
+++ b/semantic-abstraction_amd/csrc/unet.hip
@@ -430,6 +430,7 @@
     unsigned int* gnb_bits = nullptr;
     const unsigned int* occ = nullptr;
     const float* gnb_add = nullptr;
+    void* pool_y = nullptr; double* pool_stats = nullptr;
 };
 
 template <bool F32>
@@ -661,8 +662,9 @@
     for (int o = 1; o < 64; o <<= 1) m = fmaxf(m, __shfl_xor(m, o, 64));
     if ((threadIdx.x & 63) == 0) atomicMax(bits, __float_as_uint(m));
 }
-template <bool F32, int C16_T0, bool GNB = false, bool SPARSE = false>
+template <bool F32, int C16_T0, bool GNB = false, bool SPARSE = false, bool POOL = false>
 __global__ __launch_bounds__(512) void k_conv16_lds(ConvArgs a) {
+    static_assert(!POOL || (F32 && !GNB && !SPARSE), "POOL: the plain forward convolution in exact mode only");
     constexpr int C16_H0 = C16_T0 + 2, C16_HALO = C16_H0 * C16_H1 * C16_H2;
     constexpr int PLANE = (C16_HALO * 8 + 127) / 128 * 128;
     constexpr int BUF_EL = PLANE * 2 * (F32 ? 2 : 1);
@@ -685,6 +687,8 @@
         }
     }
     float amax = 0.f;
+    constexpr int POOL_EL = C16_T0 * 4 * 8 * 16;
+    float* const s_pool = reinterpret_cast<float*>(smem + (size_t)BUF_EL * 2 * 2);
 
     auto produce = [&](int brick, int buf) {
         const int b = brick / per_vol; int t = brick - b * per_vol;
@@ -799,7 +803,7 @@
     };
     constexpr int ROWS_PER_WAVE = C16_T0 * 2;
 
-    auto consume = [&](int brick, int buf) {
+    auto consume = [&](int brick, int buf, [[maybe_unused]] int par) {
         const int b = brick / per_vol; int t = brick - b * per_vol;
         const int t2 = t % n2; t /= n2;
         const int t1 = t % n1; const int t0 = t / n1;
@@ -807,7 +811,7 @@
         const f16* s_hi = reinterpret_cast<const f16*>(smem) + buf * BUF_EL;
         const f16* s_lo = s_hi + PLANE * 2;
         const size_t vol_off = (size_t)b * a.I0 * a.I1 * a.I2 * 16;
-        if (a.stats && b != st_b) { flush_stats(); st_b = b; }
+        if (!POOL && a.stats && b != st_b) { flush_stats(); st_b = b; }
         constexpr int MR = 8;
         int tapoff[5];
 #pragma unroll
@@ -888,6 +892,7 @@
                 cA = *reinterpret_cast<const f32x4*>(s_gnb + b * 48 + 4 * kg); cB = *reinterpret_cast<const f32x4*>(s_gnb + b * 48 + 16 + 4 * kg);
                 cC = *reinterpret_cast<const f32x4*>(s_gnb + b * 48 + 32 + 4 * kg);
             }
+            [[maybe_unused]] float oprev[4], pw[4];
 #pragma unroll
             for (int mi = 0; mi < MR; ++mi) {
                 float o[4];
@@ -910,6 +915,21 @@
                 }
                 ps[0] += o[0] + o[1]; ps[1] += o[0] * o[0] + o[1] * o[1];
                 ps[2] += o[2] + o[3]; ps[3] += o[2] * o[2] + o[3] * o[3];
+                if constexpr (POOL) {
+                    if (mi & 1) {
+                        if (mi > 1) asm volatile("s_waitcnt lgkmcnt(0)" :: "v"(pw[0]), "v"(pw[1]), "v"(pw[2]), "v"(pw[3]) : "memory");
+#pragma unroll
+                        for (int e = 0; e < 4; ++e) {
+                            const float t = fmaxf(oprev[e], o[e]);
+                            pw[e] = fmaxf(t, __int_as_float(__builtin_amdgcn_update_dpp(0, __float_as_int(t), 0xB1, 0xF, 0xF, true)));
+                        }
+                        if (!(vl & 1))
+                            *reinterpret_cast<float4*>(s_pool + par * POOL_EL + (((zl * 4 + (mi >> 1)) * 8 + (vl >> 1)) * 16 + 4 * kg)) = make_float4(pw[0], pw[1], pw[2], pw[3]);
+                    } else {
+#pragma unroll
+                        for (int e = 0; e < 4; ++e) oprev[e] = o[e];
+                    }
+                }
                 if (F32) {
                     *reinterpret_cast<float4*>(reinterpret_cast<float*>(a.y) + vol_off + ooff[mi]) = make_float4(o[0], o[1], o[2], o[3]);
                 } else {
@@ -917,10 +937,53 @@
                     *reinterpret_cast<f16x4*>(reinterpret_cast<f16*>(a.y) + vol_off + ooff[mi]) = h;
                 }
             }
-            if (a.stats) {
+            if constexpr (POOL) asm volatile("s_waitcnt lgkmcnt(0)" :: "v"(pw[0]), "v"(pw[1]), "v"(pw[2]), "v"(pw[3]) : "memory");
+            if (!POOL && a.stats) {
 #pragma unroll
                 for (int j = 0; j < 4; ++j) st[j] += (double)ps[j];
             }
+        }
+    };
+
+    auto flush_pool_stats = [&]() {
+        if (st_b >= 0) {
+#pragma unroll
+            for (int j = 0; j < 4; ++j) {
+                double v = st[j];
+#pragma unroll
+                for (int m = 4; m < 64; m <<= 1) v += __shfl_xor(v, m, 64);
+                if (lane < 4) atomicAdd(a.pool_stats + ((long)st_b * 8 + 2 * lane + (j >> 1)) * 2 + (j & 1), v);
+                st[j] = 0.0;
+            }
+        }
+    };
+    auto finish_pool = [&](int brick, int par) {
+        const int b = brick / per_vol; int t = brick - b * per_vol;
+        const int t2 = t % n2; t /= n2;
+        const int t1 = t % n1; const int t0 = t / n1;
+        const int P0 = a.I0 >> 1, P1 = a.I1 >> 1, P2 = a.I2 >> 1;
+        constexpr int RPW = C16_T0 / 2;
+        const float* sp = s_pool + par * POOL_EL;
+        const int px = (lane >> 2) & 7, c4 = lane & 3;
+        float ps[4] = {0.f, 0.f, 0.f, 0.f};
+#pragma unroll
+        for (int k = 0; k < RPW / 2; ++k) {
+            const int row = wid * RPW + 2 * k + (lane >> 5);
+            const int pz = row >> 2, py = row & 3;
+            const f32x4 u = *reinterpret_cast<const f32x4*>(sp + (((2 * pz) * 4 + py) * 8 + px) * 16 + 4 * c4);
+            const f32x4 v = *reinterpret_cast<const f32x4*>(sp + (((2 * pz + 1) * 4 + py) * 8 + px) * 16 + 4 * c4);
+            float m[4];
+#pragma unroll
+            for (int e = 0; e < 4; ++e) m[e] = fmaxf(u[e], v[e]);
+            const long oi = ((((long)b * P0 + (t0 * (C16_T0 / 2) + pz)) * P1 + (t1 * (C16_T1 / 2) + py)) * P2 + (t2 * (C16_T2 / 2) + px)) * 16 + 4 * c4;
+            *reinterpret_cast<float4*>(reinterpret_cast<float*>(a.pool_y) + oi) = make_float4(m[0], m[1], m[2], m[3]);
+            ps[0] += m[0] + m[1]; ps[1] += m[0] * m[0] + m[1] * m[1];
+            ps[2] += m[2] + m[3]; ps[3] += m[2] * m[2] + m[3] * m[3];
+        }
+        if (a.pool_stats) {
+            if (b != st_b) { flush_pool_stats(); st_b = b; }
+#pragma unroll
+            for (int j = 0; j < 4; ++j) st[j] += (double)ps[j];
         }
     };
 
@@ -941,11 +1004,14 @@
         load_weights();
         lds_barrier();
         int buf = 0, it = 0;
+        [[maybe_unused]] int prev = -1;
         for (int brick = brick_of(0); brick >= 0; brick = brick_of(++it), buf ^= 1) {
-            if (!CONV16_ABL(a.ablate == 1)) consume(brick, buf);
+            if constexpr (POOL) { if (prev >= 0) finish_pool(prev, (it - 1) & 1); prev = brick; }
+            if (!CONV16_ABL(a.ablate == 1)) consume(brick, buf, it & 1);
             lds_barrier();
         }
-        if (a.stats) flush_stats();
+        if constexpr (POOL) { if (prev >= 0) finish_pool(prev, (it - 1) & 1); if (a.pool_stats) flush_pool_stats(); }
+        if (!POOL && a.stats) flush_stats();
         if (GNB && a.gnb_bits) conv_absmax_commit(a.gnb_bits, amax);
     }
 }
@@ -990,6 +1056,14 @@
             SEMABS_CHECK_LAUNCH();
             return SEMABS_OK;
         }
+        if (a.pool_y) {
+            static SemabsLdsAttr attrp;
+            const size_t ldsp = lds + (size_t)2 * T0 * 4 * 8 * 16 * sizeof(float);
+            semabs_ensure_lds(&k_conv16_lds<true, T0, false, false, true>, (int)ldsp, attrp);
+            hipLaunchKernelGGL((k_conv16_lds<true, T0, false, false, true>), dim3((unsigned)nb), dim3(512), ldsp, s, a);
+            SEMABS_CHECK_LAUNCH();
+            return SEMABS_OK;
+        }
         static SemabsLdsAttr attr;
         semabs_ensure_lds(&k_conv16_lds<true, T0>, (int)lds, attr);
         hipLaunchKernelGGL((k_conv16_lds<true, T0>), dim3((unsigned)nb), dim3(512), lds, s, a);
@@ -1005,6 +1079,7 @@
             SEMABS_CHECK_LAUNCH();
             return SEMABS_OK;
         }
+        SEMABS_REQUIRE(!a.pool_y, "conv16: the pooled epilogue exists in exact mode only");
         static SemabsLdsAttr attr;
         semabs_ensure_lds(&k_conv16_lds<false, T0>, (int)lds, attr);
         hipLaunchKernelGGL((k_conv16_lds<false, T0>), dim3((unsigned)nb), dim3(512), lds, s, a);
@@ -1471,7 +1546,8 @@
 
 static int conv3d_impl(const void* x, const void* w_hi, const void* w_lo, void* y, const float* gn_scale, const float* gn_shift,
                        const float* bias, const void* resid, int B, int D0, int D1, int D2, int Cin, int Cout, int ksize,
-                       int relu, int act_flags, double* out_sums, int out_groups, void* stream, const unsigned int* occ = nullptr) {
+                       int relu, int act_flags, double* out_sums, int out_groups, void* stream, const unsigned int* occ = nullptr,
+                       void* pool_y = nullptr, double* pool_stats = nullptr) {
     if (B == 0) return SEMABS_OK;
     const int act_f32 = act_flags & 1;
     const bool bricks = !(act_flags & SEMABS_CONV_GENERIC);
@@ -1500,6 +1576,7 @@
     if (bricks && ksize == 3 && Cin == 16 && Cout == 16 && D0 % 8 == 0 && D1 % C16_T1 == 0 && D2 % C16_T2 == 0 && (long)D0 * D1 * D2 * 16 < (1L << 31)) {
         if (out_sums && out_groups == 8) { a.stats = out_sums; fused = true; }
         a.occ = occ;
+        a.pool_y = pool_y; a.pool_stats = pool_stats;
         rc = conv16_lds_launch(a, act_f32, (hipStream_t)stream);
     } else if (occ) {
         semabs_set_error("semabs_conv3d_sparse_stats: the occupancy bitmap is read by the 16 -> 16 level-0 kernel only (D0 % 8, D1 % 8, D2 % 16 == 0)");
@@ -1532,6 +1609,22 @@
     SEMABS_REQUIRE(out_sums && occ, "semabs_conv3d_sparse_stats: out_sums / occ is null");
     SEMABS_REQUIRE(!(act_f32 & SEMABS_CONV_GENERIC), "semabs_conv3d_sparse_stats: the generic kernel reads the whole volume");
     return conv3d_impl(x, w_hi, w_lo, y, gn_scale, gn_shift, bias, resid, B, D0, D1, D2, Cin, Cout, ksize, relu, act_f32, out_sums, out_groups, stream, occ);
+}
+
+extern "C" int semabs_maxpool3d(const void* x, void* y, int B, int D0, int D1, int D2, int C, int act_f32, void* stream);
+extern "C" int semabs_conv3d_pool(const void* x, const void* w_hi, const void* w_lo, void* y, const float* gn_scale, const float* gn_shift,
+                                  const float* bias, const void* resid, int B, int D0, int D1, int D2, int Cin, int Cout, int ksize,
+                                  int relu, int act_f32, void* pooled, double* pool_sums, int pool_groups, void* stream) {
+    SEMABS_REQUIRE(pooled && D0 % 2 == 0 && D1 % 2 == 0 && D2 % 2 == 0, "semabs_conv3d_pool: pooled is null or a volume extent is odd");
+    SEMABS_REQUIRE(!pool_sums || (pool_groups > 0 && Cout % pool_groups == 0), "semabs_conv3d_pool: Cout must be a multiple of pool_groups");
+    const bool fused = (act_f32 & 1) && !(act_f32 & SEMABS_CONV_GENERIC) && ksize == 3 && Cin == 16 && Cout == 16 && D0 % 8 == 0 && D1 % C16_T1 == 0 && D2 % C16_T2 == 0 &&
+                       (long)D0 * D1 * D2 * 16 < (1L << 31) && (!pool_sums || pool_groups == 8);
+    int rc = conv3d_impl(x, w_hi, w_lo, y, gn_scale, gn_shift, bias, resid, B, D0, D1, D2, Cin, Cout, ksize, relu, act_f32, nullptr, 0, stream, nullptr,
+                         fused ? pooled : nullptr, fused ? pool_sums : nullptr);
+    if (rc != SEMABS_OK || fused || B == 0) return rc;
+    rc = semabs_maxpool3d(y, pooled, B, D0, D1, D2, Cout, act_f32 & 1, stream);
+    if (rc == SEMABS_OK && pool_sums) rc = semabs_gn_stats(pooled, pool_sums, B, (long)(D0 / 2) * (D1 / 2) * (D2 / 2), Cout, pool_groups, act_f32 & 1, stream);
+    return rc;
 }
 
 static int conv3d_gnbwd_route(int B, int D0, int D1, int D2, int Cin, int Cout, int G, bool have_add) {
diff --git a/semantic-abstraction_amd/unet3d.py b/semantic-abstraction_amd/unet3d.py
--- a/semantic-abstraction_amd/unet3d.py
+++ b/semantic-abstraction_amd/unet3d.py
@@ -117,7 +117,8 @@
 
 
 
-def gn_conv(x, conv: _Conv, relu, zeros, f32, resid=None, gn=True, in_sums=None, out_groups=0, generic=False, occ=None, rec: _Rec | None = None):
+def gn_conv(x, conv: _Conv, relu, zeros, f32, resid=None, gn=True, in_sums=None, out_groups=0, generic=False, occ=None, rec: _Rec | None = None,
+            pool_groups=0):
     B, D0, D1, D2, Cc = x.shape
     nvox, dev, st = D0 * D1 * D2, x.device, _lib.stream()
     scale = shift = None
@@ -139,6 +140,12 @@
         rec.name, rec.x, rec.y, rec.scale, rec.shift = conv.name, x, y, scale, shift
     args = (_lib.ptr(x), _lib.ptr(conv.w_hi), _lib.ptr(conv.w_lo), _lib.ptr(y), _lib.ptr(scale), _lib.ptr(shift),
             _lib.ptr(conv.bias), _lib.ptr(resid), B, D0, D1, D2, conv.cin, conv.cout, conv.k, int(relu), f32 | (256 if generic else 0) | conv.packed)
+    if pool_groups:
+        assert occ is None and not out_groups
+        pooled = torch.empty(B, D0 // 2, D1 // 2, D2 // 2, conv.cout, dtype=y.dtype, device=dev)
+        psums = zeros((B, pool_groups, 2), torch.float64)
+        _lib.call("semabs_conv3d_pool", *args, _lib.ptr(pooled), _lib.ptr(psums), pool_groups, st)
+        return y, (pooled, psums)
     if not out_groups:
         assert occ is None
         _lib.call("semabs_conv3d", *args, st)
@@ -151,14 +158,14 @@
     return y, out_sums
 
 
-def res_block(x, convs, zeros, f32, in_sums=None, occ=None, tape=None):
+def res_block(x, convs, zeros, f32, in_sums=None, occ=None, tape=None, pool_groups=0):
     r1, r2, r3 = (None,) * 3 if tape is None else (_Rec(), _Rec(), _Rec())
     out1, s1 = gn_conv(x, convs[0], True, zeros, f32, in_sums=in_sums, out_groups=convs[1].groups, occ=occ, rec=r1)
     out2, s2 = gn_conv(out1, convs[1], True, zeros, f32, in_sums=s1, out_groups=convs[2].groups, rec=r2)
-    y, _ = gn_conv(out2, convs[2], True, zeros, f32, resid=out1, in_sums=s2, rec=r3)
+    y, pooled = gn_conv(out2, convs[2], True, zeros, f32, resid=out1, in_sums=s2, rec=r3, pool_groups=pool_groups)
     if tape is not None:
         tape.append(("block", r1, r2, r3))
-    return y
+    return (y, pooled) if pool_groups else y
 
 
 def maxpool(x, f32):
@@ -184,12 +191,16 @@
 
 def unet_forward(x, enc, dec, final: _Conv, zeros, f32, in_sums=None, occ=None, taps=None, skip_final=False, tape=None, rows_w=None):
     feats = []
+    pooled = None
     for i, convs in enumerate(enc):
         if i > 0:
             if tape is not None:
                 tape.append(("pool", x, i - 1))
-            x = maxpool(x, f32)
-        x = res_block(x, convs, zeros, f32, in_sums=in_sums if i == 0 else None, occ=occ if i == 0 else None, tape=tape)
+            x, in_sums = pooled
+        pg = enc[i + 1][0].groups if i + 1 < len(enc) else 0
+        x = res_block(x, convs, zeros, f32, in_sums=in_sums, occ=occ if i == 0 else None, tape=tape, pool_groups=pg)
+        if pg:
+            x, pooled = x
         if taps is not None:
             taps[f"enc{i}"] = x
         feats.insert(0, x)
```

Result: no change. 8.873 scenes/s, median of 6 (+0.8%).
